# jamornsriwasansak/evplp

Hardware: AMD Instinct MI355X
Metric: Mpaths/s (higher is better)
Workload: dtype f32

## Files before the change

evplp_amd/__init__.py:

```python
from __future__ import annotations

import ctypes as C
import os
from typing import Optional, Sequence

import numpy as np

_HERE = os.path.dirname(os.path.abspath(__file__))
LIB_PATH = os.environ.get("EVPLP_LIB") or os.path.join(_HERE, "lib", "libevplp_hip.so")
INCLUDE_DIR = os.path.join(os.path.dirname(_HERE), "include")

ABI_VERSION = 5

OK, ERR_INVALID, ERR_NO_DEVICE, ERR_HIP, ERR_IO, ERR_PARSE, ERR_OOM = 0, -1, -2, -3, -4, -5, -6
USABLE_VPL, USABLE_PHOTON, LAMBERT_ONLY, PHONG_ONLY = 1, 2, 4, 8
MIS_MODES = {"one": 0, "balance": 1, "max": 2, "power2": 3, "geometryClamp": 4, "geometryBrdfClamp": 5}
BVH_LBVH, BVH_SAH, BVH_SBVH, BVH_LBVH_GPU = 0, 1, 2, 3
(BUF_RECORDS, BUF_GBUF_POSITION, BUF_GBUF_NORMAL, BUF_GBUF_DIFFUSE, BUF_GBUF_PHONG, BUF_LIGHT,
 BUF_VPL_ACCUM, BUF_PHOTON_ACCUM, BUF_COUNT) = range(9)
(PASS_PRIMARY, PASS_LIGHT_TRACE, PASS_GATHER_VPL, PASS_GATHER_VSL, PASS_SPLAT, PASS_RESOLVE, PASS_PATH_TRACE,
 PASS_GATHER_LVC, PASS_COUNT) = range(9)

RECORD_DTYPE = np.dtype([
    ("pos", np.float32, 3), ("flags", np.uint32),
# ... 581 lines not shown
    def adaptive_tiles(self) -> np.ndarray:
        out = np.zeros(((self.H + 7) // 8, (self.W + 7) // 8), dtype=np.int32)
        self._check(self._lib.evplp_adaptive_tiles(self._h, _ptr(out), out.size))
        return out

    def adaptive_set_budgets(self, samples_per_tile):
        b = np.ascontiguousarray(samples_per_tile, dtype=np.int32)
        self._check(self._lib.evplp_adaptive_set_budgets(self._h, _ptr(b), b.size))

    def adaptive_budgets(self) -> np.ndarray:
        out = np.zeros(((self.H + 7) // 8, (self.W + 7) // 8), dtype=np.int32)
        self._check(self._lib.evplp_adaptive_budgets(self._h, _ptr(out), out.size))
        return out

    def adaptive_budget_window(self, window: int):
        self._check(self._lib.evplp_adaptive_budget_window(self._h, int(window)))

    def adaptive_tile_noise(self, scale, light_scale=1.0, mask_emitter=False) -> np.ndarray:
        out = np.zeros(((self.H + 7) // 8, (self.W + 7) // 8), dtype=np.float64)
        self._check(self._lib.evplp_adaptive_tile_noise(self._h, float(scale), float(light_scale), int(mask_emitter), _ptr(out), out.size))
        return out

    def set_blocks(self, image_blocks=None):
        if image_blocks is None:
            self._check(self._lib.evplp_set_blocks(self._h, None, 0)); return
        b = np.ascontiguousarray(image_blocks, dtype=np.int32)
        self._check(self._lib.evplp_set_blocks(self._h, _ptr(b), b.size))

    def blocks(self) -> np.ndarray:
        n = self._check(self._lib.evplp_get_blocks(self._h, None, 0))
        out = np.zeros(n, dtype=np.int32)
        self._check(self._lib.evplp_get_blocks(self._h, _ptr(out), n))
        return out

    def calibrate_blocks(self, on: bool = True):
        self._check(self._lib.evplp_calibrate_blocks(self._h, int(on)))

    def block_costs(self) -> np.ndarray:
        sr = self.cfg.strip_rows if self.cfg.strip_count > 1 else (self.H + 7) // 8 * 8
        out = np.zeros((self.H + sr - 1) // sr, dtype=np.uint64)
        self._check(self._lib.evplp_block_costs(self._h, _ptr(out), out.size))
        return out

    def buffer_info(self, which: int):
        p, n = C.c_void_p(), C.c_size_t()
        self._check(self._lib.evplp_buffer_info(self._h, which, C.byref(p), C.byref(n)))
        return p.value, n.value

    def bind_buffer(self, which: int, device_ptr: int, nbytes: int):
        self._check(self._lib.evplp_bind_buffer(self._h, which, C.c_void_p(device_ptr), nbytes))

    def buffer_bytes(self, which: int) -> int:
        n = C.c_size_t()
        self._check(self._lib.evplp_buffer_info(self._h, which, None, C.byref(n)))
        return n.value

    def download(self, which: int) -> np.ndarray:
        n = self.buffer_bytes(which)
        if which == BUF_RECORDS:
            out = np.empty(n // 96, dtype=RECORD_DTYPE)
        else:
            out = np.empty((self.local_rows, self.W, 4), dtype=np.float32)
        self._check(self._lib.evplp_download(self._h, which, _ptr(out), n))
        return out

    def upload(self, which: int, data: np.ndarray):
        data = np.ascontiguousarray(data)
        self._check(self._lib.evplp_upload(self._h, which, _ptr(data), data.nbytes))

    def pass_stats(self, which: int) -> dict:
        s = PassStats()
        self._check(self._lib.evplp_pass_stats_get(self._h, which, C.byref(s)))
        return {"ms": s.ms, "pairs": s.pairs, "rays": s.rays, "usable": s.usable, "dominant_kernel_ms": s.dominant_kernel_ms,
                "nodes": s.reserved[0] | (s.reserved[1] << 32), "shaded": s.shaded, "launches": s.launches,
                "samples": (s.reserved[0] | (s.reserved[1] << 32)) if which == PASS_GATHER_VSL else 0}

    def profile_kernels(self, on: bool = True):
        self._check(self._lib.evplp_profile_kernels(self._h, int(on)))

    def profile_passes(self, on: bool = True):
        self._check(self._lib.evplp_profile_passes(self._h, int(on)))

    def debug_counters(self, which: int) -> np.ndarray:
        out = np.zeros(256, dtype=np.uint64)
        n = self._check(self._lib.evplp_debug_counters(self._h, which, _ptr(out), out.size))
        return out[:n]

    def global_rows(self) -> np.ndarray:
        from . import strips
        if self.cfg.strip_count <= 1:
            return strips.global_rows(self.H, self.cfg.strip_rank, self.cfg.strip_count, self.cfg.strip_rows)
        return strips.rows_of_blocks(self.H, self.blocks(), self.cfg.strip_rows, self.local_rows)


def refit_levels(nodes, level_capacity: int = 64):
    raw = np.ascontiguousarray(nodes).view(np.uint8).reshape(-1, 64)
    n = raw.shape[0]
    height, order, begin = np.zeros(max(n, 1), np.int32), np.zeros(max(n, 1), np.int32), np.zeros(max(level_capacity, 0) + 1, np.int32)
    rc = lib().evplp_refit_levels(_ptr(raw), n, _ptr(height), _ptr(order), _ptr(begin), int(level_capacity))
    if rc < 0:
        raise EvplpError(rc, "evplp_refit_levels: not a tree (a child index out of range, a node reached twice, a cycle), or more heights than level_capacity")
    return height[:n], order[:int(begin[rc])], begin[:rc + 1]


def accel_cost(nodes) -> dict:
    raw = np.ascontiguousarray(nodes).view(np.uint8).reshape(-1, 64)
    out = (C.c_double * 5)()
    rc = lib().evplp_accel_cost(_ptr(raw), raw.shape[0], out)
    if rc < 0:
        raise EvplpError(rc, "evplp_accel_cost: not a tree (a child index out of range, a node reached twice, a cycle), or no nodes")
    return {"cost": out[0], "root_area": out[1], "inner_area": out[2], "leaf_pair_area": out[3], "leaf_tri_area": out[4], "reached_nodes": rc}


Context.refit_levels = staticmethod(refit_levels)


def deal_blocks(costs, n_ranks: int, capacity_blocks: int) -> np.ndarray:
    c = np.ascontiguousarray(costs, dtype=np.uint64)
    owner = np.zeros(c.size, dtype=np.int32)
    rc = lib().evplp_deal_blocks(_ptr(c), c.size, n_ranks, capacity_blocks, _ptr(owner))
    if rc < 0:
        raise EvplpError(rc, "evplp_deal_blocks: the blocks do not fit the ranks' capacity")
    return owner


def plan_budgets(rel, n_t, samples: int, min_samples: int = 1, tile_rel_mse: float = 0.0, reference_quantile: float = 1.0) -> np.ndarray:
    r = np.ascontiguousarray(rel, dtype=np.float64)
    n = np.ascontiguousarray(n_t, dtype=np.int32)
    if r.size != n.size:
        raise ValueError(f"plan_budgets: {r.size} noise figures but {n.size} sample counts")
    out = np.zeros(n.shape, dtype=np.int32)
    rc = lib().evplp_plan_budgets(_ptr(r), _ptr(n), n.size, int(samples), int(min_samples), float(tile_rel_mse), float(reference_quantile), _ptr(out))
    if rc < 0:
        raise EvplpError(rc, "evplp_plan_budgets: samples 1 .. 64, min_samples 0 .. samples, reference_quantile in (0, 1], finite rel >= 0, >= 1 tile")
    return out


def split_model(num_light_paths: int, photons_per_path: int, n_ranks: int):
    out = (C.c_double * 2)()
    rc = lib().evplp_group_split_model(num_light_paths, photons_per_path, n_ranks, C.byref(out))
    return bool(rc == 1), out[0], out[1]


def rank_blocks(costs, owner, rank: int) -> np.ndarray:
    o = np.ascontiguousarray(owner, dtype=np.int32)
    c = None if costs is None else np.ascontiguousarray(costs, dtype=np.uint64)
    out = np.zeros(o.size, dtype=np.int32)
    n = lib().evplp_rank_blocks(_ptr(c), _ptr(o), o.size, rank, _ptr(out), out.size)
    if n < 0:
        raise EvplpError(n, "evplp_rank_blocks")
    return out[:n]


class Group:

    def __init__(self, res_x, res_y, num_light_paths, num_vpl_light_paths, photons_per_path, n_ranks, devices=None, strip_rows=0,
                 use_rccl=False, deterministic=False, bvh_builder=BVH_SAH, overlap_light_tracing=False, partition="strips", strip_capacity_pct=0, split_light_paths=0, cut_scratch_bytes=0, vsl_mask_bytes=0):
        self._lib = lib()
        cfg = Config()
        cfg.abi_version = ABI_VERSION; cfg.res_x = res_x; cfg.res_y = res_y
        cfg.num_light_paths = num_light_paths; cfg.num_vpl_light_paths = num_vpl_light_paths; cfg.photons_per_path = photons_per_path
        cfg.bvh_builder = bvh_builder; cfg.deterministic = int(deterministic); cfg.overlap_light_tracing = int(overlap_light_tracing)
        cfg.cut_scratch_bytes = int(cut_scratch_bytes); cfg.vsl_mask_bytes = int(vsl_mask_bytes)
        gc = GroupConfig(); gc.n_ranks = n_ranks; gc.strip_rows = strip_rows; gc.use_rccl = int(use_rccl)
        if partition not in PARTITIONS:
            raise ValueError(f"partition: one of {sorted(PARTITIONS)}, got {partition!r}")
        gc.partition = PARTITIONS[partition]; gc.strip_capacity_pct = int(strip_capacity_pct); gc.split_light_paths = int(split_light_paths)
# ... 281 lines not shown
```

evplp_amd/csrc/context.cpp:

```cpp
#include "context.hpp"

#include <algorithm>
#include <cmath>
#include <cstdarg>
#include <cstddef>
#include <cstdio>
#include <cstring>
#include <vector>
#include <cstdlib>

using namespace evplp;

static thread_local char g_create_error[512] = "";
constexpr size_t kDefaultCutScratchBytes = (size_t)8 << 30, kDefaultVslMaskBytes = (size_t)2 << 30;

void evplp_context::set_error(const char *fmt, ...) {
    va_list ap; va_start(ap, fmt);
    vsnprintf(error, sizeof(error), fmt, ap);
    va_end(ap);
}

#define CTX_CHECK(ctx) do { if (!(ctx)) return EVPLP_ERR_INVALID; if ((ctx)->quiesce && std::this_thread::get_id() != (ctx)->worker_tid) (ctx)->quiesce((ctx)->quiesce_arg); } while (0)
#define HIP_TRY(ctx, expr) do { hipError_t e_ = (expr); if (e_ != hipSuccess) { (ctx)->set_error("%s failed: %s", #expr, hipGetErrorString(e_)); return EVPLP_ERR_HIP; } } while (0)

static size_t buffer_bytes(const evplp_context *c, int which) {
    const size_t px = (size_t)c->st.W * c->st.local_rows;
    if (which == EVPLP_BUF_RECORDS) return sizeof(evplp_record) * (size_t)c->cfg.num_light_paths * c->cfg.photons_per_path;
    return px * sizeof(float4);
}

static int settle_splat(evplp_context *c);
static int adapt_reset(evplp_context *c);
namespace evplp { AdaptTiles adapt_view(const evplp_context *c, float scale); }

namespace evplp { void set_context_error(evplp_context *ctx, const char *text) { if (ctx) ctx->set_error("%s", text ? text : ""); } }

extern "C" int evplp_abi_version(void) { return EVPLP_ABI_VERSION; }

extern "C" const char *evplp_last_error(const evplp_context *ctx) { return ctx ? ctx->error : g_create_error; }

extern "C" int evplp_create(const evplp_config *cfg, evplp_context **out) {
    if (!cfg || !out) { snprintf(g_create_error, sizeof(g_create_error), "evplp_create: null argument"); return EVPLP_ERR_INVALID; }
    *out = nullptr;
    if (cfg->abi_version != EVPLP_ABI_VERSION) { snprintf(g_create_error, sizeof(g_create_error), "ABI version mismatch: caller %d, library %d", cfg->abi_version, EVPLP_ABI_VERSION); return EVPLP_ERR_INVALID; }
    if (cfg->res_x <= 0 || cfg->res_y <= 0 || cfg->photons_per_path == 0 || cfg->num_light_paths == 0) {
        snprintf(g_create_error, sizeof(g_create_error), "evplp_create: resolution, num_light_paths and photons_per_path must be positive"); return EVPLP_ERR_INVALID;
    }
    if (cfg->gather_splits_per_wave < 0 || cfg->gather_splits_per_wave > 32 || (cfg->gather_splits_per_wave & (cfg->gather_splits_per_wave - 1)) != 0) {
        snprintf(g_create_error, sizeof(g_create_error), "evplp_create: gather_splits_per_wave must be 0 (automatic) or a power of two <= 32"); return EVPLP_ERR_INVALID;
    }
    if (cfg->strip_capacity_rows < 0) { snprintf(g_create_error, sizeof(g_create_error), "evplp_create: strip_capacity_rows is negative"); return EVPLP_ERR_INVALID; }
    if (cfg->num_vpl_light_paths > cfg->num_light_paths) {
        snprintf(g_create_error, sizeof(g_create_error), "evplp_create: num_vpl_light_paths > num_light_paths (VPLs are the first paths of the same set, lighttracing.cu:368)"); return EVPLP_ERR_INVALID;
    }
    int strip_count = cfg->strip_count > 0 ? cfg->strip_count : 1;
    int strip_rows = strip_count == 1 ? ((cfg->res_y + 7) / 8) * 8 : cfg->strip_rows;
    if (strip_rows <= 0 || (strip_rows % 8) != 0 || cfg->strip_rank < 0 || cfg->strip_rank >= strip_count) {
        snprintf(g_create_error, sizeof(g_create_error), "evplp_create: strip_rows must be a positive multiple of 8 and 0 <= strip_rank < strip_count"); return EVPLP_ERR_INVALID;
    }
    int ndev = 0;
    hipError_t e = hipGetDeviceCount(&ndev);
    if (e != hipSuccess || ndev <= 0) {
        snprintf(g_create_error, sizeof(g_create_error), "no HIP device available (%s); libevplp_hip has no CPU fallback", e != hipSuccess ? hipGetErrorString(e) : "device count 0");
        return EVPLP_ERR_NO_DEVICE;
    }
    if (cfg->device < 0 || cfg->device >= ndev) { snprintf(g_create_error, sizeof(g_create_error), "device %d out of range (%d devices)", cfg->device, ndev); return EVPLP_ERR_INVALID; }
    e = hipSetDevice(cfg->device);
    if (e != hipSuccess) { snprintf(g_create_error, sizeof(g_create_error), "hipSetDevice: %s", hipGetErrorString(e)); return EVPLP_ERR_NO_DEVICE; }

    evplp_context *c = new evplp_context();
    c->cfg = *cfg; c->cfg.strip_count = strip_count; c->cfg.strip_rows = strip_rows;
    if (const char *env = std::getenv("EVPLP_BVH_BUILDER"))
        c->env_bvh_builder = !std::strcmp(env, "sbvh") ? EVPLP_BVH_SBVH : !std::strcmp(env, "lbvh") ? EVPLP_BVH_LBVH : !std::strcmp(env, "gpu") ? EVPLP_BVH_LBVH_GPU : EVPLP_BVH_SAH;
    if (const char *env = std::getenv("EVPLP_CUTS")) c->env_cuts = atoi(env) != 0 ? 1 : 0;
    if (const char *env = std::getenv("EVPLP_ITEM_DEAL")) c->env_item_deal = atoi(env) != 0 ? 1 : 0;
    if (const char *env = std::getenv("EVPLP_CUT_BYTES")) c->env_cut_bytes = (size_t)strtoull(env, nullptr, 10);
    if (const char *env = std::getenv("EVPLP_GATHER_K")) { int v = atoi(env); if (v >= 1 && v <= 32 && (v & (v - 1)) == 0) c->env_gather_k = v; }
    if (const char *env = std::getenv("EVPLP_TILE_BLOCK_LOG2")) c->env_tile_block_log2 = std::max(0, atoi(env));
    if (const char *env = std::getenv("EVPLP_SPLIT_MIN")) c->env_split_min = std::max(0, atoi(env));
    c->st.W = cfg->res_x; c->st.H = cfg->res_y;
    c->st.strip_rank = cfg->strip_rank; c->st.strip_count = strip_count; c->st.strip_rows = strip_rows;
    int nblocks = (cfg->res_y + strip_rows - 1) / strip_rows;
    int owned = (nblocks + strip_count - 1) / strip_count;
    if (strip_count > 1 && cfg->strip_capacity_rows > owned * strip_rows) owned = std::min((cfg->strip_capacity_rows + strip_rows - 1) / strip_rows, nblocks);
    c->st.local_rows = owned * strip_rows;
    c->st.cap_blocks = owned; c->image_blocks = nblocks;
    c->rows_in_image = 0;
    for (int l = 0; l < c->st.local_rows; l++) if (c->st.global_row(l) < c->st.H) c->rows_in_image++;

    auto fail = [&](const char *what, hipError_t err) {
        snprintf(g_create_error, sizeof(g_create_error), "%s: %s", what, hipGetErrorString(err));
        evplp_destroy(c); return err == hipErrorOutOfMemory ? EVPLP_ERR_OOM : EVPLP_ERR_HIP;
    };
    if ((e = hipStreamCreateWithFlags(&c->own_stream, hipStreamNonBlocking)) != hipSuccess) return fail("hipStreamCreate", e);
    c->stream = c->own_stream;
    if (cfg->overlap_light_tracing) {
        if ((e = hipStreamCreateWithFlags(&c->aux_stream, hipStreamNonBlocking)) != hipSuccess) return fail("hipStreamCreate", e);
        if ((e = hipEventCreateWithFlags(&c->ev_records_read, hipEventDisableTiming)) != hipSuccess) return fail("hipEventCreate", e);
        if ((e = hipEventCreateWithFlags(&c->ev_light_done, hipEventDisableTiming)) != hipSuccess) return fail("hipEventCreate", e);
        if ((e = hipEventCreateWithFlags(&c->ev_back_read, hipEventDisableTiming)) != hipSuccess) return fail("hipEventCreate", e);
    }
    for (int i = 0; i < EVPLP_PASS_COUNT; i++) {
        if ((e = hipEventCreate(&c->ev_begin[i])) != hipSuccess) return fail("hipEventCreate", e);
        if ((e = hipEventCreate(&c->ev_end[i])) != hipSuccess) return fail("hipEventCreate", e);
        if ((e = hipEventCreate(&c->ev_dom_begin[i])) != hipSuccess) return fail("hipEventCreate", e);
        if ((e = hipEventCreate(&c->ev_dom_end[i])) != hipSuccess) return fail("hipEventCreate", e);
    }
    for (int b = 0; b < EVPLP_BUF_COUNT; b++) {
        size_t bytes = buffer_bytes(c, b);
        if ((e = hipMalloc(&c->buf[b], bytes)) != hipSuccess) return fail("hipMalloc(buffer)", e);
        if ((e = hipMemset(c->buf[b], 0, bytes)) != hipSuccess) return fail("hipMemset", e);
        c->buf_owned[b] = true;
    }
    const uint32_t nvpl_slots = std::max<uint32_t>(cfg->num_vpl_light_paths * cfg->photons_per_path, 1u);
    if ((e = hipMalloc((void **)&c->d_vpls, sizeof(evplp_record) * nvpl_slots)) != hipSuccess) return fail("hipMalloc(vpls)", e);
    if ((e = hipMalloc((void **)&c->d_vpl_src, sizeof(uint32_t) * nvpl_slots)) != hipSuccess) return fail("hipMalloc(vpl_src)", e);
    if ((e = hipMalloc((void **)&c->d_scalars, 64 * sizeof(uint32_t))) != hipSuccess) return fail("hipMalloc(scalars)", e);
    if ((e = hipMemset(c->d_scalars, 0, 64 * sizeof(uint32_t))) != hipSuccess) return fail("hipMemset", e);
    if ((e = hipMalloc((void **)&c->d_counters, sizeof(PassCounters) * EVPLP_PASS_COUNT)) != hipSuccess) return fail("hipMalloc(counters)", e);
    if ((e = hipMemset(c->d_counters, 0, sizeof(PassCounters) * EVPLP_PASS_COUNT)) != hipSuccess) return fail("hipMemset", e);
    if ((e = hipMalloc((void **)&c->d_rgb, sizeof(float) * 3 * (size_t)c->st.W * c->st.local_rows)) != hipSuccess) return fail("hipMalloc(rgb)", e);
    c->tiles_x = (c->st.W + 7) / 8; c->tiles_y = c->st.local_rows / 8;
    const size_t ntiles = (size_t)c->tiles_x * c->tiles_y;
    const size_t nrec = (size_t)cfg->num_light_paths * cfg->photons_per_path;
    {
        size_t mean = ntiles ? nrec * 2 / std::max<size_t>(ntiles, 1) : 0, k = 64;
        while (k < 8 * mean && k < (1u << 20)) k <<= 1;
        c->bin_stride = (uint32_t)k;
        if (const char *env = std::getenv("EVPLP_BIN_STRIDE")) c->bin_stride = (uint32_t)std::max(1, atoi(env));
        c->bucket_w_log2 = 4; c->bucket_h_log2 = kBucketTilesLog2 - 4;
        auto count_buckets = [&]() {
            c->buckets_x = (c->tiles_x + (1 << c->bucket_w_log2) - 1) >> c->bucket_w_log2;
            c->num_buckets = c->buckets_x * ((c->tiles_y + (1 << c->bucket_h_log2) - 1) >> c->bucket_h_log2);
        };
        count_buckets();
        while (c->num_buckets > kMaxBuckets && c->bucket_w_log2 + c->bucket_h_log2 < kMaxBucketTilesLog2) {
            if (c->bucket_h_log2 < c->bucket_w_log2) c->bucket_h_log2++; else c->bucket_w_log2++;
            count_buckets();
        }
        if (c->num_buckets > kMaxBuckets) {
            snprintf(g_create_error, sizeof(g_create_error), "evplp_create: more than %d x %d image tiles in one context (use row strips)", kMaxBuckets, 1 << kMaxBucketTilesLog2);
            evplp_destroy(c); return EVPLP_ERR_INVALID;
        }
        c->num_bin_groups = (int32_t)((nrec + kBinGroup - 1) / kBinGroup);
    }
    if ((e = hipMalloc((void **)&c->d_tile_box, sizeof(float4) * 2 * std::max<size_t>(ntiles, 1))) != hipSuccess) return fail("hipMalloc(tile_box)", e);
    if ((e = hipMalloc((void **)&c->d_summary, sizeof(uint32_t) * (kSummaryFinal + kSummaryStride))) != hipSuccess) return fail("hipMalloc(summary)", e);
    if (const char *env = std::getenv("EVPLP_TILE_MIXED")) c->env_tile_mixed = atoi(env) != 0 ? 1 : 0;
    if (const char *env = std::getenv("EVPLP_TILE_HEAVY")) c->heavy_threshold = (uint32_t)std::max(atoi(env), 1);
    c->mixed_trigger = 2u * c->heavy_threshold;
    if (const char *env = std::getenv("EVPLP_TILE_MIXED_TRIGGER")) c->mixed_trigger = (uint32_t)std::max(atoi(env), 0);
    c->heavy_cap = (uint32_t)std::min<size_t>(std::max<size_t>((size_t)c->tiles_x * c->tiles_y, 1), 2048);
    if (const char *env = std::getenv("EVPLP_TILE_HEAVY_CAP")) c->heavy_cap = (uint32_t)std::max(atoi(env), 1);
    if ((e = hipMalloc((void **)&c->d_heavy_list, sizeof(uint32_t) * c->heavy_cap)) != hipSuccess) return fail("hipMalloc(heavy list)", e);
    if ((e = hipMalloc((void **)&c->d_tile_flags, std::max<size_t>((size_t)c->tiles_x * c->tiles_y, 1))) != hipSuccess) return fail("hipMalloc(tile flags)", e);
    if ((e = hipMemset(c->d_summary, 0, sizeof(uint32_t) * (kSummaryFinal + kSummaryStride))) != hipSuccess) return fail("hipMemset(summary)", e);
    if ((e = hipMalloc((void **)&c->d_tile_pairs, sizeof(uint32_t) * std::max<size_t>(ntiles, 1))) != hipSuccess) return fail("hipMalloc(tile_pairs)", e);
    if ((e = hipMalloc((void **)&c->d_tile_frags, sizeof(uint32_t) * std::max<size_t>(ntiles, 1))) != hipSuccess) return fail("hipMalloc(tile_frags)", e);
    if ((e = hipMalloc((void **)&c->d_tile_cursor, sizeof(uint32_t) * (ntiles + 1))) != hipSuccess) return fail("hipMalloc(tile_cursor)", e);
    const size_t ngroups = std::max(c->num_bin_groups, 1);
    if ((e = hipMalloc((void **)&c->d_seg, sizeof(uint32_t) * ngroups * kSegCap)) != hipSuccess) return fail("hipMalloc(seg)", e);
    if ((e = hipMalloc((void **)&c->d_seg_off, sizeof(uint16_t) * ngroups * (c->num_buckets + 1))) != hipSuccess) return fail("hipMalloc(seg_off)", e);
    if ((e = hipMalloc((void **)&c->d_big_list, sizeof(uint32_t) * ngroups * kBinGroup)) != hipSuccess) return fail("hipMalloc(big_list)", e);
    if ((e = hipMalloc((void **)&c->d_big_count, sizeof(uint32_t) * ngroups)) != hipSuccess) return fail("hipMalloc(big_count)", e);
    if ((e = hipMalloc((void **)&c->d_bin_items, sizeof(uint32_t) * std::max<size_t>(ntiles * c->bin_stride, 1))) != hipSuccess) return fail("hipMalloc(bin_items)", e);
    if (cfg->deterministic && (e = hipMalloc((void **)&c->d_bin_items_tmp, sizeof(uint32_t) * std::max<size_t>(ntiles * c->bin_stride, 1))) != hipSuccess) return fail("hipMalloc(bin_items_tmp)", e);
    if ((e = hipMalloc((void **)&c->d_compact, sizeof(float4) * kCompactF4 * nrec)) != hipSuccess) return fail("hipMalloc(compact)", e);
    if ((e = hipHostMalloc((void **)&c->h_summary, 8 * sizeof(uint32_t), hipHostMallocDefault)) != hipSuccess) return fail("hipHostMalloc(summary)", e);
    std::memset(c->h_summary, 0, 8 * sizeof(uint32_t));
    for (int i = 0; i < 2; i++) {
        if ((e = hipEventCreate(&c->pend[i].ev)) != hipSuccess) return fail("hipEventCreate", e);
        c->pend[i].h = c->h_summary + 4 * i;
    }
    *out = c;
    return EVPLP_OK;
}

static void free_scene_device(evplp_context *c) {
    hipFree((void *)c->sc.nodes); hipFree((void *)c->sc.nodes4); hipFree((void *)c->sc.leaves); hipFree((void *)c->sc.tri_flat); hipFree((void *)c->sc.tri_index); hipFree((void *)c->sc.attrs);
    hipFree((void *)c->sc.materials); hipFree((void *)c->sc.textures); hipFree((void *)c->sc.tex_pool); hipFree((void *)c->sc.light_cdf);
    std::memset(&c->sc, 0, sizeof(c->sc));
    hipFree(c->d_refit_order); hipFree(c->d_refit_boxes); hipFree(c->d_refit_stage); if (c->h_refit_stage) hipHostFree(c->h_refit_stage);
    c->d_refit_order = nullptr; c->d_refit_boxes = c->d_refit_stage = c->h_refit_stage = nullptr;
    c->refit_levels = 0; c->refit_level_begin.clear(); std::vector<BvhNode>().swap(c->host_nodes);
    hipFree(c->d_cost); if (c->h_cost) hipHostFree(c->h_cost);
    c->d_cost = c->h_cost = nullptr; c->refit_reached = c->refit_leaf_refs = 0;
}

extern "C" void evplp_destroy(evplp_context *c) {
    if (!c) return;
    hipSetDevice(c->cfg.device);
    c->npend = 0;
    if (c->aux_stream) hipStreamSynchronize(c->aux_stream);
    if (c->own_stream) hipStreamSynchronize(c->own_stream);
    for (int b = 0; b < EVPLP_BUF_COUNT; b++) if (c->buf_owned[b]) hipFree(c->buf[b]);
    free_scene_device(c);
    hipFree(c->d_vpls); hipFree(c->d_vpl_src); hipFree(c->d_scalars); hipFree(c->d_counters); hipFree(c->d_rgb); hipFree(c->d_partial); hipFree(c->d_vsl_masks); hipFree(c->d_cuts); hipFree(c->d_primary_cuts); hipFree(c->d_lt_overflow);
    hipFree(c->d_tile_cursor); hipFree(c->d_bin_items); hipFree(c->d_bin_items_tmp); hipFree(c->d_seg); hipFree(c->d_seg_off); hipFree(c->d_big_list); hipFree(c->d_big_count);
    hipFree(c->d_compact); hipFree(c->d_tile_box); hipFree(c->d_tile_pairs); hipFree(c->d_summary); hipFree(c->d_heavy_list); hipFree(c->d_tile_flags);
    hipFree(c->d_proxy_slabs); hipFree(c->d_proxy_hm); hipFree(c->d_tile_frags); hipFree(c->d_blocks); hipFree(c->d_block_cost);
    hipFree(c->d_err_ref); hipFree(c->d_err_keep); hipFree(c->d_err_rows);
    hipFree(c->d_noise); hipFree(c->d_noise_keep); hipFree(c->d_noise_rows);
    hipFree(c->d_adapt_tiles); hipFree(c->d_adapt_snap); hipFree(c->d_adapt_mask);
    hipFree(c->d_dn_var); hipFree(c->d_dn_pack); hipFree(c->d_dn_u);
    hipFree(c->d_pt_batch); hipFree(c->d_pt_first); hipFree(c->d_pt_table); hipFree(c->d_tile_noise);
    for (int i = 0; i < EVPLP_PASS_COUNT; i++) {
        if (c->ev_begin[i]) hipEventDestroy(c->ev_begin[i]);
        if (c->ev_end[i]) hipEventDestroy(c->ev_end[i]);
        if (c->ev_dom_begin[i]) hipEventDestroy(c->ev_dom_begin[i]);
        if (c->ev_dom_end[i]) hipEventDestroy(c->ev_dom_end[i]);
    }
    for (int i = 0; i < 2; i++) if (c->pend[i].ev) hipEventDestroy(c->pend[i].ev);
    if (c->h_summary) hipHostFree(c->h_summary);
    if (c->aux_stream) hipStreamDestroy(c->aux_stream);
    if (c->ev_records_read) hipEventDestroy(c->ev_records_read);
    if (c->ev_light_done) hipEventDestroy(c->ev_light_done);
    if (c->ev_back_read) hipEventDestroy(c->ev_back_read);
    if (c->ev_refit_staged) hipEventDestroy(c->ev_refit_staged);
    for (int i = 0; i < 5; i++) if (c->ev_refit[i]) hipEventDestroy(c->ev_refit[i]);
    for (int i = 0; i < 2; i++) if (c->ev_cost[i]) hipEventDestroy(c->ev_cost[i]);
    hipFree(c->records_back);
    for (int k = 0; k < 4; k++) hipFree(c->gbuf_back[k]);
    hipFree(c->d_tile_box_back);
    if (c->own_stream) hipStreamDestroy(c->own_stream);
    delete c;
}

extern "C" int evplp_set_stream(evplp_context *c, void *s) {
    CTX_CHECK(c);
// ... 315 lines not shown
static int refit_prepare(evplp_context *c) {
    if (c->refit_levels > 0) return EVPLP_OK;
    const int32_t nn = c->accel_nodes;
    if (c->host_nodes.empty()) {
        c->host_nodes.resize((size_t)nn);
        HIP_TRY(c, hipMemcpyAsync(c->host_nodes.data(), c->sc.nodes, sizeof(BvhNode) * (size_t)nn, hipMemcpyDeviceToHost, c->stream));
        HIP_TRY(c, hipStreamSynchronize(c->stream));
    }
    std::vector<int32_t> height((size_t)nn), order((size_t)nn);
    c->refit_level_begin.assign((size_t)kMaxDepth + 1, 0);
    const int levels = evplp_refit_levels(c->host_nodes.data(), nn, height.data(), order.data(), c->refit_level_begin.data(), kMaxDepth);
    if (levels >= 1) {
        c->refit_reached = c->refit_level_begin[(size_t)levels]; c->refit_leaf_refs = 0;
        for (int32_t k = 0; k < c->refit_reached; k++) {
            const BvhNode &f = c->host_nodes[(size_t)order[(size_t)k]];
            c->refit_leaf_refs += (f.c0 < 0 && f.c0 != kNoChild) + (f.c1 < 0 && f.c1 != kNoChild);
        }
    }
    std::vector<BvhNode>().swap(c->host_nodes);
    if (levels < 1) { c->set_error("evplp_refit_accel: the node array is not a tree of at most %d levels", kMaxDepth); return EVPLP_ERR_INVALID; }
    const size_t stage = 9 * (size_t)c->scene_tris + (size_t)c->sc.light_count;
    hipError_t e = hipMalloc((void **)&c->d_refit_order, sizeof(int32_t) * (size_t)nn);
    if (e == hipSuccess) e = hipMalloc((void **)&c->d_refit_boxes, sizeof(float) * 6 * (size_t)nn);
    if (e == hipSuccess) e = hipMalloc((void **)&c->d_refit_stage, sizeof(float) * stage);
    if (e == hipSuccess) e = hipHostMalloc((void **)&c->h_refit_stage, sizeof(float) * stage, hipHostMallocDefault);
    if (e == hipSuccess) e = hipMemcpy(c->d_refit_order, order.data(), sizeof(int32_t) * (size_t)nn, hipMemcpyHostToDevice);
    if (e == hipSuccess && !c->ev_refit_staged) e = hipEventCreateWithFlags(&c->ev_refit_staged, hipEventDisableTiming);
    for (int i = 0; i < 5 && e == hipSuccess; i++) if (!c->ev_refit[i]) e = hipEventCreate(&c->ev_refit[i]);
    if (e != hipSuccess) { c->set_error("evplp_refit_accel: plan and staging: %s", hipGetErrorString(e)); return e == hipErrorOutOfMemory ? EVPLP_ERR_OOM : EVPLP_ERR_HIP; }
    c->refit_levels = levels;
    return EVPLP_OK;
}

extern "C" int evplp_refit_accel(evplp_context *c) {
    CTX_CHECK(c);
    if (!evplp::refit_check(c)) return EVPLP_ERR_INVALID;
    if (!c->scene_dirty) return EVPLP_OK;
    HIP_TRY(c, hipSetDevice(c->cfg.device));
    int rc = refit_prepare(c); if (rc) return rc;
    std::vector<float> verts; std::vector<int32_t> first;
    flatten_verts(c, verts, first);
    std::vector<char> has_area;
    const float pad = scene_pad(verts.data(), first.back(), has_area);
    std::vector<float> cdf;
    scene_scalars(c, verts.data(), c->sc.light_first, c->sc.light_count, cdf);
    const bool timed = c->profile_passes, stages = timed && c->profile_kernels;
    if (c->refit_count > 0) HIP_TRY(c, hipEventSynchronize(c->ev_refit_staged));
    size_t staged = 0;
    for (size_t mi = 0; mi < c->meshes.size(); mi++) if (c->mesh_dirty[mi]) {
        const size_t n = 9 * (size_t)(first[mi + 1] - first[mi]);
        std::memcpy(c->h_refit_stage + staged, &verts[9 * (size_t)first[mi]], sizeof(float) * n);
        staged += n;
    }
    if (timed) HIP_TRY(c, hipEventRecord(c->ev_refit[0], c->stream));
    if (staged) HIP_TRY(c, hipMemcpyAsync(c->d_refit_stage, c->h_refit_stage, sizeof(float) * staged, hipMemcpyHostToDevice, c->stream));
    staged = 0;
    for (size_t mi = 0; mi < c->meshes.size();) {
        if (!c->mesh_dirty[mi]) { mi++; continue; }
        size_t me = mi; while (me < c->meshes.size() && c->mesh_dirty[me]) me++;
        const int32_t count = first[me] - first[mi];
        refit_scatter(c->d_refit_stage + staged, first[mi], count, (TriAttr *)c->sc.attrs, c->stream);
        staged += 9 * (size_t)count; mi = me;
    }
    if (stages) HIP_TRY(c, hipEventRecord(c->ev_refit[1], c->stream));
    RefitScene r; std::memset(&r, 0, sizeof(r));
    r.nodes = (BvhNode *)c->sc.nodes; r.nnodes = c->accel_nodes; r.leaves = (LeafBlock *)c->sc.leaves; r.tri_flat = (TriFlat *)c->sc.tri_flat; r.tri_index = c->sc.tri_index;
    r.nslots = 4 * c->accel_leaves; r.attrs = c->sc.attrs; r.ntri = c->scene_tris; r.boxes = c->d_refit_boxes;
    refit_leaves(r, c->stream);
    if (stages) HIP_TRY(c, hipEventRecord(c->ev_refit[2], c->stream));
    for (int32_t l = 0; l < c->refit_levels; l++)
        refit_level(r, c->d_refit_order + c->refit_level_begin[(size_t)l], c->refit_level_begin[(size_t)l + 1] - c->refit_level_begin[(size_t)l], pad, c->stream);
    if (stages) HIP_TRY(c, hipEventRecord(c->ev_refit[3], c->stream));
    build_nodes4_into(c->sc.nodes, c->accel_nodes, c->stream, (BvhNode4 *)c->sc.nodes4);
    if (c->mesh_dirty[(size_t)c->light_mesh]) {
        float *h = c->h_refit_stage + 9 * (size_t)c->scene_tris;
        std::memcpy(h, cdf.data(), sizeof(float) * cdf.size());
        HIP_TRY(c, hipMemcpyAsync((void *)c->sc.light_cdf, h, sizeof(float) * cdf.size(), hipMemcpyHostToDevice, c->stream));
    }
    HIP_TRY(c, hipEventRecord(c->ev_refit_staged, c->stream));
    if (timed) HIP_TRY(c, hipEventRecord(c->ev_refit[4], c->stream));
    if (c->aux_stream) HIP_TRY(c, hipStreamWaitEvent(c->aux_stream, c->ev_refit_staged, 0));
    HIP_TRY(c, hipGetLastError());
    c->accel_pad = pad; c->refit_timed = timed; c->refit_stages_timed = stages; c->refit_count++; c->refits_since_build++;
    c->primary_cuts_valid = false; c->tile_box_valid = false;
    std::fill(c->mesh_dirty.begin(), c->mesh_dirty.end(), 0); c->scene_dirty = false;
    if (c->policy_ratio > 0.0) {
        double q[5];
        if ((rc = measure_cost(c, q))) return rc;
        if (q[0] > c->policy_ratio * c->built_cost) {
            if ((rc = build_accel(c, c->policy_builder))) return rc;
            c->policy_rebuilds++; c->last_action = 2;
        } else c->last_action = 1;
    }
    return EVPLP_OK;
}

static int measure_cost(evplp_context *c, double out[5]) {
    int rc = refit_prepare(c); if (rc) return rc;
    const int32_t nchunks = (c->refit_reached + kCostChunk - 1) / kCostChunk;
    const size_t bytes = sizeof(double) * (1 + 3 * (size_t)nchunks);
    if (!c->d_cost) {
        hipError_t e = hipMalloc((void **)&c->d_cost, bytes);
        if (e == hipSuccess) e = hipHostMalloc((void **)&c->h_cost, bytes, hipHostMallocDefault);
        if (e != hipSuccess) { c->set_error("evplp_accel_quality: the sums' arrays: %s", hipGetErrorString(e)); return e == hipErrorOutOfMemory ? EVPLP_ERR_OOM : EVPLP_ERR_HIP; }
    }
    const bool timed = c->profile_passes;
    for (int i = 0; i < 2 && timed; i++) if (!c->ev_cost[i]) HIP_TRY(c, hipEventCreate(&c->ev_cost[i]));
    if (timed) HIP_TRY(c, hipEventRecord(c->ev_cost[0], c->stream));
    accel_cost(c->sc.nodes, c->accel_nodes, c->d_refit_order, c->refit_reached, c->d_cost, c->stream);
    HIP_TRY(c, hipGetLastError());
    HIP_TRY(c, hipMemcpyAsync(c->h_cost, c->d_cost, bytes, hipMemcpyDeviceToHost, c->stream));
    if (timed) HIP_TRY(c, hipEventRecord(c->ev_cost[1], c->stream));
    HIP_TRY(c, hipStreamSynchronize(c->stream));
    c->cost_timed = timed;
    accel_cost_finish(c->h_cost + 1, nchunks, c->h_cost[0], out);
    if (!c->built_cost_known) { c->built_cost = out[0]; c->built_cost_known = true; }
    return EVPLP_OK;
}

namespace evplp {
bool accel_quality_check(evplp_context *c, const char *name) {
    if (!c->accel_built) { c->set_error("%s: scene not built (evplp_build_accel)", name); return false; }
    if (c->scene_dirty) { c->set_error("%s: vertices were updated (evplp_update_mesh): call evplp_refit_accel or evplp_build_accel first", name); return false; }
    return true;
}
bool refit_policy_check(evplp_context *c, double max_cost_ratio, int32_t rebuild_builder) {
    if (!(max_cost_ratio >= 0.0) || !std::isfinite(max_cost_ratio)) { c->set_error("evplp_set_refit_policy: max_cost_ratio must be finite and >= 0 (0: off)"); return false; }
    if (rebuild_builder < -1 || rebuild_builder > EVPLP_BVH_LBVH_GPU) { c->set_error("evplp_set_refit_policy: rebuild_builder %d is neither an evplp_bvh_builder nor -1", rebuild_builder); return false; }
    if (c->scene_dirty) { c->set_error("evplp_set_refit_policy: vertices were updated (evplp_update_mesh): call evplp_refit_accel or evplp_build_accel first"); return false; }
    return true;
}
}

extern "C" int evplp_accel_quality(evplp_context *c, struct evplp_accel_quality *out) {
    CTX_CHECK(c);
    if (!out) { c->set_error("evplp_accel_quality: null destination"); return EVPLP_ERR_INVALID; }
    if (!evplp::accel_quality_check(c, "evplp_accel_quality")) return EVPLP_ERR_INVALID;
    HIP_TRY(c, hipSetDevice(c->cfg.device));
    double q[5];
    const int rc = measure_cost(c, q); if (rc) return rc;
    std::memset(out, 0, sizeof(*out));
    out->cost = q[0]; out->root_area = q[1]; out->inner_area = q[2]; out->leaf_pair_area = q[3]; out->leaf_tri_area = q[4];
    out->built_cost = c->built_cost; out->reached_nodes = c->refit_reached; out->leaf_refs = c->refit_leaf_refs;
    out->refits_since_build = c->refits_since_build; out->policy_rebuilds = c->policy_rebuilds; out->last_action = c->last_action;
    return EVPLP_OK;
}

extern "C" int evplp_set_refit_policy(evplp_context *c, double max_cost_ratio, int32_t rebuild_builder) {
    CTX_CHECK(c);
    if (!evplp::refit_policy_check(c, max_cost_ratio, rebuild_builder)) return EVPLP_ERR_INVALID;
    if (max_cost_ratio > 0.0 && c->accel_built && !c->built_cost_known) {
        HIP_TRY(c, hipSetDevice(c->cfg.device));
        double q[5];
        const int rc = measure_cost(c, q); if (rc) return rc;
    }
    c->policy_ratio = max_cost_ratio; c->policy_builder = rebuild_builder;
    return EVPLP_OK;
}

extern "C" int evplp_refit_info(evplp_context *c, int32_t *refits, int32_t *levels, float *last_refit_ms) {
    CTX_CHECK(c);
    if (refits) *refits = c->refit_count;
    if (levels) *levels = c->refit_levels;
    if (last_refit_ms) {
        *last_refit_ms = 0.f;
        if (c->refit_count > 0 && c->refit_timed) {
            HIP_TRY(c, hipSetDevice(c->cfg.device));
// ... 31 lines not shown
    HIP_TRY(c, hipMemcpyAsync(host_dst, src[which], bytes, hipMemcpyDeviceToHost, c->stream));
    HIP_TRY(c, hipStreamSynchronize(c->stream));
    return EVPLP_OK;
}

static uint32_t split_threshold(const evplp_context *c, uint32_t footprint) {
    if (c->env_split_min > 0) return (uint32_t)c->env_split_min;
    return footprint == (uint32_t)EVPLP_FOOTPRINT_PROXY ? 1536u : 768u;
}
static int settle_one(evplp_context *c) {
    if (c->npend == 0) return EVPLP_OK;
    HIP_TRY(c, hipSetDevice(c->cfg.device));
    HIP_TRY(c, hipEventSynchronize(c->pend[0].ev));
    const uint32_t total = c->pend[0].h[0], biggest = c->pend[0].h[1], overflow = c->pend[0].h[2];
    SplatArgs a = c->pend[0].args;
    std::swap(c->pend[0], c->pend[1]); c->npend--;
    c->last_bin_entries = total; c->last_bin_max = biggest;
    if (!overflow) return EVPLP_OK;
    HIP_TRY(c, hipStreamSynchronize(c->stream));
    uint64_t want = 64; while (want < (uint64_t)overflow + overflow / 4) want <<= 1;
    const size_t ntiles = (size_t)c->tiles_x * c->tiles_y;
    if (want * ntiles > 0xfffffff0ull) { c->set_error("photon bins: %llu slots per tile needed", (unsigned long long)overflow); return EVPLP_ERR_OOM; }
    if (want > c->bin_stride) {
        hipFree(c->d_bin_items); c->d_bin_items = nullptr;
        if (c->d_bin_items_tmp) { hipFree(c->d_bin_items_tmp); c->d_bin_items_tmp = nullptr; }
        hipError_t e1 = hipMalloc((void **)&c->d_bin_items, sizeof(uint32_t) * ntiles * want);
        hipError_t e2 = c->cfg.deterministic ? hipMalloc((void **)&c->d_bin_items_tmp, sizeof(uint32_t) * ntiles * want) : hipSuccess;
        if (e1 != hipSuccess || e2 != hipSuccess) { c->set_error("photon bins: cannot allocate %zu x %llu slots", ntiles, (unsigned long long)want); return EVPLP_ERR_OOM; }
        c->bin_stride = (uint32_t)want;
    }
    a.bin_items = c->d_bin_items; a.bin_items_tmp = c->d_bin_items_tmp; a.bin_stride = c->bin_stride;
    for (int i = 0; i < c->npend; i++) {
        c->pend[i].args.bin_items = c->d_bin_items; c->pend[i].args.bin_items_tmp = c->d_bin_items_tmp; c->pend[i].args.bin_stride = c->bin_stride;
    }
    HIP_TRY(c, hipEventRecord(c->ev_begin[EVPLP_PASS_SPLAT], c->stream));
    c->pass_timed[EVPLP_PASS_SPLAT] = true;
    launch_splat_bin(a, c->stream);
    const bool split_tiles = c->cfg.deterministic ? true : biggest >= split_threshold(c, a.fp.splat_footprint);
    launch_splat_tiles(a, split_tiles, c->stream, c->ev_dom_begin[EVPLP_PASS_SPLAT], c->ev_dom_end[EVPLP_PASS_SPLAT]);
    HIP_TRY(c, hipEventRecord(c->ev_end[EVPLP_PASS_SPLAT], c->stream));
    if (c->aux_stream) HIP_TRY(c, hipEventRecord((const void *)a.records == c->buf[EVPLP_BUF_RECORDS] ? c->ev_records_read : c->ev_back_read, c->stream));
    HIP_TRY(c, hipGetLastError());
    return EVPLP_OK;
}
static int settle_splat(evplp_context *c) {
    while (c->npend > 0) { int rc = settle_one(c); if (rc) return rc; }
    return EVPLP_OK;
}
static int settle_readers_of(evplp_context *c, const void *records, const void *g_pos) {
    int upto = 0;
    for (int i = 0; i < c->npend; i++)
        if ((records && (const void *)c->pend[i].args.records == records) || (g_pos && (const void *)c->pend[i].args.g_pos == g_pos)) upto = i + 1;
    for (int i = 0; i < upto; i++) { int rc = settle_one(c); if (rc) return rc; }
    return EVPLP_OK;
}
static int pass_ready(evplp_context *c, const char *name, bool need_camera, bool settle = true) {
    if (!c->accel_built) { c->set_error("%s: scene not built (evplp_build_accel)", name); return EVPLP_ERR_INVALID; }
    if (c->scene_dirty) { c->set_error("%s: vertices were updated (evplp_update_mesh): call evplp_refit_accel or evplp_build_accel first", name); return EVPLP_ERR_INVALID; }
    if (need_camera && !c->camera_set) { c->set_error("%s: camera not set", name); return EVPLP_ERR_INVALID; }
    hipError_t e = hipSetDevice(c->cfg.device);
    if (e != hipSuccess) { c->set_error("hipSetDevice: %s", hipGetErrorString(e)); return EVPLP_ERR_HIP; }
    return settle ? settle_splat(c) : EVPLP_OK;
}
#ifndef EVPLP_TRAVERSAL_STATS
#define EVPLP_TRAVERSAL_STATS 0
#endif
static bool pass_uses_counters(int pass) {
    return pass == EVPLP_PASS_GATHER_VPL || pass == EVPLP_PASS_GATHER_VSL || pass == EVPLP_PASS_GATHER_LVC || pass == EVPLP_PASS_PATH_TRACE || EVPLP_TRAVERSAL_STATS || EVPLP_DEBUG_NAN;
}
static int pass_begin(evplp_context *c, int pass) {
    if (pass_uses_counters(pass)) HIP_TRY(c, hipMemsetAsync(&c->d_counters[pass], 0, sizeof(PassCounters), c->stream));
    if (c->profile_passes || pass == EVPLP_PASS_PRIMARY) HIP_TRY(c, hipEventRecord(c->ev_begin[pass], c->stream));
    c->pass_ran[pass] = true; c->pass_has_dom[pass] = false; c->pass_timed[pass] = c->profile_passes;
    return EVPLP_OK;
}
static int pass_end(evplp_context *c, int pass) {
    if (c->pass_timed[pass]) HIP_TRY(c, hipEventRecord(c->ev_end[pass], c->stream));
    if (c->aux_stream && (pass == EVPLP_PASS_GATHER_VPL || pass == EVPLP_PASS_GATHER_VSL || pass == EVPLP_PASS_GATHER_LVC || pass == EVPLP_PASS_SPLAT))
        HIP_TRY(c, hipEventRecord(c->ev_records_read, c->stream));
    HIP_TRY(c, hipGetLastError());
    return EVPLP_OK;
}

static bool jitter_within_cuts(const evplp_context *c, const float jitter[2]) {
    return std::fabs(jitter[0]) <= 1.99f / (float)c->st.W && std::fabs(jitter[1]) <= 1.99f / (float)c->st.H;
}
static void primary_cuts_into(evplp_context *c, PrimaryArgs &a) {
    PrimaryCutArgs pc; std::memset(&pc, 0, sizeof(pc));
    pc.nodes = c->sc.nodes; pc.st = c->st; pc.cam = c->cam; pc.tiles_x = c->tiles_x; pc.tiles_y = c->tiles_y;
    pc.gw_log2 = 1; pc.gh_log2 = (c->st.strip_count == 1 || c->st.strip_rows >= 16) ? 1 : 0;
    pc.groups_x = (c->tiles_x + (1 << pc.gw_log2) - 1) >> pc.gw_log2; pc.groups_y = (c->tiles_y + (1 << pc.gh_log2) - 1) >> pc.gh_log2;
    if (!c->d_primary_cuts) {
        hipError_t me = hipMalloc((void **)&c->d_primary_cuts, (size_t)pc.groups_x * pc.groups_y * (size_t)kCutSlotBytes);
        if (me != hipSuccess) { (void)hipGetLastError(); c->d_primary_cuts = nullptr; }
        c->primary_cuts_valid = false;
    }
    if (c->d_primary_cuts) {
        pc.cuts = c->d_primary_cuts;
        if (!c->primary_cuts_valid) { launch_primary_cuts(pc, c->stream); c->primary_cuts_valid = true; }
        a.cuts = c->d_primary_cuts; a.cut_gw_log2 = pc.gw_log2; a.cut_gh_log2 = pc.gh_log2; a.cut_groups_x = pc.groups_x;
    }
}

extern "C" int evplp_primary(evplp_context *c, const float jitter[2], int32_t clear_light) {
    CTX_CHECK(c);
    static const int kPlanes[4] = { EVPLP_BUF_GBUF_POSITION, EVPLP_BUF_GBUF_NORMAL, EVPLP_BUF_GBUF_DIFFUSE, EVPLP_BUF_GBUF_PHONG };
    bool flip = c->aux_stream && c->npend > 0 && !c->gbuf_exposed && !c->gbuf_pos_exposed;
    for (int k = 0; k < 4 && flip; k++) flip = c->buf_owned[kPlanes[k]];
    int rc = pass_ready(c, "evplp_primary", true, !flip); if (rc) return rc;
    if (flip && c->gbuf_back[0] && (rc = settle_readers_of(c, nullptr, c->gbuf_back[0]))) return rc;
    if (flip) {
        for (int k = 0; k < 4; k++) if (!c->gbuf_back[k]) {
            hipError_t me = hipMalloc(&c->gbuf_back[k], buffer_bytes(c, kPlanes[k]));
            if (me != hipSuccess) { c->set_error("evplp_primary: second G-buffer: %s", hipGetErrorString(me)); return EVPLP_ERR_OOM; }
        }
        if (!c->d_tile_box_back) {
            hipError_t me = hipMalloc((void **)&c->d_tile_box_back, sizeof(float4) * 2 * std::max<size_t>((size_t)c->tiles_x * c->tiles_y, 1));
            if (me != hipSuccess) { c->set_error("evplp_primary: second tile-box table: %s", hipGetErrorString(me)); return EVPLP_ERR_OOM; }
        }
        for (int k = 0; k < 4; k++) std::swap(c->buf[kPlanes[k]], c->gbuf_back[k]);
        std::swap(c->d_tile_box, c->d_tile_box_back);
    }
    PrimaryArgs a; std::memset(&a, 0, sizeof(a));
    a.sc = c->sc; a.st = c->st; a.cam = c->cam;
    a.jitter[0] = jitter ? jitter[0] : 0.f; a.jitter[1] = jitter ? jitter[1] : 0.f; a.clear_light = clear_light;
    a.g_pos = (float4 *)c->buf[EVPLP_BUF_GBUF_POSITION]; a.g_nrm = (float4 *)c->buf[EVPLP_BUF_GBUF_NORMAL];
    a.g_dif = (float4 *)c->buf[EVPLP_BUF_GBUF_DIFFUSE]; a.g_phg = (float4 *)c->buf[EVPLP_BUF_GBUF_PHONG];
    a.g_light = (float4 *)c->buf[EVPLP_BUF_LIGHT];
    a.tile_box = c->d_tile_box;
    if (!std::isfinite(a.jitter[0]) || !std::isfinite(a.jitter[1])) { c->set_error("evplp_primary: jitter is not finite"); return EVPLP_ERR_INVALID; }
    if (c->env_cuts != 0 && c->tiles_x * c->tiles_y > 0 && jitter_within_cuts(c, a.jitter)) primary_cuts_into(c, a);
    if ((rc = pass_begin(c, EVPLP_PASS_PRIMARY))) return rc;
    launch_primary(a, c->stream);
    c->tile_box_valid = !c->gbuf_pos_exposed;
    c->stats_host[EVPLP_PASS_PRIMARY].rays = 2ull * (uint64_t)c->st.W * c->rows_in_image;
    return pass_end(c, EVPLP_PASS_PRIMARY);
}

extern "C" int evplp_trace_light_paths(evplp_context *c, uint32_t rng_seed, uint32_t path_begin, uint32_t path_count) {
    CTX_CHECK(c);
    const bool to_back_buffer = c->aux_stream && path_begin == 0 && path_count == c->cfg.num_light_paths && c->buf_owned[EVPLP_BUF_RECORDS] && !c->records_exposed;
    int rc = pass_ready(c, "evplp_trace_light_paths", false, !to_back_buffer); if (rc) return rc;
    if (to_back_buffer && c->records_back && (rc = settle_readers_of(c, c->records_back, nullptr))) return rc;
    if ((uint64_t)path_begin + path_count > c->cfg.num_light_paths) { c->set_error("evplp_trace_light_paths: path range exceeds num_light_paths"); return EVPLP_ERR_INVALID; }
    LightTraceArgs a; std::memset(&a, 0, sizeof(a));
    a.sc = c->sc; a.rng_seed = rng_seed; a.path_begin = path_begin; a.path_count = path_count; a.photons_per_path = c->cfg.photons_per_path;
    a.records = (evplp_record *)c->buf[EVPLP_BUF_RECORDS];
    {
        const size_t threads = ((size_t)path_count + 63) / 64 * 64, need = threads * (size_t)lt_overflow_entries(c->sc) * sizeof(int32_t);
        if (need > c->lt_overflow_bytes) {
            HIP_TRY(c, hipStreamSynchronize(c->stream)); if (c->aux_stream) HIP_TRY(c, hipStreamSynchronize(c->aux_stream));
            hipFree(c->d_lt_overflow); c->d_lt_overflow = nullptr; c->lt_overflow_bytes = 0;
            hipError_t me = hipMalloc((void **)&c->d_lt_overflow, need);
            if (me != hipSuccess) { c->set_error("evplp_trace_light_paths: stack overflow area: %s", hipGetErrorString(me)); return EVPLP_ERR_OOM; }
            c->lt_overflow_bytes = need;
        }
        a.stack_overflow = c->d_lt_overflow; a.overflow_stride = (uint32_t)threads;
    }
    if (!c->aux_stream) {
        if ((rc = pass_begin(c, EVPLP_PASS_LIGHT_TRACE))) return rc;
        launch_light_trace(a, c->stream);
        return pass_end(c, EVPLP_PASS_LIGHT_TRACE);
    }
    if (to_back_buffer) {
        if (!c->records_back) {
            hipError_t me = hipMalloc(&c->records_back, buffer_bytes(c, EVPLP_BUF_RECORDS));
            if (me != hipSuccess) { c->set_error("evplp_trace_light_paths: second record buffer: %s", hipGetErrorString(me)); return EVPLP_ERR_OOM; }
        }
        std::swap(c->buf[EVPLP_BUF_RECORDS], c->records_back);
        std::swap(c->ev_records_read, c->ev_back_read);
        a.records = (evplp_record *)c->buf[EVPLP_BUF_RECORDS];
    }
    HIP_TRY(c, hipStreamWaitEvent(c->aux_stream, c->ev_records_read, 0));
    if (c->pass_ran[EVPLP_PASS_PRIMARY]) HIP_TRY(c, hipStreamWaitEvent(c->aux_stream, c->ev_begin[EVPLP_PASS_PRIMARY], 0));
    if (c->profile_passes) HIP_TRY(c, hipEventRecord(c->ev_begin[EVPLP_PASS_LIGHT_TRACE], c->aux_stream));
    c->pass_ran[EVPLP_PASS_LIGHT_TRACE] = true; c->pass_has_dom[EVPLP_PASS_LIGHT_TRACE] = false; c->pass_timed[EVPLP_PASS_LIGHT_TRACE] = c->profile_passes;
    launch_light_trace(a, c->aux_stream);
    if (c->profile_passes) HIP_TRY(c, hipEventRecord(c->ev_end[EVPLP_PASS_LIGHT_TRACE], c->aux_stream));
    HIP_TRY(c, hipEventRecord(c->ev_light_done, c->aux_stream));
    HIP_TRY(c, hipStreamWaitEvent(c->stream, c->ev_light_done, 0));
    HIP_TRY(c, hipGetLastError());
    return EVPLP_OK;
}

static bool small_gather_launch(const evplp_context *c) { return (size_t)c->tiles_x * (size_t)((c->rows_in_image + 7) / 8) <= 8192; }
static int fill_gather_args(evplp_context *c, const evplp_frame_params *fp, GatherArgs &a, int pass) {
    std::memset(&a, 0, sizeof(a));
    a.sc = c->sc; a.st = c->st; a.fp = *fp; a.pdf_mc2 = fp->pdf_mc * fp->pdf_mc;
    a.g_pos = (const float4 *)c->buf[EVPLP_BUF_GBUF_POSITION]; a.g_nrm = (const float4 *)c->buf[EVPLP_BUF_GBUF_NORMAL];
    a.g_dif = (const float4 *)c->buf[EVPLP_BUF_GBUF_DIFFUSE]; a.g_phg = (const float4 *)c->buf[EVPLP_BUF_GBUF_PHONG];
    a.vpls = c->d_vpls; a.vpl_src_index = c->d_vpl_src; a.nvpl = &c->d_scalars[0];
    a.out = (float4 *)c->buf[EVPLP_BUF_VPL_ACCUM];
    a.partial_stride = (size_t)c->st.W * c->st.local_rows;
    a.counters = &c->d_counters[pass];
    a.splits_per_wave = 1;
    a.block_cost = c->calibrate ? c->d_block_cost : nullptr;
    a.item_deal = c->env_item_deal >= 0 ? c->env_item_deal : (small_gather_launch(c) ? 1 : 0);
    int sh = 8;
    if (c->st.strip_count > 1) { sh = 1; while (sh * 2 <= std::min(8, c->st.strip_rows / 8) && (c->st.strip_rows / 8) % (sh * 2) == 0) sh *= 2; }
    a.block_h_log2 = sh == 8 ? 3 : sh == 4 ? 2 : sh == 2 ? 1 : 0;
    if (c->env_tile_block_log2 >= 0) a.block_h_log2 = std::min(c->env_tile_block_log2, a.block_h_log2);
    return EVPLP_OK;
}
static int ensure_gather_workspace(evplp_context *c, GatherArgs &a, size_t groups) {
    const size_t px = (size_t)c->st.W * c->st.local_rows;
    if (c->partial_groups < groups) {
        HIP_TRY(c, hipStreamSynchronize(c->stream));
        hipFree(c->d_partial); c->d_partial = nullptr; c->partial_groups = 0;
        hipError_t e = hipMalloc((void **)&c->d_partial, sizeof(float4) * groups * px);
        if (e != hipSuccess) { c->set_error("gather: cannot allocate %zu bytes of partial sums: %s", sizeof(float4) * groups * px, hipGetErrorString(e)); return EVPLP_ERR_OOM; }
        c->partial_groups = groups;
    }
    a.partial = c->d_partial;
    return EVPLP_OK;
}
static int check_fp(evplp_context *c, const evplp_frame_params *fp, const char *name) {
    if (!fp) { c->set_error("%s: null frame params", name); return EVPLP_ERR_INVALID; }
    if (fp->photons_per_path != c->cfg.photons_per_path || fp->num_light_paths != c->cfg.num_light_paths || fp->num_vpl_light_paths > c->cfg.num_vpl_light_paths) {
        c->set_error("%s: frame params disagree with the configuration (paths / photons per path)", name); return EVPLP_ERR_INVALID;
    }
    if (fp->mis_mode > 5u) { c->set_error("%s: mis_mode %u out of range", name, fp->mis_mode); return EVPLP_ERR_INVALID; }
    return EVPLP_OK;
}
static size_t nvpl_slots_of(const evplp_context *c) { return std::max<size_t>((size_t)c->cfg.num_vpl_light_paths * c->cfg.photons_per_path, 1); }
static int run_gather(evplp_context *c, const evplp_frame_params *fp, bool vsl) {
    const int pass = vsl ? EVPLP_PASS_GATHER_VSL : EVPLP_PASS_GATHER_VPL;
    const char *name = vsl ? "evplp_gather_vsl" : "evplp_gather_vpl";
    int rc = pass_ready(c, name, false); if (rc) return rc;
    if ((rc = check_fp(c, fp, name))) return rc;
    if (fp->num_vpl_light_paths == 0) { c->set_error("%s: num_vpl_light_paths is 0 (the reference disables the pass, rtcomphoton.h:200-203)", name); return EVPLP_ERR_INVALID; }
    if (c->adapt_pt) { c->set_error("%s: adaptivity is on in path-trace mode (evplp_adaptive_enable_pt): evplp_path_trace only", name); return EVPLP_ERR_INVALID; }
    if (c->d_adapt_tiles && fp->do_accumulate == 0) { c->set_error("%s: adaptivity is on (evplp_adaptive_enable): a gather must accumulate", name); return EVPLP_ERR_INVALID; }
    GatherArgs a; fill_gather_args(c, fp, a, pass);
    AdaptArgs ad{};
    if (c->d_adapt_tiles) { ad.tiles = c->d_adapt_tiles; ad.snap = c->d_adapt_snap; ad.n1 = (int32_t)(c->adapt_n + 1); }
    const bool gbudget = c->adapt_gather_budget;
    const int32_t ntiles_all = c->tiles_x * c->tiles_y, phase = (int32_t)(c->adapt_m % c->adapt_window);
    if (gbudget) ad.tiles = c->d_adapt_mask;
    int k = 1;
    {
        const bool small_launch = small_gather_launch(c);
        k = c->cfg.gather_splits_per_wave > 0 ? c->cfg.gather_splits_per_wave : (small_launch ? 1 : kDefaultSplitsPerWave);
        if (c->env_gather_k > 0) k = c->env_gather_k;
        const size_t max_vpls = std::max<size_t>((size_t)c->cfg.num_vpl_light_paths * c->cfg.photons_per_path, 1);
        while (k > 1 && (max_vpls / kVplSplit + 1) * (size_t)k >= 65536) k >>= 1;
        if (vsl) while (k > 1 && (max_vpls / kVplSplit + 1) * (size_t)k > 4095) k >>= 1;
        if (vsl && (max_vpls / kVplSplit + 1) > 4095) {
            c->set_error("%s: %zu VSL record slots exceed the %d this build can gather in one pass", name, max_vpls, 4094 * kVplSplit); return EVPLP_ERR_INVALID;
        }
    }
    a.splits_per_wave = k;
    if ((rc = ensure_gather_workspace(c, a, (size_t)(kVplSplit / k)))) return rc;
    CutArgs ca; std::memset(&ca, 0, sizeof(ca));
    bool use_cuts = c->env_cuts != 0;
    const int sh = 1 << a.block_h_log2, nby = (c->tiles_y + sh - 1) / sh;
    int band_rows = nby;
    if (use_cuts && nby > 0) {
        ca.nodes = c->sc.nodes; ca.tile_box = c->d_tile_box; ca.tiles_x = c->tiles_x; ca.tiles_y = c->tiles_y;
        ca.gw_log2 = 1; ca.gh_log2 = (sh >= 2 && (c->st.strip_count == 1 || c->st.strip_rows >= 16)) ? 1 : 0;
        ca.groups_x = (c->tiles_x + (1 << ca.gw_log2) - 1) >> ca.gw_log2;
        ca.vpls = c->d_vpls; ca.nvpl = &c->d_scalars[0]; ca.vpl_stride = (uint32_t)nvpl_slots_of(c);
        const size_t per_block_row = (size_t)(sh >> ca.gh_log2) * ca.groups_x * ca.vpl_stride * (size_t)kCutSlotBytes;
        if (c->cut_cap == 0) {
            c->cut_cap = c->env_cut_bytes ? c->env_cut_bytes : (size_t)c->cfg.cut_scratch_bytes;
            if (c->cut_cap == 0) c->cut_cap = kDefaultCutScratchBytes;
        }
        band_rows = (int)std::min<size_t>((size_t)nby, c->cut_cap / std::max<size_t>(per_block_row, 1));
        if (band_rows < 1) { use_cuts = false; band_rows = nby; }
        const size_t need = use_cuts ? per_block_row * (size_t)band_rows : 0;
        if (use_cuts && need > c->cut_bytes) {
            HIP_TRY(c, hipStreamSynchronize(c->stream));
            hipFree(c->d_cuts); c->d_cuts = nullptr; c->cut_bytes = 0;
            if (hipMalloc((void **)&c->d_cuts, need) == hipSuccess) c->cut_bytes = need;
            else { (void)hipGetLastError(); use_cuts = false; band_rows = nby; }
        }
        ca.cuts = c->d_cuts;
        ca.adapt_tiles = c->calibrate ? nullptr : ad.tiles;
    } else use_cuts = false;
    if ((rc = pass_begin(c, pass))) return rc;
    const uint32_t nrec = fp->photons_per_path * fp->num_vpl_light_paths;
    if (gbudget) launch_gather_budget_mask(c->d_adapt_tiles, ntiles_all, phase, c->adapt_window, c->d_adapt_mask, c->stream);
    launch_compact_vpl((const evplp_record *)c->buf[EVPLP_BUF_RECORDS], nrec, c->d_vpls, c->d_vpl_src, &c->d_scalars[0], c->stream);
    if (use_cuts && !c->tile_box_valid) {
        launch_tile_boxes(c->st, (const float4 *)c->buf[EVPLP_BUF_GBUF_POSITION], c->d_tile_box, c->tiles_x, c->tiles_y, c->stream);
        c->tile_box_valid = !c->gbuf_pos_exposed;
    }
    int vsl_groups = 0, vsl_per_launch = 0;
    if (vsl) {
        a.masks_per_split = (int32_t)((nvpl_slots_of(c) + kVplSplit - 1) / kVplSplit);
        a.band_first = 0; a.band_rows = band_rows < nby ? band_rows : 0;
        const size_t tiles = (size_t)gather_launch_tiles(a), per_item = (size_t)k * (size_t)a.masks_per_split * sizeof(unsigned long long);
        vsl_groups = kVplSplit / k;
        vsl_per_launch = vsl_groups;
        if (c->mask_cap == 0) {
            c->mask_cap = (size_t)c->cfg.vsl_mask_bytes;
            if (const char *me = std::getenv("EVPLP_MASK_BYTES")) c->mask_cap = (size_t)strtoull(me, nullptr, 10);
            if (c->mask_cap == 0) c->mask_cap = kDefaultVslMaskBytes;
        }
        const size_t mask_cap = c->mask_cap;
        while (vsl_per_launch > 1 && tiles * (size_t)vsl_per_launch * per_item > mask_cap) vsl_per_launch = (vsl_per_launch + 1) / 2;
        const size_t mask_bytes = tiles * (size_t)vsl_per_launch * per_item;
        if (c->vsl_mask_bytes < mask_bytes) {
            HIP_TRY(c, hipStreamSynchronize(c->stream));
            hipFree(c->d_vsl_masks); c->d_vsl_masks = nullptr; c->vsl_mask_bytes = 0;
            hipError_t e = hipMalloc((void **)&c->d_vsl_masks, mask_bytes);
            if (e != hipSuccess) { c->set_error("gather_vsl: cannot allocate %zu bytes of lit masks: %s", mask_bytes, hipGetErrorString(e)); return EVPLP_ERR_OOM; }
            c->vsl_mask_bytes = mask_bytes;
        }
        a.vsl_masks = (unsigned long long *)c->d_vsl_masks;
    }
    HIP_TRY(c, hipEventRecord(c->ev_dom_begin[pass], c->stream));
    for (int b0 = 0; b0 < nby; b0 += band_rows) {
        const int rows = std::min(band_rows, nby - b0);
        a.band_first = b0; a.band_rows = band_rows < nby ? rows : 0;
        if (use_cuts) {
            const int gshift = ca.gh_log2, groups_total_y = (c->tiles_y + (1 << gshift) - 1) >> gshift;
            ca.group_row_first = (b0 * sh) >> gshift;
            ca.groups_y = std::min(((b0 + rows) * sh + (1 << gshift) - 1) >> gshift, groups_total_y) - ca.group_row_first;
            launch_gather_cuts(ca, c->stream);
            a.cuts = ca.cuts; a.cut_vpl_stride = ca.vpl_stride; a.cut_gw_log2 = ca.gw_log2; a.cut_gh_log2 = ca.gh_log2; a.cut_groups_x = ca.groups_x;
            a.cut_group_row_first = ca.group_row_first;
        }
        if (vsl) {
            for (int g0 = 0; g0 < vsl_groups; g0 += vsl_per_launch) {
                a.group_first = g0; a.group_count = std::min(vsl_per_launch, vsl_groups - g0);
                launch_gather_vsl(a, c->stream, ad);
            }
            a.group_first = 0; a.group_count = 0;
        } else launch_gather_vpl_items(a, c->stream, ad);
    }
    a.band_first = 0; a.band_rows = 0;
    HIP_TRY(c, hipEventRecord(c->ev_dom_end[pass], c->stream));
    if (gbudget) {
        launch_gather_reduce_budget(a, vsl ? 0 : 1, c->d_adapt_tiles, c->d_adapt_mask, c->d_adapt_snap, ad.n1, c->stream);
        launch_gather_budget_step(c->d_adapt_tiles, c->d_adapt_mask, ntiles_all, c->stream);
        for (int4 &r : c->adapt_tiles) if (gather_tile_takes(r, phase, c->adapt_window)) r.x += 1;
        c->adapt_m++;
    } else launch_gather_reduce(a, vsl ? 0 : 1, c->stream, ad);
    c->pass_has_dom[pass] = true;
    if ((rc = pass_end(c, pass))) return rc;
    if (fp->do_accumulate) c->adapt_n++;
    return EVPLP_OK;
}
extern "C" int evplp_gather_vpl(evplp_context *c, const evplp_frame_params *fp) { CTX_CHECK(c); return run_gather(c, fp, false); }
extern "C" int evplp_gather_vsl(evplp_context *c, const evplp_frame_params *fp) { CTX_CHECK(c); return run_gather(c, fp, true); }

extern "C" int evplp_gather_lvc(evplp_context *c, const evplp_frame_params *fp) {
    CTX_CHECK(c);
    const int pass = EVPLP_PASS_GATHER_LVC;
    if (c->adapt_pt) { c->set_error("evplp_gather_lvc: adaptivity is on in path-trace mode (evplp_adaptive_enable_pt): evplp_path_trace only"); return EVPLP_ERR_INVALID; }
    if (c->d_adapt_tiles) { c->set_error("evplp_gather_lvc: adaptivity is on (evplp_adaptive_enable): VPL and VSL gathers only"); return EVPLP_ERR_INVALID; }
    int rc = pass_ready(c, "evplp_gather_lvc", false); if (rc) return rc;
    if ((rc = check_fp(c, fp, "evplp_gather_lvc"))) return rc;
    if (fp->num_vpl_light_paths == 0) { c->set_error("evplp_gather_lvc: num_vpl_light_paths is 0"); return EVPLP_ERR_INVALID; }
    GatherArgs a; fill_gather_args(c, fp, a, pass);
    if ((rc = pass_begin(c, pass))) return rc;
    launch_gather_lvc(a, (const evplp_record *)c->buf[EVPLP_BUF_RECORDS], c->stream);
    return pass_end(c, pass);
}

extern "C" int evplp_path_trace(evplp_context *c, const float camera_pos[3], uint32_t rng_seed, uint32_t max_bounces, int32_t do_accumulate) {
    CTX_CHECK(c);
    if (c->d_adapt_tiles && !c->adapt_pt) { c->set_error("evplp_path_trace: adaptivity is on (evplp_adaptive_enable): VPL and VSL gathers only"); return EVPLP_ERR_INVALID; }
    if (c->adapt_budget) { c->set_error("evplp_path_trace: budget mode (evplp_adaptive_enable_pt(ctx, 2)): evplp_path_trace_batch only"); return EVPLP_ERR_INVALID; }
    if (c->adapt_pt && !do_accumulate) { c->set_error("evplp_path_trace: adaptivity is on (evplp_adaptive_enable_pt): a sample must accumulate"); return EVPLP_ERR_INVALID; }
    int rc = pass_ready(c, "evplp_path_trace", false); if (rc) return rc;
    if (!camera_pos) { c->set_error("evplp_path_trace: null camera position"); return EVPLP_ERR_INVALID; }
    PathTraceArgs a; std::memset(&a, 0, sizeof(a));
// ... 622 lines not shown
    return EVPLP_OK;
}
extern "C" int evplp_adaptive_budget_window(evplp_context *c, int32_t window) {
    CTX_CHECK(c);
    const char *name = "evplp_adaptive_budget_window";
    if (!c->adapt_gather_budget) { c->set_error("%s: gather budget mode is off (evplp_adaptive_enable(ctx, 2))", name); return EVPLP_ERR_INVALID; }
    if (window < 1 || window > kGatherBudgetMaxWindow) { c->set_error("%s: a window is 1 .. %d calls, not %d", name, kGatherBudgetMaxWindow, window); return EVPLP_ERR_INVALID; }
    c->adapt_window = window; c->adapt_m = 0;
    return EVPLP_OK;
}
extern "C" int evplp_adaptive_budgets(evplp_context *c, int32_t *out, int32_t capacity) {
    CTX_CHECK(c);
    if (!c->adapt_budget) { c->set_error("evplp_adaptive_budgets: budget mode is off (evplp_adaptive_enable(ctx, 2) / evplp_adaptive_enable_pt(ctx, 2))"); return EVPLP_ERR_INVALID; }
    const int64_t n = image_tile_count(c);
    if (!out || capacity < n) { c->set_error("evplp_adaptive_budgets: the image has %lld tiles, the output holds %d", (long long)n, capacity); return EVPLP_ERR_INVALID; }
    std::fill(out, out + n, 0);
    evplp::adaptive_budgets_into(c, out);
    return (int)n;
}
namespace evplp {
void adaptive_budgets_into(const evplp_context *c, int32_t *out) {
    for_own_tiles(c, [&](size_t local, size_t image) { out[image] = c->adapt_tiles[local].w; });
}
int adaptive_tile_noise_into(evplp_context *c, float scale, float ls, int32_t mask_emitter, double *out) {
    HIP_TRY(c, hipSetDevice(c->cfg.device));
    const size_t nt = adapt_tile_count(c);
    if (nt && !c->d_tile_noise) HIP_TRY(c, hipMalloc((void **)&c->d_tile_noise, sizeof(double) * nt));
    int rc = resolve_to_device(c, scale, scale, ls, mask_emitter, 0, true, false);
    if (rc) return rc;
    const double K = (double)c->noise_k, B = (double)c->noise_b;
    launch_tile_noise(c->st, noise_moments_of(c), K, B, (double)scale * (double)scale * K, (const float4 *)c->buf[EVPLP_BUF_LIGHT], ls, mask_emitter,
                      c->d_rgb, adapt_view(c, scale), (int32_t)nt, c->d_tile_noise, c->stream);
    HIP_TRY(c, hipGetLastError());
    std::vector<double> local(nt);
    if (nt) HIP_TRY(c, hipMemcpyAsync(local.data(), c->d_tile_noise, sizeof(double) * nt, hipMemcpyDeviceToHost, c->stream));
    HIP_TRY(c, hipStreamSynchronize(c->stream));
    for_own_tiles(c, [&](size_t l, size_t image) { out[image] = local[l]; });
    return EVPLP_OK;
}
}
extern "C" int evplp_adaptive_tile_noise(evplp_context *c, float scale, float ls, int32_t mask_emitter, double *rel_per_image_tile, int32_t capacity) {
    CTX_CHECK(c);
    const char *name = "evplp_adaptive_tile_noise";
    if (!c->d_adapt_tiles) { c->set_error("%s: adaptivity is off (evplp_adaptive_enable)", name); return EVPLP_ERR_INVALID; }
    const int64_t n = image_tile_count(c);
    if (!rel_per_image_tile || capacity < n) { c->set_error("%s: the image has %lld tiles, the output holds %d", name, (long long)n, capacity); return EVPLP_ERR_INVALID; }
    int rc = noise_ready(c, name);
    if (rc) return rc;
    std::fill(rel_per_image_tile, rel_per_image_tile + n, 0.0);
    if ((rc = evplp::adaptive_tile_noise_into(c, scale, ls, mask_emitter, rel_per_image_tile))) return rc;
    return (int)n;
}

static void count_rows_in_image(evplp_context *c) {
    c->rows_in_image = 0;
    for (int l = 0; l < c->st.local_rows; l++) if (c->st.global_row(l) < c->st.H) c->rows_in_image++;
}

extern "C" int evplp_set_blocks(evplp_context *c, const int32_t *image_blocks, int32_t count) {
    CTX_CHECK(c);
    { int rc_ = settle_splat(c); if (rc_) return rc_; }
    if (c->st.strip_count <= 1) { c->set_error("evplp_set_blocks: the context is not a row-strip context (strip_count > 1)"); return EVPLP_ERR_INVALID; }
    const int cap = c->st.cap_blocks, nb = c->image_blocks;
    if (image_blocks && (count < 0 || count > cap)) { c->set_error("evplp_set_blocks: %d blocks do not fit the context's %d (strip_capacity_rows)", count, cap); return EVPLP_ERR_INVALID; }
    std::vector<int32_t> table;
    if (image_blocks) {
        table.assign((size_t)cap + nb, -1);
        for (int l = 0; l < cap; l++) table[(size_t)l] = nb + l;
        for (int l = 0; l < count; l++) {
            const int b = image_blocks[l];
            if (b < 0 || b >= nb || table[(size_t)cap + b] >= 0) { c->set_error("evplp_set_blocks: block %d is outside the image's %d blocks or listed twice", b, nb); return EVPLP_ERR_INVALID; }
            table[(size_t)l] = b; table[(size_t)cap + b] = l;
        }
    }
    HIP_TRY(c, hipSetDevice(c->cfg.device));
    HIP_TRY(c, hipStreamSynchronize(c->stream)); if (c->aux_stream) HIP_TRY(c, hipStreamSynchronize(c->aux_stream));
    if (image_blocks) {
        if (!c->d_blocks) HIP_TRY(c, hipMalloc((void **)&c->d_blocks, sizeof(int32_t) * ((size_t)cap + nb)));
        HIP_TRY(c, hipMemcpy(c->d_blocks, table.data(), sizeof(int32_t) * table.size(), hipMemcpyHostToDevice));
        c->blocks_host.swap(table);
        c->st.blocks = c->d_blocks; c->st.blocks_host = c->blocks_host.data();
    } else { c->st.blocks = nullptr; c->st.blocks_host = nullptr; c->blocks_host.clear(); }
    count_rows_in_image(c);
    c->primary_cuts_valid = false; c->tile_box_valid = false;
    return evplp_clear_accumulators(c);
}
extern "C" int evplp_get_blocks(evplp_context *c, int32_t *image_blocks, int32_t capacity) {
    CTX_CHECK(c);
    int n = 0;
    const int cap = c->st.local_rows / c->st.strip_rows;
    for (int l = 0; l < cap; l++) {
        const int b = c->st.global_block(l);
        if (b >= c->image_blocks) continue;
        if (image_blocks && n < capacity) image_blocks[n] = b;
        n++;
    }
    return n;
}
extern "C" int evplp_calibrate_blocks(evplp_context *c, int32_t on) {
    CTX_CHECK(c);
    HIP_TRY(c, hipSetDevice(c->cfg.device));
    const size_t bytes = sizeof(unsigned long long) * (size_t)std::max(c->st.local_rows / std::max(c->st.strip_rows, 1), 1);
    if (on) {
        if (!c->d_block_cost) HIP_TRY(c, hipMalloc((void **)&c->d_block_cost, bytes));
        HIP_TRY(c, hipMemsetAsync(c->d_block_cost, 0, bytes, c->stream));
    }
    c->calibrate = on != 0;
    return EVPLP_OK;
}
extern "C" int evplp_block_costs(evplp_context *c, uint64_t *cost_per_image_block, int32_t capacity) {
    CTX_CHECK(c);
    if (!cost_per_image_block || capacity < c->image_blocks) { c->set_error("evplp_block_costs: the output needs room for %d blocks", c->image_blocks); return EVPLP_ERR_INVALID; }
    if (!c->d_block_cost) { c->set_error("evplp_block_costs: no calibration has run (evplp_calibrate_blocks)"); return EVPLP_ERR_INVALID; }
    HIP_TRY(c, hipSetDevice(c->cfg.device));
    const int cap = c->st.local_rows / c->st.strip_rows;
    std::vector<unsigned long long> local((size_t)cap);
    HIP_TRY(c, hipMemcpyAsync(local.data(), c->d_block_cost, sizeof(unsigned long long) * local.size(), hipMemcpyDeviceToHost, c->stream));
    HIP_TRY(c, hipStreamSynchronize(c->stream));
    for (int b = 0; b < c->image_blocks; b++) cost_per_image_block[b] = 0;
    int n = 0;
    for (int l = 0; l < cap; l++) {
        const int b = c->st.global_block(l);
        if (b < c->image_blocks) { cost_per_image_block[b] += local[(size_t)l]; n++; }
    }
    return n;
}

extern "C" int evplp_clear_accumulators(evplp_context *c) {
    CTX_CHECK(c);
    { int rc_ = settle_splat(c); if (rc_) return rc_; }
    HIP_TRY(c, hipSetDevice(c->cfg.device));
    HIP_TRY(c, hipMemsetAsync(c->buf[EVPLP_BUF_VPL_ACCUM], 0, buffer_bytes(c, EVPLP_BUF_VPL_ACCUM), c->stream));
    HIP_TRY(c, hipMemsetAsync(c->buf[EVPLP_BUF_PHOTON_ACCUM], 0, buffer_bytes(c, EVPLP_BUF_PHOTON_ACCUM), c->stream));
    HIP_TRY(c, hipMemsetAsync(c->buf[EVPLP_BUF_LIGHT], 0, buffer_bytes(c, EVPLP_BUF_LIGHT), c->stream));
    c->adapt_n = 0; c->splat_n = 0;
    if (c->d_adapt_tiles) { int rc_ = adapt_reset(c); if (rc_) return rc_; }
    if (c->d_noise) return noise_restart(c);
    return EVPLP_OK;
}

extern "C" int evplp_local_rows(const evplp_context *c) { return c ? c->st.local_rows : EVPLP_ERR_INVALID; }

extern "C" int evplp_buffer_info(evplp_context *c, int32_t which, void **ptr, size_t *bytes) {
    CTX_CHECK(c);
    if (which < 0 || which >= EVPLP_BUF_COUNT) { c->set_error("evplp_buffer_info: bad buffer id %d", which); return EVPLP_ERR_INVALID; }
    if (ptr) {
        *ptr = c->buf[which];
        if (which == EVPLP_BUF_GBUF_POSITION) { c->gbuf_pos_exposed = true; c->tile_box_valid = false; }
        if (which >= EVPLP_BUF_GBUF_POSITION && which <= EVPLP_BUF_GBUF_PHONG) c->gbuf_exposed = true;
        if (which == EVPLP_BUF_RECORDS) c->records_exposed = true;
    }
    if (bytes) *bytes = buffer_bytes(c, which);
    return EVPLP_OK;
}
extern "C" int evplp_bind_buffer(evplp_context *c, int32_t which, void *ptr, size_t bytes) {
    CTX_CHECK(c);
    { int rc_ = settle_splat(c); if (rc_) return rc_; }
    if (which < 0 || which >= EVPLP_BUF_COUNT || !ptr) { c->set_error("evplp_bind_buffer: bad arguments"); return EVPLP_ERR_INVALID; }
    if (bytes < buffer_bytes(c, which)) { c->set_error("evplp_bind_buffer: %zu bytes given, %zu needed", bytes, buffer_bytes(c, which)); return EVPLP_ERR_INVALID; }
    if (((uintptr_t)ptr & 15u) != 0) { c->set_error("evplp_bind_buffer: pointer must be 16-byte aligned"); return EVPLP_ERR_INVALID; }
    HIP_TRY(c, hipSetDevice(c->cfg.device));
    HIP_TRY(c, hipStreamSynchronize(c->stream));
    if (c->buf_owned[which]) hipFree(c->buf[which]);
    c->buf[which] = ptr; c->buf_owned[which] = false;
    if (which == EVPLP_BUF_GBUF_POSITION) { c->gbuf_pos_exposed = true; c->tile_box_valid = false; }
    if (which >= EVPLP_BUF_GBUF_POSITION && which <= EVPLP_BUF_GBUF_PHONG) c->gbuf_exposed = true;
    return EVPLP_OK;
}
extern "C" int evplp_download(evplp_context *c, int32_t which, void *dst, size_t bytes) {
    CTX_CHECK(c);
    { int rc_ = settle_splat(c); if (rc_) return rc_; }
    if (which < 0 || which >= EVPLP_BUF_COUNT || !dst || bytes > buffer_bytes(c, which)) { c->set_error("evplp_download: bad arguments"); return EVPLP_ERR_INVALID; }
    HIP_TRY(c, hipSetDevice(c->cfg.device));
    HIP_TRY(c, hipMemcpyAsync(dst, c->buf[which], bytes, hipMemcpyDeviceToHost, c->stream));
    HIP_TRY(c, hipStreamSynchronize(c->stream));
    return EVPLP_OK;
}
extern "C" int evplp_upload(evplp_context *c, int32_t which, const void *src, size_t bytes) {
    CTX_CHECK(c);
    { int rc_ = settle_splat(c); if (rc_) return rc_; }
    if (which < 0 || which >= EVPLP_BUF_COUNT || !src || bytes > buffer_bytes(c, which)) { c->set_error("evplp_upload: bad arguments"); return EVPLP_ERR_INVALID; }
    HIP_TRY(c, hipSetDevice(c->cfg.device));
    HIP_TRY(c, hipMemcpyAsync(c->buf[which], src, bytes, hipMemcpyHostToDevice, c->stream));
    HIP_TRY(c, hipStreamSynchronize(c->stream));
    if (which == EVPLP_BUF_GBUF_POSITION) c->tile_box_valid = false;
    return EVPLP_OK;
}

extern "C" int evplp_profile_kernels(evplp_context *c, int32_t on) { CTX_CHECK(c); c->profile_kernels = on != 0; return EVPLP_OK; }
extern "C" int evplp_profile_passes(evplp_context *c, int32_t on) { CTX_CHECK(c); c->profile_passes = on != 0; return EVPLP_OK; }

extern "C" int evplp_debug_counters(evplp_context *c, int32_t pass, uint64_t *out, int32_t capacity) {
    CTX_CHECK(c);
    { int rc_ = settle_splat(c); if (rc_) return rc_; }
    if (pass < 0 || pass >= EVPLP_PASS_COUNT || !out || capacity <= 0) { c->set_error("evplp_debug_counters: bad arguments"); return EVPLP_ERR_INVALID; }
    HIP_TRY(c, hipSetDevice(c->cfg.device));
    HIP_TRY(c, hipStreamSynchronize(c->stream));
    PassCounters pc;
    HIP_TRY(c, hipMemcpy(&pc, &c->d_counters[pass], sizeof(pc), hipMemcpyDeviceToHost));
    const int n = std::min<int>(capacity, (int)(sizeof(pc) / sizeof(uint64_t)));
    std::memcpy(out, &pc, sizeof(uint64_t) * (size_t)n);
    return n;
}

extern "C" int evplp_pass_stats_get(evplp_context *c, int32_t pass, evplp_pass_stats *out) {
    CTX_CHECK(c);
    { int rc_ = settle_splat(c); if (rc_) return rc_; }
    if (pass < 0 || pass >= EVPLP_PASS_COUNT || !out) { c->set_error("evplp_pass_stats_get: bad arguments"); return EVPLP_ERR_INVALID; }
    std::memset(out, 0, sizeof(*out));
    if (!c->pass_ran[pass]) return EVPLP_OK;
    HIP_TRY(c, hipSetDevice(c->cfg.device));
    if (c->pass_timed[pass]) {
        HIP_TRY(c, hipEventSynchronize(c->ev_end[pass]));
        HIP_TRY(c, hipEventElapsedTime(&out->ms, c->ev_begin[pass], c->ev_end[pass]));
    } else {
        HIP_TRY(c, hipStreamSynchronize(c->stream)); if (c->aux_stream) HIP_TRY(c, hipStreamSynchronize(c->aux_stream));
    }
    if (c->pass_has_dom[pass]) { HIP_TRY(c, hipEventElapsedTime(&out->dominant_kernel_ms, c->ev_dom_begin[pass], c->ev_dom_end[pass])); out->launches = 1; }
    else { out->dominant_kernel_ms = out->ms; out->launches = 1; }
    PassCounters pc; uint32_t scal[16];
    HIP_TRY(c, hipMemcpy(&pc, &c->d_counters[pass], sizeof(pc), hipMemcpyDeviceToHost));
    HIP_TRY(c, hipMemcpy(scal, c->d_scalars, sizeof(scal), hipMemcpyDeviceToHost));
    const uint64_t px = (uint64_t)c->st.W * c->rows_in_image;
    if (pass == EVPLP_PASS_GATHER_VPL || pass == EVPLP_PASS_GATHER_VSL) {
        unsigned long long rays = 0, shaded = 0;
        for (int k = 0; k < kCounterShards; k++) { rays += pc.shard_rays[k]; shaded += pc.shard_shaded[k]; }
        out->usable = scal[0]; out->pairs = px * scal[0]; out->rays = rays; out->shaded = shaded; out->reserved[0] = (uint32_t)std::min<unsigned long long>(pc.nodes, 0xffffffffull);
        out->reserved[1] = (uint32_t)(pc.nodes >> 32);
        if (pass == EVPLP_PASS_GATHER_VSL && !EVPLP_TRAVERSAL_STATS) {
            unsigned long long samples = 0; for (int k = 0; k < 64; k++) samples += pc.hist[k];
            out->reserved[0] = (uint32_t)samples; out->reserved[1] = (uint32_t)(samples >> 32);
        }
    } else if (pass == EVPLP_PASS_SPLAT) {
        std::vector<uint32_t> tp((size_t)c->tiles_x * c->tiles_y);
        HIP_TRY(c, hipMemcpy(tp.data(), c->d_tile_pairs, tp.size() * sizeof(uint32_t), hipMemcpyDeviceToHost));
        uint64_t sum = 0; for (uint32_t v : tp) sum += v;
        uint64_t fragments = 0;
        if (c->last_splat_proxy) {
            HIP_TRY(c, hipMemcpy(tp.data(), c->d_tile_frags, tp.size() * sizeof(uint32_t), hipMemcpyDeviceToHost));
            for (uint32_t v : tp) fragments += v;
        }
        out->pairs = sum; out->rays = fragments; out->usable = 0; out->reserved[0] = c->last_bin_entries; out->reserved[1] = c->last_bin_max;
        std::vector<uint32_t> sh((size_t)kSummaryFinal);
        HIP_TRY(c, hipMemcpy(sh.data(), c->d_summary, sh.size() * sizeof(uint32_t), hipMemcpyDeviceToHost));
        uint64_t total = 0;
        for (int k = 0; k < kSummaryShards; k++) total += (uint64_t)sh[(size_t)k * kSummaryStride + 4] | ((uint64_t)sh[(size_t)k * kSummaryStride + 5] << 32);
        out->shaded = total;
    } else if (pass == EVPLP_PASS_PATH_TRACE) { out->pairs = pc.pairs; out->rays = pc.rays; }
    else if (pass == EVPLP_PASS_GATHER_LVC) { out->pairs = pc.pairs; out->rays = pc.rays; }
    else if (pass == EVPLP_PASS_PRIMARY) out->rays = c->stats_host[pass].rays;
    return EVPLP_OK;
}
```

evplp_amd/csrc/context.hpp:

```cpp
#pragma once
#include "evplp_types.h"
#include "kernels.h"

#include <string>
#include <thread>
#include <vector>

namespace evplp {
int build_bvh_gpu(const float *verts_host, int32_t ntri, float pad_scale, hipStream_t stream, BvhDeviceBuild *out);
int build_nodes4(const BvhNode *d_nodes, int32_t nnodes, hipStream_t stream, BvhNode4 **out);
void build_nodes4_into(const BvhNode *d_nodes, int32_t nnodes, hipStream_t stream, BvhNode4 *out);
void refit_scatter(const float *d_src, int32_t first, int32_t count, TriAttr *attrs, hipStream_t stream);
void refit_leaves(const RefitScene &r, hipStream_t stream);
void refit_level(const RefitScene &r, const int32_t *d_order, int32_t count, float pad, hipStream_t stream);
void accel_cost(const BvhNode *d_nodes, int32_t nnodes, const int32_t *d_order, int32_t count, double *d_out, hipStream_t stream);
struct HostMesh { std::vector<float> verts, uvs; std::vector<int32_t> idx; int32_t material = 0; };
struct HostTexture { int32_t w = 0, h = 0; std::vector<float> rgba; };
struct HostStats { uint64_t rays = 0; };
struct ProxyHost { std::vector<float4> slabs; std::vector<float> hm; int32_t planes = 0; float rin = 0.f, rout = 0.f; };
void default_splat_proxy(std::vector<float> &verts, std::vector<int32_t> &tris);
bool build_proxy_slabs(const float *verts, int32_t nverts, const int32_t *tris, int32_t ntris, ProxyHost *out, std::string *why);
void sum_row_errors(const std::vector<RowError> &rows, const std::vector<char> &held, double npix, double out[3]);
}

struct evplp_context;
namespace evplp {
bool update_mesh_check(evplp_context *c, int32_t mesh, const float *vertices, int32_t nverts);
bool refit_check(evplp_context *c);
bool accel_quality_check(evplp_context *c, const char *name);
bool refit_policy_check(evplp_context *c, double max_cost_ratio, int32_t rebuild_builder);
NoisePlanes noise_planes(const evplp_context *c);
NoiseMoments noise_moments_of(const evplp_context *c);
size_t noise_bytes(const evplp_context *c);
int noise_rows(evplp_context *c, const NoiseMoments &m, const float4 *light, double K, double B, float scale, float ls, int32_t mask_emitter);
int noise_variance_to_device(evplp_context *c, const NoiseMoments &m, double K, double B, float scale);
void adaptive_tiles_into(const evplp_context *c, int32_t *out);
void adaptive_budgets_into(const evplp_context *c, int32_t *out);
int adaptive_tile_noise_into(evplp_context *c, float scale, float ls, int32_t mask_emitter, double *out);
struct DenoiseSettings { int32_t levels; float sigma_l, sigma_n, sigma_x; };
bool denoise_settings(const evplp_denoise_params *p, DenoiseSettings *out, char *why, size_t cap);
int denoise_keep_variance(evplp_context *c);
int denoise_prepare(evplp_context *c, const float4 *pos, const float4 *nrm, const float4 *dif, const float4 *phg, const float4 *light);
int denoise_filter(evplp_context *c, const DenoisePixel *frame, int rows, const DenoiseSettings &ds, float radius, float *out_rgb);
}

struct evplp_context {
    evplp_config cfg{};
    evplp::StripDev st{};
    int32_t rows_in_image = 0;
    std::vector<int32_t> blocks_host; int32_t *d_blocks = nullptr; int32_t image_blocks = 0;
    bool calibrate = false; unsigned long long *d_block_cost = nullptr;
    hipStream_t own_stream = nullptr, stream = nullptr;
    hipEvent_t ev_begin[EVPLP_PASS_COUNT] = {}, ev_end[EVPLP_PASS_COUNT] = {};
    hipEvent_t ev_dom_begin[EVPLP_PASS_COUNT] = {}, ev_dom_end[EVPLP_PASS_COUNT] = {};
    bool pass_ran[EVPLP_PASS_COUNT] = {}, pass_has_dom[EVPLP_PASS_COUNT] = {};
    bool profile_passes = true, pass_timed[EVPLP_PASS_COUNT] = {};
    bool profile_kernels = false;
    evplp::HostStats stats_host[EVPLP_PASS_COUNT];

    void *buf[EVPLP_BUF_COUNT] = {};
    bool buf_owned[EVPLP_BUF_COUNT] = {};

    std::vector<evplp::HostMesh> meshes;
    std::vector<evplp::Material> materials;
    std::vector<evplp::HostTexture> textures;
    int32_t light_mesh = -1;
    float light_unscaled[4] = {}, light_scaled[4] = {};
    evplp::CamBasis cam{}; evplp_camera cam_in{};
    bool camera_set = false, accel_built = false;
    float bounding_radius = 0.f, total_area = 0.f, light_area = 0.f;
    int32_t accel_nodes = 0, accel_leaves = 0, accel_depth = 0, accel_builder_used = -1; float accel_build_ms = 0.f;

    std::vector<char> mesh_dirty, tri_dropped; bool scene_dirty = false;
    std::vector<evplp::BvhNode> host_nodes; std::vector<int32_t> refit_level_begin; int32_t refit_levels = 0;
    int32_t *d_refit_order = nullptr; float *d_refit_boxes = nullptr, *d_refit_stage = nullptr, *h_refit_stage = nullptr;
    hipEvent_t ev_refit_staged = nullptr, ev_refit[5] = {}; bool refit_timed = false, refit_stages_timed = false;
    int32_t refit_count = 0, scene_tris = 0; float accel_pad = 0.f;
    int32_t refit_reached = 0, refit_leaf_refs = 0;
    double *d_cost = nullptr, *h_cost = nullptr; hipEvent_t ev_cost[2] = {}; bool cost_timed = false;
    double built_cost = 0.0, policy_ratio = 0.0; bool built_cost_known = false;
    int32_t policy_builder = -1, refits_since_build = 0, policy_rebuilds = 0, last_action = 0;

    evplp::SceneDev sc{};
    evplp_record *d_vpls = nullptr; uint32_t *d_vpl_src = nullptr;
    uint32_t *d_scalars = nullptr;
    evplp::PassCounters *d_counters = nullptr;
    float *d_rgb = nullptr;
    float4 *d_partial = nullptr; size_t partial_groups = 0;
    int32_t *d_lt_overflow = nullptr; size_t lt_overflow_bytes = 0;
    char *d_primary_cuts = nullptr; bool primary_cuts_valid = false;
    char *d_cuts = nullptr; size_t cut_bytes = 0, cut_cap = 0;
    size_t mask_cap = 0;
    void *d_vsl_masks = nullptr; size_t vsl_mask_bytes = 0;

    int32_t tiles_x = 0, tiles_y = 0; uint32_t bin_stride = 0, last_bin_entries = 0, last_bin_max = 0;
    hipStream_t aux_stream = nullptr; hipEvent_t ev_records_read = nullptr, ev_light_done = nullptr; bool light_in_flight = false;
    void *records_back = nullptr; hipEvent_t ev_back_read = nullptr; bool records_exposed = false;
    void *gbuf_back[4] = { nullptr, nullptr, nullptr, nullptr }; float4 *d_tile_box_back = nullptr; bool gbuf_exposed = false;
    bool gbuf_pos_exposed = false;
    bool tile_box_valid = false;
    int32_t num_bin_groups = 0, bucket_w_log2 = 0, bucket_h_log2 = 0, buckets_x = 0, num_buckets = 0;
    uint32_t *d_seg = nullptr, *d_big_list = nullptr, *d_big_count = nullptr; uint16_t *d_seg_off = nullptr;
    uint32_t *d_tile_cursor = nullptr, *d_bin_items = nullptr, *d_bin_items_tmp = nullptr;
    float4 *d_compact = nullptr; float4 *d_tile_box = nullptr; uint32_t *d_tile_pairs = nullptr; uint32_t *d_summary = nullptr;
    float4 *d_proxy_slabs = nullptr; float *d_proxy_hm = nullptr; int32_t proxy_count = 0; float proxy_rin = 0.f, proxy_rout = 0.f;
    uint32_t *d_tile_frags = nullptr; bool last_splat_proxy = false;
    uint32_t *d_heavy_list = nullptr; uint8_t *d_tile_flags = nullptr; uint32_t heavy_cap = 0, heavy_threshold = 256, mixed_trigger = 512; int env_tile_mixed = 1;
    uint32_t *h_summary = nullptr;
    struct PendingSplat { evplp::SplatArgs args; hipEvent_t ev = nullptr; uint32_t *h = nullptr; };
    PendingSplat pend[2];
    int npend = 0;

    int32_t env_bvh_builder = -1, env_gather_k = 0, env_tile_block_log2 = -1, env_cuts = -1;
    int32_t env_item_deal = -1;
    int32_t env_split_min = 0;
    size_t env_cut_bytes = 0;

    void (*quiesce)(void *) = nullptr; void *quiesce_arg = nullptr; std::thread::id worker_tid{};

    float *d_err_ref = nullptr; uint8_t *d_err_keep = nullptr;
    evplp::RowError *d_err_rows = nullptr; std::vector<evplp::RowError> err_rows;
    char *d_noise = nullptr; size_t noise_stride = 0; uint8_t *d_noise_keep = nullptr;
    evplp::RowError *d_noise_rows = nullptr; std::vector<evplp::RowError> noise_rows;
    int64_t noise_k = 0, noise_b = 0;
    int64_t adapt_n = 0; int4 *d_adapt_tiles = nullptr; float4 *d_adapt_snap = nullptr; std::vector<int4> adapt_tiles; int32_t adapt_last = 0;
    bool adapt_pt = false;
    char *d_pt_batch = nullptr; size_t pt_batch_bytes = 0; uint64_t pt_batch_cap = 1ull << 30;
    int32_t *d_pt_first = nullptr; uint32_t *d_pt_table = nullptr; size_t pt_table_items = 0;
    bool adapt_budget = false; double *d_tile_noise = nullptr;
    bool adapt_gather_budget = false; int32_t adapt_window = 16; int64_t adapt_m = 0; int4 *d_adapt_mask = nullptr; int64_t splat_n = 0;
    float *d_dn_var = nullptr; evplp::DenoisePixel *d_dn_pack = nullptr; float4 *d_dn_u = nullptr; size_t dn_u_px = 0;

    char error[512] = "";
    void set_error(const char *fmt, ...);
};
```

evplp_amd/csrc/kernels.h:

```cpp
#pragma once
#include "evplp_types.h"

namespace evplp {

struct PrimaryArgs {
    SceneDev sc; StripDev st; CamBasis cam;
    float jitter[2]; int32_t clear_light; int32_t pad;
    float4 *g_pos, *g_nrm, *g_dif, *g_phg, *g_light;
    float4 *tile_box;
    const char *cuts; int32_t cut_gw_log2, cut_gh_log2, cut_groups_x, pad2;
};
struct PrimaryCutArgs {
    const BvhNode *nodes; StripDev st; CamBasis cam;
    int32_t tiles_x, tiles_y, gw_log2, gh_log2, groups_x, groups_y;
    char *cuts;
};
void launch_primary_cuts(const PrimaryCutArgs &a, hipStream_t s);

struct LightTraceArgs {
    SceneDev sc;
    uint32_t rng_seed, path_begin, path_count, photons_per_path;
    evplp_record *records;
    int32_t *stack_overflow;
    uint32_t overflow_stride, pad;
};
#ifndef EVPLP_LT_STACK
#define EVPLP_LT_STACK 20
#endif
constexpr int kLtLdsStack = EVPLP_LT_STACK;
inline int lt_overflow_entries(const SceneDev &sc) {
    const int generic = 3 * ((sc.bvh_depth + 1) / 2) + 4;
    const int worst = sc.stack4_entries > 0 && sc.stack4_entries < generic ? sc.stack4_entries : generic;
    return worst > kLtLdsStack ? worst - kLtLdsStack : 0;
}

struct PassCounters {
    unsigned long long rays;
    unsigned long long nodes;
    unsigned long long pairs;
    unsigned long long aux;
    unsigned long long hist[64];
    unsigned long long shard_rays[64], shard_shaded[64];
    unsigned long long nonfinite;
};
#ifndef EVPLP_DEBUG_NAN
#define EVPLP_DEBUG_NAN 0
#endif
constexpr int kCounterShards = 64;

struct GatherArgs {
    SceneDev sc; StripDev st;
    const float4 *g_pos, *g_nrm, *g_dif, *g_phg;
    const evplp_record *vpls;
    const uint32_t *vpl_src_index;
    const uint32_t *nvpl;
    evplp_frame_params fp;
    float pdf_mc2; int32_t pad0;
    float4 *out;
    float4 *partial;
    size_t partial_stride;
    PassCounters *counters;
    int32_t splits_per_wave;
    int32_t block_h_log2;
    int32_t group_first, group_count;
    unsigned long long *vsl_masks; int32_t masks_per_split; int32_t pad1;
    const char *cuts; uint32_t cut_vpl_stride; int32_t cut_gw_log2, cut_gh_log2, cut_groups_x;
    int32_t band_first, band_rows, cut_group_row_first;
    int32_t item_deal;
    unsigned long long *block_cost;
};
struct AdaptArgs { const int4 *tiles; const float4 *snap; int32_t n1, pad; };
constexpr int kCutEntries = 8;
constexpr int kCutNodes = kCutEntries / 2;
constexpr int kCutSlotBytes = kCutNodes * 64;
struct CutArgs {
    const BvhNode *nodes;
    const float4 *tile_box;
    int32_t tiles_x, tiles_y;
    int32_t gw_log2, gh_log2;
    int32_t groups_x, groups_y;
    int32_t group_row_first, pad;
    const evplp_record *vpls; const uint32_t *nvpl; uint32_t vpl_stride;
    char *cuts;
    const int4 *adapt_tiles;
};
void launch_gather_cuts(const CutArgs &a, hipStream_t s);
void launch_tile_boxes(const StripDev &st, const float4 *g_pos, float4 *tile_box, int tiles_x, int tiles_y, hipStream_t s);
#ifndef EVPLP_VPL_SPLIT
#define EVPLP_VPL_SPLIT 128
#endif
constexpr int kVplSplit = EVPLP_VPL_SPLIT;
#ifndef EVPLP_GATHER_K
#define EVPLP_GATHER_K 2
#endif
constexpr int kDefaultSplitsPerWave = EVPLP_GATHER_K;

struct PathTraceArgs {
    SceneDev sc; StripDev st;
    const float4 *g_pos, *g_nrm, *g_dif, *g_phg;
    float camera_pos[3]; uint32_t rng_seed;
    uint32_t max_bounces, do_accumulate;
    float4 *out;
    PassCounters *counters;
};

constexpr int kPtBatchMaxSamples = 64;
constexpr int kPtBatchMaxTiles = 1 << 25;
constexpr size_t kPtBatchSlotBytes = 4 * 64 * sizeof(float4);
struct PtBatchSamples { float jitter[kPtBatchMaxSamples][2]; uint32_t seed[kPtBatchMaxSamples]; };
__host__ __device__ inline int32_t pt_tile_samples(int32_t mode, int4 r, int32_t S) {
    return mode == 0 ? S : mode == 1 ? (r.x == 0 ? S : 0) : (r.w < 0 || r.w > S ? S : r.w);
}
__host__ __device__ inline bool gather_tile_takes(int4 r, int32_t phase, int32_t S) {
    return r.w < 0 || phase < (r.w < S ? r.w : S);
}
constexpr int kGatherBudgetMaxWindow = 64;
void launch_gather_budget_mask(const int4 *tiles, int32_t ntiles, int32_t phase, int32_t window, int4 *mask, hipStream_t s);
void launch_gather_budget_step(int4 *tiles, const int4 *mask, int32_t ntiles, hipStream_t s);
void launch_gather_reduce_budget(const GatherArgs &a, int stencil_test, const int4 *tiles, const int4 *mask, float4 *snap, int32_t n1, hipStream_t s);
struct PtBatchChunk {
    const uint32_t *table; const int32_t *total;
    int32_t item_first, item_count;
    float4 *staging;
    unsigned long long cut_mask;
};
void launch_pt_batch_table(const int4 *tiles, int32_t ntiles, int32_t mode, int32_t samples, int32_t *first, uint32_t *table, hipStream_t s);
void launch_pt_batch_primary(const PrimaryArgs &a, const PtBatchSamples &sm, const PtBatchChunk &ch, hipStream_t s);
void launch_pt_batch_trace(const PathTraceArgs &a, const PtBatchSamples &sm, const PtBatchChunk &ch, hipStream_t s);
void launch_pt_batch_accumulate(const StripDev &st, float4 *plane, const int32_t *first, int32_t ntiles, const PtBatchChunk &ch, hipStream_t s);
void launch_pt_batch_close(const StripDev &st, int4 *tiles, int32_t mode, const int32_t *first, const float4 *snap, float4 *out, int32_t n_after, int32_t ntiles, hipStream_t s);

constexpr int kSummaryShards = 1024, kSummaryStride = 32, kSummaryFinal = kSummaryShards * kSummaryStride;
constexpr int kSummaryHeavy = kSummaryFinal + 8;
#ifndef EVPLP_BIN_CHUNKS
#define EVPLP_BIN_CHUNKS 1
#endif
constexpr int kBinChunks = EVPLP_BIN_CHUNKS;
constexpr int kBinGroup = 256 * kBinChunks;
constexpr int kSegCap = 4 * kBinGroup;
#ifndef EVPLP_SCATTER_G
#define EVPLP_SCATTER_G 2
#endif
constexpr int kScatterG = EVPLP_SCATTER_G;
constexpr int kMaxBuckets = 1024;
constexpr int kBucketTilesLog2 = 7;
constexpr int kMaxBucketTilesLog2 = 9;
struct SplatArgs {
    StripDev st; CamBasis cam;
    evplp_frame_params fp;
    const float4 *g_pos, *g_nrm, *g_dif, *g_phg;
    const evplp_record *records; uint32_t num_records;
    float4 *out;
    uint32_t *tile_pairs;
    float4 *tile_box;
    uint32_t *tile_cursor;
    uint32_t *bin_items;
    uint32_t bin_stride;
    uint32_t *seg;
    uint16_t *seg_off;
    uint32_t *big_list;
    uint32_t *big_count;
    int32_t num_bin_groups, bucket_w_log2, bucket_h_log2, buckets_x, num_buckets;
    uint32_t *bin_items_tmp;
    float4 *compact;
    uint32_t *overflow;
    uint32_t *summary;
    int32_t tiles_x, tiles_y; int32_t deterministic; int32_t boxes_valid;
    PassCounters *counters;
    const float4 *proxy_slabs; const float *proxy_hm; int32_t proxy_count; float proxy_rin, proxy_rout;
    uint32_t *tile_frags;
    uint32_t *heavy_list; uint8_t *tile_flags; uint32_t heavy_cap, heavy_threshold;
};
constexpr int kMaxProxySlabs = EVPLP_MAX_PROXY_PLANES;
constexpr float kProxyOpen = 1.0e15f;
constexpr int kSplatTile = 8;
constexpr int kCompactF4 = 4;

inline size_t lane_stack_bytes(const SceneDev &sc) { return (size_t)(sc.bvh_depth + 2) * 64 * sizeof(int32_t); }
inline size_t lane_stack_bytes4(const SceneDev &sc) {
    const int generic = 3 * ((sc.bvh_depth + 1) / 2) + 4;
    const int entries = sc.stack4_entries > 0 ? (sc.stack4_entries < generic ? sc.stack4_entries : generic) : generic;
    return (size_t)entries * 64 * sizeof(int32_t);
}

void launch_primary(const PrimaryArgs &a, hipStream_t s);
void launch_light_trace(const LightTraceArgs &a, hipStream_t s);
void launch_compact_vpl(const evplp_record *records, uint32_t nrec, evplp_record *out, uint32_t *src_index,
                        uint32_t *count_out, hipStream_t s);
void launch_gather_vpl_items(const GatherArgs &a, hipStream_t s, const AdaptArgs &ad = AdaptArgs{});
void launch_gather_vsl(const GatherArgs &a, hipStream_t s, const AdaptArgs &ad = AdaptArgs{});
int gather_launch_tiles(const GatherArgs &a);
void launch_gather_reduce(const GatherArgs &a, int stencil_test, hipStream_t s, const AdaptArgs &ad = AdaptArgs{});
void launch_gather_lvc(const GatherArgs &a, const evplp_record *records, hipStream_t s);
void launch_path_trace(const PathTraceArgs &a, hipStream_t s, const AdaptArgs &ad = AdaptArgs{});
void launch_splat_bin(const SplatArgs &a, hipStream_t s);
void launch_splat_tiles(const SplatArgs &a, bool split_tiles, hipStream_t s, hipEvent_t dominant_begin, hipEvent_t dominant_end);
void launch_resolve(const StripDev &st, const float4 *vpl, const float4 *pm, const float4 *light,
                    float vs, float ps, float ls, int mask_emitter, int gamma, float *out_rgb, hipStream_t s);
void launch_assemble_strips(const StripDev &st, int nranks, const uint32_t *owner, int chunk_rows, const float *gathered, float *frame, hipStream_t s, int channels = 3);
struct ShardPlanes { const float4 *p[64]; };
void launch_reduce_shards(const ShardPlanes &src, int n, int first_nonzero, size_t count, float4 *out, int num_cus, hipStream_t s);
void launch_fill_zero(void *p, size_t bytes, hipStream_t s);
struct RowError { double num, rel, rel_kept, kept; };
static_assert(sizeof(RowError) == 32, "RowError must be 32 bytes");
void launch_frame_error(const StripDev &st, const float *rgb, const float *ref, const uint8_t *keep, RowError *rows, hipStream_t s);
struct NoisePlanes { double *q; float4 *prev, *start; size_t stride; };
struct NoiseMoments { const double *q, *s; const float4 *prev, *start; size_t stride; };
void launch_noise_pool(const NoiseMoments &src, bool first, double *q, double *s_out, size_t n, hipStream_t s);
struct AdaptTiles { const int4 *tiles; int32_t tiles_x, pad; double n, scale; };
void launch_noise_fold(const NoisePlanes &m, const float4 *vpl, const float4 *pm, const StripDev &st, const AdaptTiles &at, int32_t k, hipStream_t s);
void launch_noise_rows(const StripDev &st, const NoiseMoments &m, double K, double B, double s2K, const float4 *light, float ls, int mask_emitter,
                       const float *rgb, const uint8_t *keep, RowError *rows, const AdaptTiles &at, hipStream_t s);
void launch_noise_variance(const StripDev &st, const NoiseMoments &m, double K, double B, double s2K, float *out_rgb, const AdaptTiles &at, hipStream_t s);
void launch_adaptive_retire(const StripDev &st, const NoiseMoments &m, double K, double B, double s2K, const float4 *light, float ls, int mask_emitter,
                            const float *rgb, double tau, int4 *tiles, int32_t tiles_x, int32_t tiles_y, int32_t n, const float4 *vpl, float4 *snap, hipStream_t s);

void launch_noise_fold_budget(const NoisePlanes &m, const StripDev &st, int4 *tiles, const float4 *snap, int32_t ntiles, hipStream_t s);
void launch_tile_noise(const StripDev &st, const NoiseMoments &m, double K, double B, double s2K, const float4 *light, float ls, int mask_emitter,
                       const float *rgb, const AdaptTiles &at, int32_t ntiles, double *out, hipStream_t s);

struct DenoisePixel { float4 u, pos, nrm, albedo, rgb; };
static_assert(sizeof(DenoisePixel) == 80, "DenoisePixel must be 80 bytes");
constexpr int kDenoiseFloats = (int)(sizeof(DenoisePixel) / sizeof(float));
void launch_denoise_prepare(const StripDev &st, const float *rgb, const float *var, const float4 *pos, const float4 *nrm, const float4 *dif,
                            const float4 *phg, const float4 *light, float4 *out, hipStream_t s);
struct DenoiseLevelArgs {
    const DenoisePixel *frame; const float4 *in; float4 *out;
    int32_t W, rows, in_step, h;
    float sigma_l, sigma_n, sigma_x_r, pad;
};
void launch_denoise_level(const DenoiseLevelArgs &a, hipStream_t s);
void launch_denoise_finish(const DenoisePixel *frame, const float4 *u, size_t n, float *out_rgb, hipStream_t s);

}
```

evplp_amd/csrc/kernels_cut.hip:

```cpp
#include "device_common.hpp"
#include "kernels.h"

namespace evplp {

struct CutFrustum {
    V3 p;
    float lo[3], hi[3];
    V3 pl[4]; float tol[4];
    bool planes;
};
EV_DEV bool cut_outside(const CutFrustum &F, const float c[3], const float h[3]) {
    bool out = false;
#pragma unroll
    for (int k = 0; k < 3; k++) out = out || (c[k] - h[k] > F.hi[k]) || (c[k] + h[k] < F.lo[k]);
    if (F.planes) {
        const V3 rel = v3(c[0] - F.p.x, c[1] - F.p.y, c[2] - F.p.z);
        const float mag = fabsf(rel.x) + fabsf(rel.y) + fabsf(rel.z) + h[0] + h[1] + h[2];
#pragma unroll
        for (int q = 0; q < 4; q++) {
            const V3 n = F.pl[q];
            const float far = __builtin_fmaf(fabsf(n.z), h[2], __builtin_fmaf(fabsf(n.y), h[1], __builtin_fmaf(fabsf(n.x), h[0], __builtin_fmaf(n.z, rel.z, __builtin_fmaf(n.y, rel.y, n.x * rel.x)))));
            out = out || (__builtin_fmaf(mag, F.tol[q], far) < 0.0f);
        }
    }
    return out;
}

constexpr int kCutRing = kCutEntries;
EV_DEV void cut_descend_and_store(const BvhNode *nodes, const CutFrustum &F, char *slot, bool work, int lane, int32_t (*s_ref)[64], uint32_t (*s_src)[64]) {
    int head = 0, count = 0;
    auto ring_push = [&](int32_t ref, uint32_t src) { const int at = (head + count) & (kCutRing - 1); s_ref[at][lane] = ref; s_src[at][lane] = src; count++; };
    struct Kids { int32_t r0, r1; bool k0, k1; };
    auto expand = [&](int32_t node) -> Kids {
        const float4 *q4 = reinterpret_cast<const float4 *>(nodes + node);
        const float4 n0 = q4[0], n1 = q4[1], n2 = q4[2], n3 = q4[3];
        const float c0[3] = { n0.x, n0.z, n1.x }, c1[3] = { n0.y, n0.w, n1.y };
        const float h0[3] = { n1.z, n2.x, n2.z }, h1[3] = { n1.w, n2.y, n2.w };
        Kids k; k.r0 = __float_as_int(n3.x); k.r1 = __float_as_int(n3.y);
        k.k0 = k.r0 != kNoChild && !cut_outside(F, c0, h0);
        k.k1 = k.r1 != kNoChild && !cut_outside(F, c1, h1);
        return k;
    };
    if (work) {
        {
            const Kids k = expand(0);
            if (k.k0) ring_push(k.r0, 0u);
            if (k.k1) ring_push(k.r1, 1u);
        }
        int leaves_in_row = 0;
        while (count > 0 && leaves_in_row < count) {
            const int32_t ref = s_ref[head][lane]; const uint32_t src = s_src[head][lane];
            if (ref < 0) { head = (head + 1) & (kCutRing - 1); count--; ring_push(ref, src); leaves_in_row++; continue; }
            const Kids k = expand(ref);
            if (count - 1 + (int)k.k0 + (int)k.k1 > kCutEntries) break;
            head = (head + 1) & (kCutRing - 1); count--;
            if (k.k0) ring_push(k.r0, (uint32_t)ref << 1);
            if (k.k1) ring_push(k.r1, ((uint32_t)ref << 1) | 1u);
            leaves_in_row = 0;
        }
        auto box_of = [&](int k, float c[3], float h[3], int32_t &ref) {
            const int at = (head + k) & (kCutRing - 1);
            ref = s_ref[at][lane]; const uint32_t src = s_src[at][lane];
            const float4 *q4 = reinterpret_cast<const float4 *>(nodes + (src >> 1));
            const float4 n0 = q4[0], n1 = q4[1], n2 = q4[2];
            const bool ch = (src & 1u) != 0u;
            c[0] = ch ? n0.y : n0.x; c[1] = ch ? n0.w : n0.z; c[2] = ch ? n1.y : n1.x;
            h[0] = ch ? n1.w : n1.z; h[1] = ch ? n2.y : n2.x; h[2] = ch ? n2.w : n2.z;
        };
        float dist[kCutEntries]; int order[kCutEntries];
#pragma unroll
        for (int k = 0; k < kCutEntries; k++) { order[k] = k; dist[k] = 3.0e38f; }
        const bool sort_needed = __builtin_amdgcn_ballot_w64(count > 1) != 0ull;
#pragma unroll
        for (int k = 0; k < kCutEntries; k++) {
            if (sort_needed && __builtin_amdgcn_ballot_w64(k < count) != 0ull && k < count) {
                float c[3], h[3]; int32_t r; box_of(k, c, h, r);
                const float ex = fmaxf(fabsf(F.p.x - c[0]) - h[0], 0.f), ey = fmaxf(fabsf(F.p.y - c[1]) - h[1], 0.f), ez = fmaxf(fabsf(F.p.z - c[2]) - h[2], 0.f);
                dist[k] = ex * ex + ey * ey + ez * ez;
            }
        }
#define EV_CX(i_, j_) { const bool sw = dist[j_] < dist[i_]; const float td = sw ? dist[j_] : dist[i_]; dist[j_] = sw ? dist[i_] : dist[j_]; dist[i_] = td; \
                        const int to = sw ? order[j_] : order[i_]; order[j_] = sw ? order[i_] : order[j_]; order[i_] = to; }
        static_assert(kCutEntries == 8, "the sorting network below is the 19-comparator network for 8 keys");
        if (sort_needed) {
            EV_CX(0, 1) EV_CX(2, 3) EV_CX(4, 5) EV_CX(6, 7)
            EV_CX(0, 2) EV_CX(1, 3) EV_CX(4, 6) EV_CX(5, 7)
            EV_CX(1, 2) EV_CX(5, 6) EV_CX(0, 4) EV_CX(3, 7)
            EV_CX(1, 5) EV_CX(2, 6)
            EV_CX(1, 4) EV_CX(3, 6)
            EV_CX(2, 4) EV_CX(3, 5)
            EV_CX(3, 4)
        }
#undef EV_CX
        const int nsyn = (count + 1) >> 1;
        float4 *out = reinterpret_cast<float4 *>(slot);
        if (nsyn == 0) out[3] = make_float4(0.f, 0.f, 0.f, 0.f);
#pragma unroll
        for (int s2 = 0; s2 < kCutNodes; s2++) {
            if (__builtin_amdgcn_ballot_w64(s2 < nsyn) != 0ull && s2 < nsyn) {
                float c[2][3], h[2][3]; int32_t r[2];
#pragma unroll
                for (int e = 0; e < 2; e++) {
                    if (2 * s2 + e < count) box_of(order[2 * s2 + e], c[e], h[e], r[e]);
                    else { r[e] = kNoChild; c[e][0] = c[e][1] = c[e][2] = 0.f; h[e][0] = h[e][1] = h[e][2] = -3.0e38f; }
                }
                out[4 * s2 + 0] = make_float4(c[0][0], c[1][0], c[0][1], c[1][1]);
                out[4 * s2 + 1] = make_float4(c[0][2], c[1][2], h[0][0], h[1][0]);
                out[4 * s2 + 2] = make_float4(h[0][1], h[1][1], h[0][2], h[1][2]);
                out[4 * s2 + 3] = make_float4(__int_as_float(r[0]), __int_as_float(r[1]), __int_as_float(nsyn), 0.f);
            }
        }
    }
}

template <bool ADAPT = false>
__global__ __launch_bounds__(64) void gather_cut_kernel(CutArgs a) {
    __shared__ int32_t s_ref[kCutRing][64];
    __shared__ uint32_t s_src[kCutRing][64];
    const int lane = threadIdx.x;
    const uint32_t nvpl = *a.nvpl;
    const uint32_t i = blockIdx.x % a.vpl_stride, gb = blockIdx.x / a.vpl_stride;
    if (i >= nvpl) return;
    const int gblocks_x = (a.groups_x + 7) >> 3;
    const int gx = (int)(gb % (uint32_t)gblocks_x) * 8 + (lane & 7), gyl = (int)(gb / (uint32_t)gblocks_x) * 8 + (lane >> 3);
    bool live = gx < a.groups_x && gyl < a.groups_y;
    if constexpr (ADAPT) {
        if (live) {
            const int gw = 1 << a.gw_log2, gh = 1 << a.gh_log2, gyi = a.group_row_first + gyl;
            bool retired = true;
            for (int ty = gyi * gh; ty < min((gyi + 1) * gh, a.tiles_y); ty++)
                for (int tx = gx * gw; tx < min((gx + 1) * gw, a.tiles_x); tx++) retired = retired && a.adapt_tiles[ty * a.tiles_x + tx].x != 0;
            live = !retired;
        }
    }
    if (__builtin_amdgcn_ballot_w64(live) == 0ull) return;
    const uint32_t g = (uint32_t)(min(gyl, a.groups_y - 1) * a.groups_x + min(gx, a.groups_x - 1));
    const int gy = a.group_row_first + min(gyl, a.groups_y - 1);
    const int gxc = min(gx, a.groups_x - 1);
    const float4 pv = reinterpret_cast<const float4 *>(a.vpls + i)[0];
    CutFrustum F; F.p = v3(pv.x, pv.y, pv.z);

    const int gw = 1 << a.gw_log2, gh = 1 << a.gh_log2;
    float ulo[3] = { 3.0e38f, 3.0e38f, 3.0e38f }, uhi[3] = { -3.0e38f, -3.0e38f, -3.0e38f };
    for (int ty = gy * gh; ty < min((gy + 1) * gh, a.tiles_y); ty++)
        for (int tx = gxc * gw; tx < min((gxc + 1) * gw, a.tiles_x); tx++) {
            const float4 lo = a.tile_box[2 * (ty * a.tiles_x + tx)], hi = a.tile_box[2 * (ty * a.tiles_x + tx) + 1];
            if (lo.x > hi.x) continue;
            ulo[0] = fminf(ulo[0], lo.x); ulo[1] = fminf(ulo[1], lo.y); ulo[2] = fminf(ulo[2], lo.z);
            uhi[0] = fmaxf(uhi[0], hi.x); uhi[1] = fmaxf(uhi[1], hi.y); uhi[2] = fmaxf(uhi[2], hi.z);
        }
    const bool any_tile = ulo[0] <= uhi[0];
    char *const slot = a.cuts + ((size_t)g * a.vpl_stride + i) * (size_t)kCutSlotBytes;
    if (live && !any_tile) reinterpret_cast<float4 *>(slot)[3] = make_float4(0.f, 0.f, 0.f, 0.f);
    const bool work = live && any_tile;
    if (!any_tile) { ulo[0] = ulo[1] = ulo[2] = 0.f; uhi[0] = uhi[1] = uhi[2] = 0.f; }
    {
        const float pp[3] = { F.p.x, F.p.y, F.p.z };
#pragma unroll
        for (int k = 0; k < 3; k++) {
            const float t0 = 0.0001f, t1 = 1.0f - 0.0001f;
            const float a0 = pp[k] * (1.0f - t0) + t0 * ulo[k], b0 = pp[k] * (1.0f - t0) + t0 * uhi[k];
            const float a1 = pp[k] * (1.0f - t1) + t1 * ulo[k], b1 = pp[k] * (1.0f - t1) + t1 * uhi[k];
            const float l = fminf(a0, a1), h = fmaxf(b0, b1);
            const float pad = 1.0e-5f * ((h - l) + fabsf(l) + fabsf(h)) + 1.0e-30f;
            F.lo[k] = l - pad; F.hi[k] = h + pad;
        }
    }
    {
        const V3 cen = v3(0.5f * (ulo[0] + uhi[0]), 0.5f * (ulo[1] + uhi[1]), 0.5f * (ulo[2] + uhi[2]));
        V3 m = cen - F.p;
        const float ml2 = dot(m, m);
        bool planes = ml2 > 1.0e-30f;
        m = m * __builtin_amdgcn_rsqf(fmaxf(ml2, 1.0e-30f));
        const V3 ax = fabsf(m.x) < 0.6f ? v3(1.f, 0.f, 0.f) : v3(0.f, 1.f, 0.f);
        V3 u = cross(m, ax); u = u * __builtin_amdgcn_rsqf(fmaxf(dot(u, u), 1.0e-30f));
        const V3 w = cross(m, u);
        float amin = 3.0e38f, amax = -3.0e38f, bmin = 3.0e38f, bmax = -3.0e38f;
#pragma unroll
        for (int q = 0; q < 8; q++) {
            const V3 d = v3(((q & 1) ? uhi[0] : ulo[0]) - F.p.x, ((q & 2) ? uhi[1] : ulo[1]) - F.p.y, ((q & 4) ? uhi[2] : ulo[2]) - F.p.z);
            const float dw = dot(m, d), dl2 = dot(d, d);
            if (!(dw > 0.0f) || dw * dw <= 0.0025f * dl2) planes = false;
            const float r = __builtin_amdgcn_rcpf(dw);
            const float ca = dot(u, d) * r, cb = dot(w, d) * r;
            amin = fminf(amin, ca); amax = fmaxf(amax, ca); bmin = fminf(bmin, cb); bmax = fmaxf(bmax, cb);
        }
        const float oa = 1.0e-4f * (1.0f + fmaxf(fabsf(amin), fabsf(amax))), ob = 1.0e-4f * (1.0f + fmaxf(fabsf(bmin), fabsf(bmax)));
        amin -= oa; amax += oa; bmin -= ob; bmax += ob;
        F.planes = planes;
        F.pl[0] = u - m * amin; F.pl[1] = m * amax - u; F.pl[2] = w - m * bmin; F.pl[3] = m * bmax - w;
#pragma unroll
        for (int q = 0; q < 4; q++) F.tol[q] = 4.0e-6f * (fabsf(F.pl[q].x) + fabsf(F.pl[q].y) + fabsf(F.pl[q].z));
    }

    cut_descend_and_store(a.nodes, F, slot, work, lane, s_ref, s_src);
}

__global__ __launch_bounds__(64) void primary_cut_kernel(PrimaryCutArgs a) {
    __shared__ int32_t s_ref[kCutRing][64];
    __shared__ uint32_t s_src[kCutRing][64];
    const int lane = threadIdx.x;
    const int gblocks_x = (a.groups_x + 7) >> 3;
    const int gx = (int)(blockIdx.x % (uint32_t)gblocks_x) * 8 + (lane & 7), gy = (int)(blockIdx.x / (uint32_t)gblocks_x) * 8 + (lane >> 3);
    const bool live = gx < a.groups_x && gy < a.groups_y;
    const int gxc = min(gx, a.groups_x - 1), gyc = min(gy, a.groups_y - 1);
    const int gw = 8 << a.gw_log2, gh = 8 << a.gh_log2;
    const int x0 = gxc * gw, x1 = min(x0 + gw, a.st.W) - 1;
    const int ly0 = gyc * gh, ly1 = min(ly0 + gh, a.st.local_rows) - 1;
    const int y0 = a.st.global_row(ly0), y1 = a.st.global_row(ly1);
    CutFrustum F; F.p = v3(a.cam.eye);
    const V3 S = v3(a.cam.s), U = v3(a.cam.u), Fw = v3(a.cam.f);
    const float px = 2.0f / (float)a.st.W, py = 2.0f / (float)a.st.H;
    const float ax0 = (((float)x0 + 0.5f) * px - 1.0f - px) * a.cam.aspect * a.cam.tan_half, ax1 = (((float)x1 + 0.5f) * px - 1.0f + px) * a.cam.aspect * a.cam.tan_half;
    const float by0 = (((float)min(y0, y1) + 0.5f) * py - 1.0f - py) * a.cam.tan_half, by1 = (((float)max(y0, y1) + 0.5f) * py - 1.0f + py) * a.cam.tan_half;
#pragma unroll
    for (int k = 0; k < 3; k++) { F.lo[k] = -3.0e38f; F.hi[k] = 3.0e38f; }
    F.planes = true;
    F.pl[0] = S - Fw * ax0; F.pl[1] = Fw * ax1 - S; F.pl[2] = U - Fw * by0; F.pl[3] = Fw * by1 - U;
#pragma unroll
    for (int q = 0; q < 4; q++) F.tol[q] = 4.0e-6f * (fabsf(F.pl[q].x) + fabsf(F.pl[q].y) + fabsf(F.pl[q].z));
    char *const slot = a.cuts + (size_t)(gyc * a.groups_x + gxc) * (size_t)kCutSlotBytes;
    cut_descend_and_store(a.nodes, F, slot, live, lane, s_ref, s_src);
}
void launch_primary_cuts(const PrimaryCutArgs &a, hipStream_t s) {
    const uint32_t gblocks = (uint32_t)(((a.groups_x + 7) >> 3) * ((a.groups_y + 7) >> 3));
    if (gblocks) hipLaunchKernelGGL(primary_cut_kernel, dim3(gblocks), dim3(64), 0, s, a);
}

void launch_gather_cuts(const CutArgs &a, hipStream_t s) {
    const uint32_t gblocks = (uint32_t)(((a.groups_x + 7) >> 3) * ((a.groups_y + 7) >> 3));
    if (a.vpl_stride == 0u || gblocks == 0u) return;
    if (a.adapt_tiles) hipLaunchKernelGGL(gather_cut_kernel<true>, dim3(gblocks * a.vpl_stride), dim3(64), 0, s, a);
    else hipLaunchKernelGGL(gather_cut_kernel<false>, dim3(gblocks * a.vpl_stride), dim3(64), 0, s, a);
}

}
```

evplp_amd/csrc/kernels_splat.hip:

```cpp
#include "device_common.hpp"
#include "kernels.h"
#include <cstring>

#ifndef EVPLP_PROXY_MIXED_WAVES
#define EVPLP_PROXY_MIXED_WAVES 6
#endif
#ifndef EVPLP_PROXY_WAVES
#define EVPLP_PROXY_WAVES 7
#endif
namespace evplp {

EV_DEV float rcp_hw(float x) { return __builtin_amdgcn_rcpf(x); }
EV_DEV V3 normalize_hw(V3 v) { return v * __builtin_amdgcn_rsqf(dot(v, v)); }
EV_DEV float pow_hw(float d, float e) { return e == 0.0f ? 1.0f : __builtin_amdgcn_exp2f(e * __builtin_amdgcn_logf(d)); }
EV_DEV V3 g_lambert_eval(V3 w10, V3 w12, V3 n, V3 rd) {
    if (dot(w10, n) <= 0.0f || dot(w12, n) <= 0.0f) return v3(0.f, 0.f, 0.f);
    return rd * EV_INV_PI;
}
EV_DEV V3 g_phong_eval(V3 outv, V3 inv_, V3 n, V3 rs, float e) {
    V3 r = reflect(-inv_, n);
    float d = dot(outv, r);
    if (d <= 0.00001f) return v3(0.f, 0.f, 0.f);
    return rs * (e + 2.0f) * pow_hw(d, e) * EV_INV_PI * 0.5f;
}
// ... 13 lines not shown
    v.fdir = v3(d); v.rd = v3(e); v.rs = v3(f); v.e = f.w;
    return v;
}

EV_DEV uint2 photon_rect(const SplatArgs &a, V3 pos) {
    const uint2 none = make_uint2(1u, 0u);
    const float r = a.fp.photon_radius;
    V3 q = pos - v3(a.cam.eye);
    float vx = dot(q, v3(a.cam.s)), vy = dot(q, v3(a.cam.u)), vz = dot(q, v3(a.cam.f));
    const float zlo = fmaxf(vz - r, 0.1f), zhi = fminf(vz + r, 100.0f);
    if (zlo > zhi) return none;
    float sx = rcp_hw(a.cam.aspect * a.cam.tan_half), sy = rcp_hw(a.cam.tan_half);
    float il = rcp_hw(zlo), ih = rcp_hw(zhi);
    float nx0 = fminf((vx - r) * il, (vx - r) * ih) * sx + a.fp.jitter[0];
    float nx1 = fmaxf((vx + r) * il, (vx + r) * ih) * sx + a.fp.jitter[0];
    float ny0 = fminf((vy - r) * il, (vy - r) * ih) * sy + a.fp.jitter[1];
    float ny1 = fmaxf((vy + r) * il, (vy + r) * ih) * sy + a.fp.jitter[1];
    float fx0 = (nx0 * 0.5f + 0.5f) * (float)a.st.W - 0.5f, fx1 = (nx1 * 0.5f + 0.5f) * (float)a.st.W - 0.5f;
    float fy0 = (ny0 * 0.5f + 0.5f) * (float)a.st.H - 0.5f, fy1 = (ny1 * 0.5f + 0.5f) * (float)a.st.H - 0.5f;
    const float guard = 1.0f / 32.0f;
    fx0 = fminf(fmaxf(fx0 - guard, -1.0f), (float)a.st.W); fx1 = fminf(fmaxf(fx1 + guard, -1.0f), (float)a.st.W);
    fy0 = fminf(fmaxf(fy0 - guard, -1.0f), (float)a.st.H); fy1 = fminf(fmaxf(fy1 + guard, -1.0f), (float)a.st.H);
    int x0 = max((int)ceilf(fx0), 0), x1 = min((int)floorf(fx1), a.st.W - 1);
    int y0 = max((int)ceilf(fy0), 0), y1 = min((int)floorf(fy1), a.st.H - 1);
    if (x0 > x1 || y0 > y1) return none;
    int tx0 = x0 >> 3, tx1 = x1 >> 3, ty0 = y0 >> 3, ty1 = y1 >> 3;
    return make_uint2((uint32_t)tx0 | ((uint32_t)tx1 << 16), (uint32_t)ty0 | ((uint32_t)ty1 << 16));
}
EV_DEV float photon_reach2(const SplatArgs &a, V3 pos) {
    const float pmag = fmaxf(fmaxf(fabsf(pos.x), fabsf(pos.y)), fmaxf(fabsf(pos.z), 1.0f));
    const float reach = a.fp.photon_radius * (1.0f + 1.0e-5f) + 4.0e-6f * pmag;
    return reach * reach;
}
EV_DEV bool box_within(float4 blo, float4 bhi, V3 c, float reach2) {
    const float dx = fmaxf(fmaxf(blo.x - c.x, c.x - bhi.x), 0.0f), dy = fmaxf(fmaxf(blo.y - c.y, c.y - bhi.y), 0.0f),
                dz = fmaxf(fmaxf(blo.z - c.z, c.z - bhi.z), 0.0f);
    return !(dx * dx + dy * dy + dz * dz > reach2);
}
EV_DEV int local_tile_row(const SplatArgs &a, int ty) {
    if (a.st.strip_count == 1) return ty;
    const int tiles_per_block = a.st.strip_rows >> 3, blk = ty / tiles_per_block, lb = a.st.local_block(blk);
    return lb < 0 ? -1 : lb * tiles_per_block + (ty - blk * tiles_per_block);
}

EV_DEV uint2 splat_prepare_one(const SplatArgs &a, uint32_t i, const float4 *s_ph, const float4 *s_prev, V3 &photon_pos) {
    const uint2 none = make_uint2(1u, 0u);
    Rec ph = load_rec(s_ph);
    if (!(ph.flags & EVPLP_USABLE_PHOTON)) return none;
    photon_pos = ph.pos;
    const uint2 rect = photon_rect(a, ph.pos);
    if ((rect.x & 0xffffu) > (rect.x >> 16)) return none;
    Rec prev = load_rec(s_prev);

    const float r = a.fp.photon_radius;
    V3 v12 = prev.pos - ph.pos;
    float d2 = dot(v12, v12);
    V3 w12 = normalize_hw(v12);
    float mix_w = g_lambert_pdf_w(prev.n, -w12) * prev.psel;
    mix_w += g_phong_pdf_w(prev.n, -w12, prev.fdir, prev.rs, prev.e) * (1.0f - prev.psel);
    float mix_a = mix_w * fmaxf(dot(ph.n, w12), 0.0f) * rcp_hw(d2);
    bool alive = mix_w > 0.0f;
    float k = EV_INV_PI * rcp_hw(r * r);
    float inv_n = rcp_hw((float)a.fp.num_light_paths);
    float wgt = 1.0f;
    const uint32_t mode = a.fp.mis_mode;
    if (mode == 1u) wgt = mix_a * rcp_hw(mix_a + a.fp.pdf_mc);
    else if (mode == 2u) wgt = mix_a > a.fp.pdf_mc ? 1.0f : 0.0f;
    else if (mode == 3u) { float a2 = mix_a * mix_a, b2 = a.fp.pdf_mc * a.fp.pdf_mc; wgt = a2 * rcp_hw(a2 + b2); }
    V3 wflux = ph.flux * (k * inv_n * wgt);
    float cpn = fmaxf(-dot(prev.n, w12), 0.0f);
    V3 brdf2 = g_lambert_eval(-w12, prev.fdir, prev.n, prev.rd) + g_phong_eval(-w12, prev.fdir, prev.n, prev.rs, prev.e);
    float4 *c = a.compact + (size_t)i * kCompactF4;
    c[0] = make_float4(ph.pos.x, ph.pos.y, ph.pos.z, cpn);
    c[1] = make_float4(w12.x, w12.y, w12.z, d2);
    c[2] = make_float4(wflux.x, wflux.y, wflux.z, alive ? 1.0f : 0.0f);
    if (mode == 5u) c[3] = make_float4(brdf2.x, brdf2.y, brdf2.z, 0.f);
    return rect;
}

__global__ __launch_bounds__(256) void splat_tile_box_kernel(SplatArgs a) {
    const int tid = threadIdx.x, lane = tid & 63, wave = tid >> 6;
    const int ntiles = a.tiles_x * a.tiles_y;
    const int tile0 = (blockIdx.x * 4 + wave) * 4;
    float4 gp[4]; bool in_image[4];
#pragma unroll
    for (int q = 0; q < 4; q++) {
        const int tile = min(tile0 + q, ntiles - 1);
        const int tx = tile % a.tiles_x, lty = tile / a.tiles_x;
        const int x = tx * 8 + (lane & 7), ly = lty * 8 + (lane >> 3);
        in_image[q] = x < a.st.W && ly < a.st.local_rows && a.st.global_row(min(ly, a.st.local_rows - 1)) < a.st.H;
        gp[q] = a.g_pos[(size_t)min(ly, a.st.local_rows - 1) * a.st.W + min(x, a.st.W - 1)];
    }
#pragma unroll
    for (int q = 0; q < 4; q++) {
        const int tile = tile0 + q;
        if (tile >= ntiles) break;
        float lo[3] = { 3.0e38f, 3.0e38f, 3.0e38f }, hi[3] = { -3.0e38f, -3.0e38f, -3.0e38f };
        if (in_image[q]) { lo[0] = hi[0] = gp[q].x; lo[1] = hi[1] = gp[q].y; lo[2] = hi[2] = gp[q].z; }
        for (int off = 32; off > 0; off >>= 1)
            for (int k = 0; k < 3; k++) { lo[k] = fminf(lo[k], __shfl_xor(lo[k], off)); hi[k] = fmaxf(hi[k], __shfl_xor(hi[k], off)); }
        if (lane == 0) {
            a.tile_box[2 * tile] = make_float4(lo[0], lo[1], lo[2], 0.f); a.tile_box[2 * tile + 1] = make_float4(hi[0], hi[1], hi[2], 0.f);
        }
    }
}

#define EV_BIN_FETCH(base_)                                                                                             \
    {                                                                                                                   \
        const float4 *src = reinterpret_cast<const float4 *>(a.records) + (size_t)(base_) * kRecF4;                      \
        const uint32_t n4 = (min((base_) + 256u, a.num_records) - (base_)) * kRecF4, last = n4 - 1u;                      \
        r0_ = src[min(tid, last)]; r1_ = src[min(tid + 256u, last)]; r2_ = src[min(tid + 512u, last)];                    \
        r3_ = src[min(tid + 768u, last)]; r4_ = src[min(tid + 1024u, last)]; r5_ = src[min(tid + 1280u, last)];           \
        pv = *(src + (((base_) != 0u && tid < (uint32_t)kRecF4) ? (int)tid - kRecF4 : 0));                                \
    }
#define EV_BIN_STAGE(base_)                                                                                             \
    {                                                                                                                   \
        const uint32_t n4 = (min((base_) + 256u, a.num_records) - (base_)) * kRecF4;                                      \
        float4 *dst = s_rec + kRecF4;                                                                                   \
        if (tid < n4) dst[tid] = r0_;                                                                                   \
        if (tid + 256u < n4) dst[tid + 256u] = r1_;                                                                     \
        if (tid + 512u < n4) dst[tid + 512u] = r2_;                                                                     \
        if (tid + 768u < n4) dst[tid + 768u] = r3_;                                                                     \
        if (tid + 1024u < n4) dst[tid + 1024u] = r4_;                                                                   \
        if (tid + 1280u < n4) dst[tid + 1280u] = r5_;                                                                   \
        if ((base_) != 0u && tid < (uint32_t)kRecF4) s_rec[tid] = pv;                                                   \
    }
__global__ __launch_bounds__(256) void splat_bin_kernel(SplatArgs a) {
    __shared__ float4 s_rec[257 * kRecF4];
    __shared__ uint32_t s_pair[kSegCap];
    extern __shared__ uint32_t s_bucket_lds[];
    const uint32_t nb4 = ((uint32_t)a.num_buckets + 3u) & ~3u;
    uint32_t *const s_cnt = s_bucket_lds, *const s_off = s_bucket_lds + nb4;
    __shared__ uint32_t s_n, s_nbig, s_wsum[4];
    const uint32_t tid = threadIdx.x, group = blockIdx.x, wg_base = group * (uint32_t)kBinGroup;
    for (uint32_t b = tid; b < nb4; b += 256u) s_cnt[b] = 0u;
    if (tid == 0u) { s_n = 0u; s_nbig = 0u; }
    for (uint32_t k = blockIdx.x * 256u + tid; k < (uint32_t)(a.tiles_x * a.tiles_y); k += gridDim.x * 256u) a.tile_cursor[k] = 0u;
    if (blockIdx.x == 0u) {
        for (uint32_t k = tid; k < (uint32_t)kSummaryShards; k += 256u) { a.summary[k * kSummaryStride] = 0u; a.summary[k * kSummaryStride + 1] = 0u; }
        if (tid == 0u) { *a.overflow = 0u; a.summary[kSummaryHeavy] = 0u; }
    }
    const uint32_t bw_mask = (1u << a.bucket_w_log2) - 1u, bh_mask = (1u << a.bucket_h_log2) - 1u;

    float4 r0_, r1_, r2_, r3_, r4_, r5_, pv;
    if (wg_base < a.num_records) EV_BIN_FETCH(wg_base)
    for (int c = 0; c < kBinChunks; c++) {
        const uint32_t base = wg_base + 256u * (uint32_t)c;
        if (base >= a.num_records) break;
        EV_BIN_STAGE(base)
        __syncthreads();
        if (c + 1 < kBinChunks && base + 256u < a.num_records) EV_BIN_FETCH(base + 256u)
        const uint32_t i = base + tid;
        uint2 rc = make_uint2(1u, 0u);
        V3 c0 = v3(0.f, 0.f, 0.f);
        if (i < a.num_records && i != 0u) rc = splat_prepare_one(a, i, &s_rec[(tid + 1u) * kRecF4], &s_rec[tid * kRecF4], c0);
        const int tx0 = rc.x & 0xffff, tx1 = rc.x >> 16, ty0 = rc.y & 0xffff, ty1 = rc.y >> 16;
        const float reach2 = photon_reach2(a, c0);
#if EVPLP_TRAVERSAL_STATS
        { const int nx_ = tx1 - tx0 + 1, ny_ = ty1 - ty0 + 1; int cls = tx0 > tx1 ? 0 : (nx_ <= 2 && ny_ <= 2) ? 1 : (nx_ <= 3 && ny_ <= 3) ? 2 : 3;
          atomicAdd(&a.counters->hist[cls], 1ull); if (cls) { atomicAdd(&a.counters->hist[4], (unsigned long long)(nx_ * ny_)); atomicAdd(&a.counters->hist[8 + min(nx_ * ny_, 16)], 1ull); } }
#endif
        if (tx0 > tx1) {
        } else if (tx1 - tx0 <= 2 && ty1 - ty0 <= 2) {
            int tx[9], lty[9]; float4 blo[9], bhi[9];
#pragma unroll
            for (int q = 0; q < 9; q++) {
                tx[q] = tx0 + (q % 3);
                const int ty = ty0 + (q / 3);
                lty[q] = (tx[q] <= tx1 && ty <= ty1) ? local_tile_row(a, ty) : -1;
            }
#pragma unroll
            for (int q = 0; q < 9; q++) if (lty[q] >= 0) { const int t = lty[q] * a.tiles_x + tx[q]; blo[q] = a.tile_box[2 * t]; bhi[q] = a.tile_box[2 * t + 1]; }
            uint32_t hit = 0u;
#pragma unroll
            for (int q = 0; q < 9; q++) if (lty[q] >= 0 && box_within(blo[q], bhi[q], c0, reach2)) hit |= 1u << q;
            const uint32_t cnt = (uint32_t)__builtin_popcount(hit);
            uint32_t at = cnt ? atomicAdd(&s_n, cnt) : 0u;
            if (at + cnt > (uint32_t)kSegCap) {
                for (uint32_t k = at; k < min(at + cnt, (uint32_t)kSegCap); k++) s_pair[k] = 0xffffffffu;
                a.big_list[(size_t)group * kBinGroup + atomicAdd(&s_nbig, 1u)] = i;
            } else {
#pragma unroll
                for (int q = 0; q < 9; q++) if (hit & (1u << q)) {
                    const uint32_t b = (uint32_t)(lty[q] >> a.bucket_h_log2) * (uint32_t)a.buckets_x + (uint32_t)(tx[q] >> a.bucket_w_log2);
                    const uint32_t tib = (((uint32_t)lty[q] & bh_mask) << a.bucket_w_log2) | ((uint32_t)tx[q] & bw_mask);
// ... 349 lines not shown
                }
                if (act && sub == 0u) {
                    const float nearp = 0.1f * rcp_hw(dot(D, v3(a.cam.f))) - 1.0f, slack = 1.0e-7f;
                    int count = 0;
                    if (enter < exitp) count = ((enter >= nearp && enter <= slack) ? 1 : 0) + ((exitp >= nearp && exitp <= slack) ? 1 : 0);
                    const uint32_t bit = 1u << (pj & 31u), word = pj >> 5;
                    if (count == 0) atomicOr(&verdict[pl * 4u + word], bit);
                    else if (count == 2) atomicOr(&verdict[pl * 4u + 2u + word], bit);
                }
                __builtin_amdgcn_fence(__ATOMIC_ACQ_REL, "wavefront"); __builtin_amdgcn_wave_barrier();
                const float4 vd = aux[lane];
                kill |= ((uint64_t)__float_as_uint(vd.y) << 32) | (uint64_t)__float_as_uint(vd.x);
                dbl |= ((uint64_t)__float_as_uint(vd.w) << 32) | (uint64_t)__float_as_uint(vd.z);
                __builtin_amdgcn_fence(__ATOMIC_ACQ_REL, "wavefront"); __builtin_amdgcn_wave_barrier();
            }
            mask &= ~kill;
            frags += (uint32_t)__builtin_popcountll(mask) + (uint32_t)__builtin_popcountll(dbl);
        }
        while (__ballot(mask != 0ull) != 0ull) {
            if (mask != 0ull) {
                const uint32_t j = (uint32_t)__builtin_ctzll(mask);
                mask &= mask - 1ull;
                float4 c0 = stage[j], c1 = stage[64 + j], c2 = stage[128 + j];
                V3 w12 = v3(c1);
                V3 brdf1 = g_lambert_eval(w10, w12, sn, sd);
                if (tile_glossy) brdf1 = brdf1 + g_phong_eval(w10, w12, sn, sps, se);
                if (c2.w != 0.0f) {
                    V3 col;
                    if (mode <= 3u) col = brdf1 * v3(c2);
                    else {
                        float cc = fmaxf(dot(sn, w12), 0.0f) * c0.w;
                        if (cc <= 0.0f) col = v3(0.f, 0.f, 0.f);
                        else {
                            float g = cc * rcp_hw(c1.w);
                            if (mode == 4u) col = (brdf1 * v3(c2)) * (fmaxf(g - clampv, 0.0f) * rcp_hw(g));
                            else {
                                V3 brdf2 = v3(stage[192 + j]);
                                V3 num = (brdf1 * brdf2) * g;
                                num = v3(fmaxf(num.x - clampv, 0.f), fmaxf(num.y - clampv, 0.f), fmaxf(num.z - clampv, 0.f));
                                V3 den = brdf2 * g;
                                V3 pre = v3(c2);
                                col = v3(den.x != 0.f ? pre.x * num.x * rcp_hw(den.x) : 0.f, den.y != 0.f ? pre.y * num.y * rcp_hw(den.y) : 0.f,
                                         den.z != 0.f ? pre.z * num.z * rcp_hw(den.z) : 0.f);
                            }
                        }
                    }
                    sum = sum + col;
                    if (PROXY && ((dbl >> j) & 1ull) != 0ull) sum = sum + col;
                }
            }
        }
        __builtin_amdgcn_wave_barrier();
    }
    for (int off = 32; off > 0; off >>= 1) { pairs += __shfl_down(pairs, off); if (PROXY) frags += __shfl_down(frags, off); }
    if (W == 4) {
        const uint32_t frags0 = (uint32_t)__shfl((int)frags, 0);
        if (wave != 0) stage[lane] = make_float4(sum.x, sum.y, sum.z, lane == 0 ? __uint_as_float(pairs) : lane == 1 ? __uint_as_float(frags0) : 0.f);
        __syncthreads();
    }
    if (part == 0) {
        if (W == 4) for (int w = 1; w < 4; w++) {
            const float4 *other = stage_base + w * stage_rows * 64;
            float4 q = other[lane]; sum = sum + v3(q);
            if (lane == 0) { pairs += __float_as_uint(q.w); if (PROXY) frags += __float_as_uint(other[1].w); }
        }
#if EVPLP_DEBUG_NAN
        if (in_image && !(isfinite(sum.x) && isfinite(sum.y) && isfinite(sum.z))) atomicAdd(&a.counters->nonfinite, 1ull);
#endif
        if (in_image) {
            float4 o = a.out[p];
            a.out[p] = make_float4(o.x + sum.x, o.y + sum.y, o.z + sum.z, o.w);
        }
#if EVPLP_TILE_TIMES
        if (lane == 0 && tile < 65536) { g_tile_times[3 * tile] = t_start; g_tile_times[3 * tile + 1] = __builtin_amdgcn_s_memrealtime(); g_tile_times[3 * tile + 2] = (unsigned long long)(e - b); }
#endif
        if (lane == 0) {
            a.tile_pairs[tile] = pairs;
            if (PROXY) a.tile_frags[tile] = frags;
            if (pairs) atomicAdd(reinterpret_cast<unsigned long long *>(&a.summary[((uint32_t)tile & (uint32_t)(kSummaryShards - 1)) * kSummaryStride + 4]), (unsigned long long)pairs);
        }
    }
}

void launch_tile_boxes(const StripDev &st, const float4 *g_pos, float4 *tile_box, int tiles_x, int tiles_y, hipStream_t s) {
    SplatArgs a; std::memset(&a, 0, sizeof(a));
    a.st = st; a.g_pos = g_pos; a.tile_box = tile_box; a.tiles_x = tiles_x; a.tiles_y = tiles_y;
    const uint32_t ntiles = (uint32_t)(tiles_x * tiles_y);
    if (ntiles) hipLaunchKernelGGL(splat_tile_box_kernel, dim3((ntiles + 15) / 16), dim3(256), 0, s, a);
}
void launch_splat_bin(const SplatArgs &a, hipStream_t s) {
    const uint32_t ntiles = (uint32_t)(a.tiles_x * a.tiles_y);
    if (!a.boxes_valid) hipLaunchKernelGGL(splat_tile_box_kernel, dim3((ntiles + 15) / 16), dim3(256), 0, s, a);
    uint32_t *items = a.deterministic ? a.bin_items_tmp : a.bin_items;
    hipLaunchKernelGGL(splat_bin_kernel, dim3((uint32_t)a.num_bin_groups), dim3(256), sizeof(uint32_t) * 2u * (size_t)(((uint32_t)a.num_buckets + 3u) & ~3u), s, a);
    const uint32_t per = 256u * kScatterG, slices = ((uint32_t)a.num_bin_groups + per - 1u) / per, big_rows = ((uint32_t)a.num_bin_groups + slices - 1u) / slices;
    hipLaunchKernelGGL(splat_scatter_kernel, dim3(slices, (uint32_t)a.num_buckets + big_rows), dim3(256), 0, s, a, items);
}
void launch_splat_tiles(const SplatArgs &a, bool split_tiles, hipStream_t s, hipEvent_t dom_begin, hipEvent_t dom_end) {
    const uint32_t ntiles = (uint32_t)(a.tiles_x * a.tiles_y);
    if (a.deterministic) hipLaunchKernelGGL(splat_sort_kernel, dim3(ntiles), dim3(256), 0, s, a.tile_cursor, a.bin_stride, a.bin_items_tmp, a.bin_items, a.overflow);
    if (dom_begin) hipEventRecord(dom_begin, s);
    const bool proxy = a.fp.splat_footprint == (uint32_t)EVPLP_FOOTPRINT_PROXY;
    const size_t lds_bytes = sizeof(float4) * (size_t)(4 * (a.fp.mis_mode == 5u ? 4 : 3) * 64) + (proxy ? sizeof(float4) * (size_t)(4 * 64 + a.proxy_count) + sizeof(float) * (size_t)a.proxy_count : 0);
    if (a.heavy_list && !a.deterministic) {
        hipLaunchKernelGGL(splat_heavy_kernel, dim3((ntiles + 255) / 256), dim3(256), 0, s, a);
        const uint32_t grid = a.heavy_cap + (ntiles + 3) / 4;
        if (proxy) hipLaunchKernelGGL((splat_tiles_kernel<0, true>), dim3(grid), dim3(256), lds_bytes, s, a); else hipLaunchKernelGGL((splat_tiles_kernel<0, false>), dim3(grid), dim3(256), lds_bytes, s, a);
        if (dom_end) hipEventRecord(dom_end, s);
        return;
    }
    if (split_tiles) { if (proxy) hipLaunchKernelGGL((splat_tiles_kernel<4, true>), dim3(ntiles), dim3(256), lds_bytes, s, a); else hipLaunchKernelGGL((splat_tiles_kernel<4, false>), dim3(ntiles), dim3(256), lds_bytes, s, a); }
    else { if (proxy) hipLaunchKernelGGL((splat_tiles_kernel<1, true>), dim3((ntiles + 3) / 4), dim3(256), lds_bytes, s, a); else hipLaunchKernelGGL((splat_tiles_kernel<1, false>), dim3((ntiles + 3) / 4), dim3(256), lds_bytes, s, a); }
    if (dom_end) hipEventRecord(dom_end, s);
}

__global__ __launch_bounds__(256) void resolve_kernel(StripDev st, const float4 *vpl, const float4 *pm, const float4 *light,
                                                      float vs, float ps, float ls, int mask_emitter, int gamma, float *out_rgb) {
    const size_t i = (size_t)blockIdx.x * 256 + threadIdx.x;
    const size_t n = (size_t)st.W * st.local_rows;
    if (i >= n) return;
    float4 v = vpl[i], q = pm[i], l = light[i];
    float lx = l.x * ls;
    float stepv = mask_emitter ? ((0.0f < lx) ? 0.0f : 1.0f) : 1.0f;
    float r = stepv * (v.x * vs + q.x * ps) + l.x * ls;
    float g = stepv * (v.y * vs + q.y * ps) + l.y * ls;
    float b = stepv * (v.z * vs + q.z * ps) + l.z * ls;
    if (gamma) { r = powf(r, 1.0f / 2.2f); g = powf(g, 1.0f / 2.2f); b = powf(b, 1.0f / 2.2f); }
    out_rgb[3 * i + 0] = r; out_rgb[3 * i + 1] = g; out_rgb[3 * i + 2] = b;
}
void launch_resolve(const StripDev &st, const float4 *vpl, const float4 *pm, const float4 *light,
                    float vs, float ps, float ls, int mask_emitter, int gamma, float *out_rgb, hipStream_t s) {
    size_t n = (size_t)st.W * st.local_rows;
    hipLaunchKernelGGL(resolve_kernel, dim3((unsigned)((n + 255) / 256)), dim3(256), 0, s, st, vpl, pm, light, vs, ps, ls, mask_emitter, gamma, out_rgb);
}
template <bool FirstNonzero>
__global__ __launch_bounds__(256) void reduce_shards_kernel(ShardPlanes src, int n, size_t count, float4 *out) {
    const size_t stride = (size_t)gridDim.x * 256;
    for (size_t i = (size_t)blockIdx.x * 256 + threadIdx.x; i < count; i += stride) {
        float4 acc = make_float4(0.f, 0.f, 0.f, 0.f);
        bool have = false;
        for (int r0 = 0; r0 < n; r0 += 4) {
            float4 v[4];
#pragma unroll
            for (int k = 0; k < 4; k++) v[k] = r0 + k < n ? src.p[r0 + k][i] : make_float4(0.f, 0.f, 0.f, 0.f);
#pragma unroll
            for (int k = 0; k < 4; k++) {
                if (r0 + k >= n) break;
                if (FirstNonzero) {
                    const bool nz = v[k].x != 0.f || v[k].y != 0.f || v[k].z != 0.f || v[k].w != 0.f;
                    if (!have && nz) { acc = v[k]; have = true; }
                } else if (r0 + k == 0) acc = v[k];
                else { acc.x = __fadd_rn(acc.x, v[k].x); acc.y = __fadd_rn(acc.y, v[k].y); acc.z = __fadd_rn(acc.z, v[k].z); acc.w = __fadd_rn(acc.w, v[k].w); }
            }
        }
        out[i] = acc;
    }
}
void launch_reduce_shards(const ShardPlanes &src, int n, int first_nonzero, size_t count, float4 *out, int num_cus, hipStream_t s) {
    const size_t blocks = std::min<size_t>((count + 255) / 256, (size_t)std::max(num_cus, 1) * 8);
    if (blocks == 0) return;
    if (first_nonzero) hipLaunchKernelGGL(reduce_shards_kernel<true>, dim3((unsigned)blocks), dim3(256), 0, s, src, n, count, out);
    else hipLaunchKernelGGL(reduce_shards_kernel<false>, dim3((unsigned)blocks), dim3(256), 0, s, src, n, count, out);
}
__global__ __launch_bounds__(256) void assemble_strips_kernel(StripDev st, int nranks, const uint32_t *owner, int chunk_rows, const float *gathered, float *frame, int channels) {
    const size_t i = (size_t)blockIdx.x * 256 + threadIdx.x;
    const size_t row_floats = (size_t)st.W * channels, n = row_floats * (size_t)st.H;
    if (i >= n) return;
    const int y = (int)(i / row_floats); const size_t x = i - (size_t)y * row_floats;
    const int blk = y / st.strip_rows; int r, lb;
// ... 12 lines not shown
```

evplp_amd/csrc/kernels_trace.hip:

```cpp
#include "device_common.hpp"
#include "kernels.h"

namespace evplp {

#ifndef EVPLP_PRIMARY_BLOCKS
#define EVPLP_PRIMARY_BLOCKS 1
#endif
#ifndef EVPLP_PRIMARY_BLOCK_LOG2
#define EVPLP_PRIMARY_BLOCK_LOG2 2
#endif
#if EVPLP_PRIMARY_TIMES
__device__ unsigned long long g_primary_times[2 * 65536];
extern "C" int evplp_debug_primary_times(unsigned long long *out, int n) { return (int)hipMemcpyFromSymbol(out, HIP_SYMBOL(g_primary_times), sizeof(unsigned long long) * (size_t)n); }
#endif
__global__ __launch_bounds__(64) void primary_kernel(PrimaryArgs a) {
#pragma clang fp contract(off)
#if EVPLP_PRIMARY_TIMES
    const unsigned long long t_start = __builtin_amdgcn_s_memrealtime();
#endif
    const int lane = threadIdx.x;
    const int tiles_x = (a.st.W + 7) >> 3;
#if EVPLP_PRIMARY_BLOCKS
    constexpr int L = EVPLP_PRIMARY_BLOCK_LOG2, B = 1 << L;
    const int tiles_y = (a.st.local_rows + 7) >> 3, nbx = (tiles_x + B - 1) >> L;
    const int bj = (int)blockIdx.x >> 3, blk = (bj >> (2 * L)) * 8 + ((int)blockIdx.x & 7), within = bj & (B * B - 1);
    const int tx = (blk % nbx) * B + (within & (B - 1)), ty = (blk / nbx) * B + (within >> L);
    if (tx >= tiles_x || ty >= tiles_y) return;
    const int tile = ty * tiles_x + tx;
#else
    const int tile = blockIdx.x;
    const int tx = tile % tiles_x, ty = tile / tiles_x;
#endif
    const int x = tx * 8 + (lane & 7);
    const int ly = ty * 8 + (lane >> 3);
    const int y = a.st.global_row(min(ly, a.st.local_rows - 1));
    const bool in_image = x < a.st.W && ly < a.st.local_rows && y < a.st.H;
    const size_t p = (size_t)min(ly, a.st.local_rows - 1) * a.st.W + min(x, a.st.W - 1);

#define PRIMARY_JIT0 a.jitter[0]
#define PRIMARY_JIT1 a.jitter[1]
#define PRIMARY_USE_CUT a.cuts
#include "primary_body.hpp"
#undef PRIMARY_JIT0
#undef PRIMARY_JIT1
#undef PRIMARY_USE_CUT
    if (a.tile_box) {
        float lo[3] = { 3.0e38f, 3.0e38f, 3.0e38f }, hi[3] = { -3.0e38f, -3.0e38f, -3.0e38f };
        if (in_image) { lo[0] = hi[0] = pos.x; lo[1] = hi[1] = pos.y; lo[2] = hi[2] = pos.z; }
        for (int off = 32; off > 0; off >>= 1)
            for (int k = 0; k < 3; k++) { lo[k] = fminf(lo[k], __shfl_xor(lo[k], off)); hi[k] = fmaxf(hi[k], __shfl_xor(hi[k], off)); }
        if (lane == 0) { a.tile_box[2 * tile] = make_float4(lo[0], lo[1], lo[2], 0.f); a.tile_box[2 * tile + 1] = make_float4(hi[0], hi[1], hi[2], 0.f); }
    }
#if EVPLP_PRIMARY_TIMES
    if (lane == 0 && tile < 65536) { g_primary_times[2 * tile] = t_start; g_primary_times[2 * tile + 1] = __builtin_amdgcn_s_memrealtime(); }
#endif
    if (!in_image) return;
    a.g_pos[p] = pos; a.g_nrm[p] = nrm; a.g_dif[p] = dif; a.g_phg[p] = phg;
    if (!(a.clear_light & EVPLP_LIGHT_SKIP)) {
        if (light_visible) a.g_light[p] = make_float4(a.sc.light_unscaled[0], a.sc.light_unscaled[1], a.sc.light_unscaled[2], 0.f);
        else if (a.clear_light & EVPLP_LIGHT_CLEAR) a.g_light[p] = make_float4(0.f, 0.f, 0.f, 0.f);
    }
}

EV_DEV float russian_prob_lt(V3 f) { return fminf(fmaxf(f.x, fmaxf(f.y, f.z)), 0.98f); }

EV_DEV void store_record(evplp_record *r, V3 pos, uint32_t flags, V3 n, float psel, V3 flux, V3 fdir, V3 rd, V3 rs, float e) {
    float4 *q = reinterpret_cast<float4 *>(r);
    q[0] = make_float4(pos.x, pos.y, pos.z, __uint_as_float(flags));
    q[1] = make_float4(n.x, n.y, n.z, psel);
    q[2] = make_float4(flux.x, flux.y, flux.z, 0.f);
    q[3] = make_float4(fdir.x, fdir.y, fdir.z, 0.f);
    q[4] = make_float4(rd.x, rd.y, rd.z, 0.f);
    q[5] = make_float4(rs.x, rs.y, rs.z, e);
}

#ifndef EVPLP_LT_WAVES
#define EVPLP_LT_WAVES 4
#endif
#ifndef EVPLP_LT_PAIRS
#define EVPLP_LT_PAIRS 1
#endif
#ifndef EVPLP_LT_SPEC
#define EVPLP_LT_SPEC 1
#endif
#if EVPLP_LT_TIMES
__device__ unsigned long long g_lt_times[2 * 16384];
extern "C" int evplp_debug_lt_times(unsigned long long *out, int n) { return (int)hipMemcpyFromSymbol(out, HIP_SYMBOL(g_lt_times), sizeof(unsigned long long) * (size_t)n); }
#endif
__global__ __launch_bounds__(64, EVPLP_LT_WAVES) void light_trace_kernel(LightTraceArgs a) {
    extern __shared__ int32_t lds_stack[];
#if EVPLP_LT_TIMES
    const unsigned long long t_start = __builtin_amdgcn_s_memrealtime();
#endif
    const int lane = threadIdx.x;
    const uint32_t local = blockIdx.x * 64u + lane;
    if (local >= a.path_count) return;
    const uint32_t id = a.path_begin + local;
    const uint32_t P = a.photons_per_path;
    evplp_record *rec = a.records + (size_t)id * P;
    int32_t *stack = lds_stack + lane;

    const V3 zero = v3(0.f, 0.f, 0.f);
    uint32_t filled = 1;

    Rng rng; rng_init(rng, id, a.rng_seed, 0u);
    V3 position, normal; float pdf;
    V3 flux = light_sample(a.sc, position, normal, pdf, rng);
    V3 direction; float phong_pdf;
    V3 att = phong_sample(direction, phong_pdf, normal, normal, v3(1.f, 1.f, 1.f), a.sc.light_intensity[3], rng);
    store_record(&rec[0], position, EVPLP_USABLE_VPL, normal, 0.0f, flux, normal, zero, v3(1.f, 1.f, 1.f), a.sc.light_intensity[3]);

    V3 pflux = flux * att;
    V3 next_pos = position, next_dir = direction;
    for (uint32_t i = 1; i < P; i++) {
        uint32_t flag = (i != P - 1) ? (EVPLP_USABLE_VPL | EVPLP_USABLE_PHOTON) : EVPLP_USABLE_PHOTON;
        float t, b, g;
        int32_t tri = closest_lane4<64, kLtLdsStack, EVPLP_LT_SPEC, EVPLP_LT_PAIRS != 0>(a.sc, next_pos, next_dir, 0.0001f, 3.0e38f, 0, t, b, g, stack, a.stack_overflow + local, a.overflow_stride);
        if (tri < 0) break;
        const TriAttr &ta = a.sc.attrs[tri];
        V3 p0 = v3(ta.v), p1 = v3(ta.v + 3), p2 = v3(ta.v + 6);
        V3 gn = normalize_exact(cross_exact(p0 - p2, p1 - p0));
        V3 wgn = normalize_exact(gn);
        V3 ffn = wgn * copysignf(1.0f, dot_exact(-next_dir, wgn));
        V3 hit_pos = madd_exact(next_pos, next_dir, t);
        const Material &m = a.sc.materials[ta.material];
        if (dot_exact(gn, next_dir) > 0.f || m.light[0] > 0.01f) break;
        V3 kd, ks; float ns;
        material_at(a.sc, ta, b, g, kd, ks, ns);
        float max_l = max_color(kd), max_p = max_color(ks);
        if (max_l + max_p <= 0.000001f) break;
        float psel = max_l / (max_p + max_l);
        float choose = fminf(rng_uniform(rng), 0.999999f);
        float russian = russian_prob_lt(pflux);
        V3 stored_flux = pflux;
// ... 77 lines not shown
```

Before: 46870.

## Cull VPL cuts by VPL and receiver normal bounds per tile group

Per-tile normal bounds are now computed alongside the position bounds in the primary and tile-box kernels. Gather-cut setup uses them to skip VPLs whose tile group lies entirely behind the VPL's surface, or whose receivers all face away from it. It also adds a fifth plane from the VPL normal to the cut-descent frustum test so BVH nodes behind the VPL are pruned. The aim is to drop VPL–tile work that contributes nothing. The cost is extra shuffle reductions, a larger tile-box table, cull counters updated with atomics, and more state to invalidate when the G-buffer is exposed or uploaded.

```diff
diff --git a/evplp_amd/__init__.py b/evplp_amd/__init__.py
--- a/evplp_amd/__init__.py
+++ b/evplp_amd/__init__.py
@@ -687,7 +687,7 @@
         self._check(self._lib.evplp_profile_passes(self._h, int(on)))
 
     def debug_counters(self, which: int) -> np.ndarray:
-        out = np.zeros(256, dtype=np.uint64)
+        out = np.zeros(320, dtype=np.uint64)
         n = self._check(self._lib.evplp_debug_counters(self._h, which, _ptr(out), out.size))
         return out[:n]
 
diff --git a/evplp_amd/csrc/context.cpp b/evplp_amd/csrc/context.cpp
--- a/evplp_amd/csrc/context.cpp
+++ b/evplp_amd/csrc/context.cpp
@@ -73,6 +73,7 @@
     if (const char *env = std::getenv("EVPLP_BVH_BUILDER"))
         c->env_bvh_builder = !std::strcmp(env, "sbvh") ? EVPLP_BVH_SBVH : !std::strcmp(env, "lbvh") ? EVPLP_BVH_LBVH : !std::strcmp(env, "gpu") ? EVPLP_BVH_LBVH_GPU : EVPLP_BVH_SAH;
     if (const char *env = std::getenv("EVPLP_CUTS")) c->env_cuts = atoi(env) != 0 ? 1 : 0;
+    if (const char *env = std::getenv("EVPLP_CUT_CULLS")) c->env_cut_culls = atoi(env) & 7;
     if (const char *env = std::getenv("EVPLP_ITEM_DEAL")) c->env_item_deal = atoi(env) != 0 ? 1 : 0;
     if (const char *env = std::getenv("EVPLP_CUT_BYTES")) c->env_cut_bytes = (size_t)strtoull(env, nullptr, 10);
     if (const char *env = std::getenv("EVPLP_GATHER_K")) { int v = atoi(env); if (v >= 1 && v <= 32 && (v & (v - 1)) == 0) c->env_gather_k = v; }
@@ -144,7 +145,7 @@
         }
         c->num_bin_groups = (int32_t)((nrec + kBinGroup - 1) / kBinGroup);
     }
-    if ((e = hipMalloc((void **)&c->d_tile_box, sizeof(float4) * 2 * std::max<size_t>(ntiles, 1))) != hipSuccess) return fail("hipMalloc(tile_box)", e);
+    if ((e = hipMalloc((void **)&c->d_tile_box, sizeof(float4) * 4 * std::max<size_t>(ntiles, 1))) != hipSuccess) return fail("hipMalloc(tile_box)", e);
     if ((e = hipMalloc((void **)&c->d_summary, sizeof(uint32_t) * (kSummaryFinal + kSummaryStride))) != hipSuccess) return fail("hipMalloc(summary)", e);
     if (const char *env = std::getenv("EVPLP_TILE_MIXED")) c->env_tile_mixed = atoi(env) != 0 ? 1 : 0;
     if (const char *env = std::getenv("EVPLP_TILE_HEAVY")) c->heavy_threshold = (uint32_t)std::max(atoi(env), 1);
@@ -626,7 +627,7 @@
     if (c->aux_stream) HIP_TRY(c, hipStreamWaitEvent(c->aux_stream, c->ev_refit_staged, 0));
     HIP_TRY(c, hipGetLastError());
     c->accel_pad = pad; c->refit_timed = timed; c->refit_stages_timed = stages; c->refit_count++; c->refits_since_build++;
-    c->primary_cuts_valid = false; c->tile_box_valid = false;
+    c->primary_cuts_valid = false; c->tile_box_valid = false; c->tile_nrm_valid = false;
     std::fill(c->mesh_dirty.begin(), c->mesh_dirty.end(), 0); c->scene_dirty = false;
     if (c->policy_ratio > 0.0) {
         double q[5];
@@ -824,6 +825,7 @@
     return EVPLP_OK;
 }
 
+static float4 *tile_nrm_of(const evplp_context *c) { return c->d_tile_box + 2 * std::max<size_t>((size_t)c->tiles_x * c->tiles_y, 1); }
 static bool jitter_within_cuts(const evplp_context *c, const float jitter[2]) {
     return std::fabs(jitter[0]) <= 1.99f / (float)c->st.W && std::fabs(jitter[1]) <= 1.99f / (float)c->st.H;
 }
@@ -857,7 +859,7 @@
             if (me != hipSuccess) { c->set_error("evplp_primary: second G-buffer: %s", hipGetErrorString(me)); return EVPLP_ERR_OOM; }
         }
         if (!c->d_tile_box_back) {
-            hipError_t me = hipMalloc((void **)&c->d_tile_box_back, sizeof(float4) * 2 * std::max<size_t>((size_t)c->tiles_x * c->tiles_y, 1));
+            hipError_t me = hipMalloc((void **)&c->d_tile_box_back, sizeof(float4) * 4 * std::max<size_t>((size_t)c->tiles_x * c->tiles_y, 1));
             if (me != hipSuccess) { c->set_error("evplp_primary: second tile-box table: %s", hipGetErrorString(me)); return EVPLP_ERR_OOM; }
         }
         for (int k = 0; k < 4; k++) std::swap(c->buf[kPlanes[k]], c->gbuf_back[k]);
@@ -869,12 +871,12 @@
     a.g_pos = (float4 *)c->buf[EVPLP_BUF_GBUF_POSITION]; a.g_nrm = (float4 *)c->buf[EVPLP_BUF_GBUF_NORMAL];
     a.g_dif = (float4 *)c->buf[EVPLP_BUF_GBUF_DIFFUSE]; a.g_phg = (float4 *)c->buf[EVPLP_BUF_GBUF_PHONG];
     a.g_light = (float4 *)c->buf[EVPLP_BUF_LIGHT];
-    a.tile_box = c->d_tile_box;
+    a.tile_box = c->d_tile_box; a.tile_nrm = tile_nrm_of(c);
     if (!std::isfinite(a.jitter[0]) || !std::isfinite(a.jitter[1])) { c->set_error("evplp_primary: jitter is not finite"); return EVPLP_ERR_INVALID; }
     if (c->env_cuts != 0 && c->tiles_x * c->tiles_y > 0 && jitter_within_cuts(c, a.jitter)) primary_cuts_into(c, a);
     if ((rc = pass_begin(c, EVPLP_PASS_PRIMARY))) return rc;
     launch_primary(a, c->stream);
-    c->tile_box_valid = !c->gbuf_pos_exposed;
+    c->tile_box_valid = !c->gbuf_pos_exposed; c->tile_nrm_valid = !c->gbuf_exposed;
     c->stats_host[EVPLP_PASS_PRIMARY].rays = 2ull * (uint64_t)c->st.W * c->rows_in_image;
     return pass_end(c, EVPLP_PASS_PRIMARY);
 }
@@ -1023,9 +1025,14 @@
     const uint32_t nrec = fp->photons_per_path * fp->num_vpl_light_paths;
     if (gbudget) launch_gather_budget_mask(c->d_adapt_tiles, ntiles_all, phase, c->adapt_window, c->d_adapt_mask, c->stream);
     launch_compact_vpl((const evplp_record *)c->buf[EVPLP_BUF_RECORDS], nrec, c->d_vpls, c->d_vpl_src, &c->d_scalars[0], c->stream);
-    if (use_cuts && !c->tile_box_valid) {
-        launch_tile_boxes(c->st, (const float4 *)c->buf[EVPLP_BUF_GBUF_POSITION], c->d_tile_box, c->tiles_x, c->tiles_y, c->stream);
-        c->tile_box_valid = !c->gbuf_pos_exposed;
+    if (use_cuts && (!c->tile_box_valid || (!c->tile_nrm_valid && !c->gbuf_exposed))) {
+        launch_tile_boxes(c->st, (const float4 *)c->buf[EVPLP_BUF_GBUF_POSITION], (const float4 *)c->buf[EVPLP_BUF_GBUF_NORMAL], c->d_tile_box, tile_nrm_of(c), c->tiles_x, c->tiles_y, c->stream);
+        c->tile_box_valid = !c->gbuf_pos_exposed; c->tile_nrm_valid = !c->gbuf_exposed;
+    }
+    if (use_cuts && !vsl) {
+        ca.tile_nrm = tile_nrm_of(c); ca.counters = &c->d_counters[pass];
+        ca.vpl_culls = 1 | 4 | ((c->tile_box_valid && c->tile_nrm_valid) ? 2 : 0);
+        if (c->env_cut_culls >= 0) ca.vpl_culls &= c->env_cut_culls;
     }
     int vsl_groups = 0, vsl_per_launch = 0;
     if (vsl) {
@@ -1814,7 +1821,7 @@
         c->st.blocks = c->d_blocks; c->st.blocks_host = c->blocks_host.data();
     } else { c->st.blocks = nullptr; c->st.blocks_host = nullptr; c->blocks_host.clear(); }
     count_rows_in_image(c);
-    c->primary_cuts_valid = false; c->tile_box_valid = false;
+    c->primary_cuts_valid = false; c->tile_box_valid = false; c->tile_nrm_valid = false;
     return evplp_clear_accumulators(c);
 }
 extern "C" int evplp_get_blocks(evplp_context *c, int32_t *image_blocks, int32_t capacity) {
@@ -1879,7 +1886,7 @@
     if (ptr) {
         *ptr = c->buf[which];
         if (which == EVPLP_BUF_GBUF_POSITION) { c->gbuf_pos_exposed = true; c->tile_box_valid = false; }
-        if (which >= EVPLP_BUF_GBUF_POSITION && which <= EVPLP_BUF_GBUF_PHONG) c->gbuf_exposed = true;
+        if (which >= EVPLP_BUF_GBUF_POSITION && which <= EVPLP_BUF_GBUF_PHONG) { c->gbuf_exposed = true; c->tile_nrm_valid = false; }
         if (which == EVPLP_BUF_RECORDS) c->records_exposed = true;
     }
     if (bytes) *bytes = buffer_bytes(c, which);
@@ -1896,7 +1903,7 @@
     if (c->buf_owned[which]) hipFree(c->buf[which]);
     c->buf[which] = ptr; c->buf_owned[which] = false;
     if (which == EVPLP_BUF_GBUF_POSITION) { c->gbuf_pos_exposed = true; c->tile_box_valid = false; }
-    if (which >= EVPLP_BUF_GBUF_POSITION && which <= EVPLP_BUF_GBUF_PHONG) c->gbuf_exposed = true;
+    if (which >= EVPLP_BUF_GBUF_POSITION && which <= EVPLP_BUF_GBUF_PHONG) { c->gbuf_exposed = true; c->tile_nrm_valid = false; }
     return EVPLP_OK;
 }
 extern "C" int evplp_download(evplp_context *c, int32_t which, void *dst, size_t bytes) {
@@ -1916,6 +1923,7 @@
     HIP_TRY(c, hipMemcpyAsync(c->buf[which], src, bytes, hipMemcpyHostToDevice, c->stream));
     HIP_TRY(c, hipStreamSynchronize(c->stream));
     if (which == EVPLP_BUF_GBUF_POSITION) c->tile_box_valid = false;
+    if (which == EVPLP_BUF_GBUF_NORMAL) c->tile_nrm_valid = false;
     return EVPLP_OK;
 }
 
diff --git a/evplp_amd/csrc/context.hpp b/evplp_amd/csrc/context.hpp
--- a/evplp_amd/csrc/context.hpp
+++ b/evplp_amd/csrc/context.hpp
@@ -99,6 +99,7 @@
     void *gbuf_back[4] = { nullptr, nullptr, nullptr, nullptr }; float4 *d_tile_box_back = nullptr; bool gbuf_exposed = false;
     bool gbuf_pos_exposed = false;
     bool tile_box_valid = false;
+    bool tile_nrm_valid = false;
     int32_t num_bin_groups = 0, bucket_w_log2 = 0, bucket_h_log2 = 0, buckets_x = 0, num_buckets = 0;
     uint32_t *d_seg = nullptr, *d_big_list = nullptr, *d_big_count = nullptr; uint16_t *d_seg_off = nullptr;
     uint32_t *d_tile_cursor = nullptr, *d_bin_items = nullptr, *d_bin_items_tmp = nullptr;
@@ -111,7 +112,7 @@
     PendingSplat pend[2];
     int npend = 0;
 
-    int32_t env_bvh_builder = -1, env_gather_k = 0, env_tile_block_log2 = -1, env_cuts = -1;
+    int32_t env_bvh_builder = -1, env_gather_k = 0, env_tile_block_log2 = -1, env_cuts = -1, env_cut_culls = -1;
     int32_t env_item_deal = -1;
     int32_t env_split_min = 0;
     size_t env_cut_bytes = 0;
diff --git a/evplp_amd/csrc/cut_cull.h b/evplp_amd/csrc/cut_cull.h
--- /dev/null
+++ b/evplp_amd/csrc/cut_cull.h
@@ -0,0 +1,49 @@
+#ifndef EVPLP_CUT_CULL_H
+#define EVPLP_CUT_CULL_H
+
+#if defined(__HIPCC__)
+#define EVC_FN __host__ __device__ static inline
+#else
+#define EVC_FN static inline
+#endif
+#if defined(__clang__)
+#define EVC_NO_CONTRACT _Pragma("clang fp contract(off)")
+#else
+#define EVC_NO_CONTRACT
+#endif
+
+#define EVC_GUARD 1.0e18f
+
+EVC_FN float evc_abs(float a) { return a < 0.0f ? -a : a; }
+EVC_FN float evc_min(float a, float b) { return a < b ? a : b; }
+EVC_FN float evc_max(float a, float b) { return a > b ? a : b; }
+
+EVC_FN int evc_vpl_side_culled(const float p[3], const float n[3], const float lo[3], const float hi[3], float nmag) {
+    EVC_NO_CONTRACT
+    float m[3]; int ok = nmag < EVC_GUARD;
+    for (int k = 0; k < 3; k++) {
+        const float A = p[k] - hi[k], B = p[k] - lo[k];
+        const float a = n[k] * A, b = n[k] * B;
+        m[k] = evc_min(a, b);
+        ok = ok && evc_abs(A) < EVC_GUARD && evc_abs(B) < EVC_GUARD && evc_abs(n[k]) < EVC_GUARD;
+    }
+    const float xy = m[0] + m[1];
+    const float low = xy + m[2];
+    return ok && low >= 0.0f;
+}
+
+EVC_FN int evc_receiver_side_culled(const float p[3], const float n[3], const float lo[3], const float hi[3], const float nlo[3], const float nhi[3]) {
+    EVC_NO_CONTRACT
+    float M[3]; int ok = 1;
+    for (int k = 0; k < 3; k++) {
+        const float A = p[k] - hi[k], B = p[k] - lo[k];
+        const float a0 = nlo[k] * A, a1 = nlo[k] * B, b0 = nhi[k] * A, b1 = nhi[k] * B;
+        M[k] = evc_max(evc_max(a0, a1), evc_max(b0, b1));
+        ok = ok && evc_abs(A) < EVC_GUARD && evc_abs(B) < EVC_GUARD && evc_abs(n[k]) < EVC_GUARD && evc_abs(nlo[k]) < EVC_GUARD && evc_abs(nhi[k]) < EVC_GUARD;
+    }
+    const float xy = M[0] + M[1];
+    const float high = xy + M[2];
+    return ok && high <= 0.0f;
+}
+
+#endif
diff --git a/evplp_amd/csrc/kernels.h b/evplp_amd/csrc/kernels.h
--- a/evplp_amd/csrc/kernels.h
+++ b/evplp_amd/csrc/kernels.h
@@ -8,6 +8,7 @@
     float jitter[2]; int32_t clear_light; int32_t pad;
     float4 *g_pos, *g_nrm, *g_dif, *g_phg, *g_light;
     float4 *tile_box;
+    float4 *tile_nrm;
     const char *cuts; int32_t cut_gw_log2, cut_gh_log2, cut_groups_x, pad2;
 };
 struct PrimaryCutArgs {
@@ -42,6 +43,7 @@
     unsigned long long hist[64];
     unsigned long long shard_rays[64], shard_shaded[64];
     unsigned long long nonfinite;
+    unsigned long long cull_pairs[32], cull_waves[32];
 };
 #ifndef EVPLP_DEBUG_NAN
 #define EVPLP_DEBUG_NAN 0
@@ -79,13 +81,16 @@
     int32_t tiles_x, tiles_y;
     int32_t gw_log2, gh_log2;
     int32_t groups_x, groups_y;
-    int32_t group_row_first, pad;
+    int32_t group_row_first;
+    int32_t vpl_culls;
+    const float4 *tile_nrm;
+    PassCounters *counters;
     const evplp_record *vpls; const uint32_t *nvpl; uint32_t vpl_stride;
     char *cuts;
     const int4 *adapt_tiles;
 };
 void launch_gather_cuts(const CutArgs &a, hipStream_t s);
-void launch_tile_boxes(const StripDev &st, const float4 *g_pos, float4 *tile_box, int tiles_x, int tiles_y, hipStream_t s);
+void launch_tile_boxes(const StripDev &st, const float4 *g_pos, const float4 *g_nrm, float4 *tile_box, float4 *tile_nrm, int tiles_x, int tiles_y, hipStream_t s);
 #ifndef EVPLP_VPL_SPLIT
 #define EVPLP_VPL_SPLIT 128
 #endif
@@ -153,6 +158,7 @@
     float4 *out;
     uint32_t *tile_pairs;
     float4 *tile_box;
+    float4 *tile_nrm;
     uint32_t *tile_cursor;
     uint32_t *bin_items;
     uint32_t bin_stride;
diff --git a/evplp_amd/csrc/kernels_cut.hip b/evplp_amd/csrc/kernels_cut.hip
--- a/evplp_amd/csrc/kernels_cut.hip
+++ b/evplp_amd/csrc/kernels_cut.hip
@@ -1,5 +1,6 @@
 #include "device_common.hpp"
 #include "kernels.h"
+#include "cut_cull.h"
 
 namespace evplp {
 
@@ -8,6 +9,7 @@
     float lo[3], hi[3];
     V3 pl[4]; float tol[4];
     bool planes;
+    bool plane5; V3 n5; float tol5, off5;
 };
 EV_DEV bool cut_outside(const CutFrustum &F, const float c[3], const float h[3]) {
     bool out = false;
@@ -22,6 +24,13 @@
             const float far = __builtin_fmaf(fabsf(n.z), h[2], __builtin_fmaf(fabsf(n.y), h[1], __builtin_fmaf(fabsf(n.x), h[0], __builtin_fmaf(n.z, rel.z, __builtin_fmaf(n.y, rel.y, n.x * rel.x)))));
             out = out || (__builtin_fmaf(mag, F.tol[q], far) < 0.0f);
         }
+    }
+    if (F.plane5) {
+        const V3 rel = v3(c[0] - F.p.x, c[1] - F.p.y, c[2] - F.p.z);
+        const float mag = fabsf(rel.x) + fabsf(rel.y) + fabsf(rel.z) + h[0] + h[1] + h[2];
+        const V3 n = F.n5;
+        const float far = __builtin_fmaf(fabsf(n.z), h[2], __builtin_fmaf(fabsf(n.y), h[1], __builtin_fmaf(fabsf(n.x), h[0], __builtin_fmaf(n.z, rel.z, __builtin_fmaf(n.y, rel.y, n.x * rel.x)))));
+        out = out || (__builtin_fmaf(mag, F.tol5, far) < F.off5);
     }
     return out;
 }
@@ -142,17 +151,44 @@
 
     const int gw = 1 << a.gw_log2, gh = 1 << a.gh_log2;
     float ulo[3] = { 3.0e38f, 3.0e38f, 3.0e38f }, uhi[3] = { -3.0e38f, -3.0e38f, -3.0e38f };
+    float nlo[3] = { 3.0e38f, 3.0e38f, 3.0e38f }, nhi[3] = { -3.0e38f, -3.0e38f, -3.0e38f };
+    const bool culls = a.vpl_culls != 0;
     for (int ty = gy * gh; ty < min((gy + 1) * gh, a.tiles_y); ty++)
         for (int tx = gxc * gw; tx < min((gxc + 1) * gw, a.tiles_x); tx++) {
             const float4 lo = a.tile_box[2 * (ty * a.tiles_x + tx)], hi = a.tile_box[2 * (ty * a.tiles_x + tx) + 1];
             if (lo.x > hi.x) continue;
             ulo[0] = fminf(ulo[0], lo.x); ulo[1] = fminf(ulo[1], lo.y); ulo[2] = fminf(ulo[2], lo.z);
             uhi[0] = fmaxf(uhi[0], hi.x); uhi[1] = fmaxf(uhi[1], hi.y); uhi[2] = fmaxf(uhi[2], hi.z);
+            if (culls) {
+                const float4 l = a.tile_nrm[2 * (ty * a.tiles_x + tx)], h = a.tile_nrm[2 * (ty * a.tiles_x + tx) + 1];
+                nlo[0] = fminf(nlo[0], l.x); nlo[1] = fminf(nlo[1], l.y); nlo[2] = fminf(nlo[2], l.z);
+                nhi[0] = fmaxf(nhi[0], h.x); nhi[1] = fmaxf(nhi[1], h.y); nhi[2] = fmaxf(nhi[2], h.z);
+            }
         }
     const bool any_tile = ulo[0] <= uhi[0];
     char *const slot = a.cuts + ((size_t)g * a.vpl_stride + i) * (size_t)kCutSlotBytes;
-    if (live && !any_tile) reinterpret_cast<float4 *>(slot)[3] = make_float4(0.f, 0.f, 0.f, 0.f);
-    const bool work = live && any_tile;
+    bool culled = false;
+    if (culls && live && any_tile) {
+        const float4 nv = reinterpret_cast<const float4 *>(a.vpls + i)[1];
+        const float pp[3] = { pv.x, pv.y, pv.z }, nn[3] = { nv.x, nv.y, nv.z };
+        float nmag = 0.0f;
+#pragma unroll
+        for (int k = 0; k < 3; k++) nmag = fmaxf(nmag, fmaxf(fabsf(nlo[k]), fabsf(nhi[k])));
+        if (!(nlo[0] <= nhi[0])) nmag = 3.0e38f;
+        culled = evc_vpl_side_culled(pp, nn, ulo, uhi, nmag) != 0;
+        if (a.vpl_culls & 2) culled = culled || evc_receiver_side_culled(pp, nn, ulo, uhi, nlo, nhi) != 0;
+    }
+    if (live && (!any_tile || culled)) reinterpret_cast<float4 *>(slot)[3] = make_float4(0.f, 0.f, 0.f, 0.f);
+    const bool work = live && any_tile && !culled;
+    const bool none_left = __builtin_amdgcn_ballot_w64(work) == 0ull;
+    if (culls) {
+        const unsigned long long cm = __builtin_amdgcn_ballot_w64(culled);
+        if (lane == 0 && cm != 0ull) {
+            atomicAdd(&a.counters->cull_pairs[blockIdx.x & 31u], (unsigned long long)__builtin_popcountll(cm));
+            if (none_left) atomicAdd(&a.counters->cull_waves[blockIdx.x & 31u], 1ull);
+        }
+    }
+    if (none_left) return;
     if (!any_tile) { ulo[0] = ulo[1] = ulo[2] = 0.f; uhi[0] = uhi[1] = uhi[2] = 0.f; }
     {
         const float pp[3] = { F.p.x, F.p.y, F.p.z };
@@ -193,6 +229,22 @@
         for (int q = 0; q < 4; q++) F.tol[q] = 4.0e-6f * (fabsf(F.pl[q].x) + fabsf(F.pl[q].y) + fabsf(F.pl[q].z));
     }
 
+    F.plane5 = false; F.n5 = v3(0.f, 0.f, 0.f); F.tol5 = 0.f; F.off5 = 0.f;
+    if (a.vpl_culls & 4) {
+        const float4 nv = reinterpret_cast<const float4 *>(a.vpls + i)[1];
+        F.n5 = v3(nv.x, nv.y, nv.z);
+        float S = 0.0f, behind = 0.0f;
+        const float pp[3] = { F.p.x, F.p.y, F.p.z }, nn[3] = { nv.x, nv.y, nv.z };
+#pragma unroll
+        for (int k = 0; k < 3; k++) {
+            S += fabsf(nn[k]) * fmaxf(fabsf(pp[k] - ulo[k]), fabsf(pp[k] - uhi[k]));
+            behind += fminf(nn[k] * (ulo[k] - pp[k]), nn[k] * (uhi[k] - pp[k]));
+        }
+        F.plane5 = __builtin_amdgcn_ballot_w64(work && !(behind > 0.0f)) != 0ull;
+        F.tol5 = 4.0e-6f * (fabsf(nv.x) + fabsf(nv.y) + fabsf(nv.z));
+        F.off5 = -1.0e-6f * S;
+        if (!(S < 1.0e30f)) { F.n5 = v3(0.f, 0.f, 0.f); F.tol5 = 0.f; F.off5 = -3.0e38f; }
+    }
     cut_descend_and_store(a.nodes, F, slot, work, lane, s_ref, s_src);
 }
 
@@ -215,7 +267,7 @@
     const float by0 = (((float)min(y0, y1) + 0.5f) * py - 1.0f - py) * a.cam.tan_half, by1 = (((float)max(y0, y1) + 0.5f) * py - 1.0f + py) * a.cam.tan_half;
 #pragma unroll
     for (int k = 0; k < 3; k++) { F.lo[k] = -3.0e38f; F.hi[k] = 3.0e38f; }
-    F.planes = true;
+    F.planes = true; F.plane5 = false; F.n5 = v3(0.f, 0.f, 0.f); F.tol5 = 0.f; F.off5 = 0.f;
     F.pl[0] = S - Fw * ax0; F.pl[1] = Fw * ax1 - S; F.pl[2] = U - Fw * by0; F.pl[3] = Fw * by1 - U;
 #pragma unroll
     for (int q = 0; q < 4; q++) F.tol[q] = 4.0e-6f * (fabsf(F.pl[q].x) + fabsf(F.pl[q].y) + fabsf(F.pl[q].z));
diff --git a/evplp_amd/csrc/kernels_splat.hip b/evplp_amd/csrc/kernels_splat.hip
--- a/evplp_amd/csrc/kernels_splat.hip
+++ b/evplp_amd/csrc/kernels_splat.hip
@@ -119,7 +119,8 @@
     const int tid = threadIdx.x, lane = tid & 63, wave = tid >> 6;
     const int ntiles = a.tiles_x * a.tiles_y;
     const int tile0 = (blockIdx.x * 4 + wave) * 4;
-    float4 gp[4]; bool in_image[4];
+    float4 gp[4], gn[4]; bool in_image[4];
+    const bool normals = a.tile_nrm != nullptr;
 #pragma unroll
     for (int q = 0; q < 4; q++) {
         const int tile = min(tile0 + q, ntiles - 1);
@@ -127,6 +128,7 @@
         const int x = tx * 8 + (lane & 7), ly = lty * 8 + (lane >> 3);
         in_image[q] = x < a.st.W && ly < a.st.local_rows && a.st.global_row(min(ly, a.st.local_rows - 1)) < a.st.H;
         gp[q] = a.g_pos[(size_t)min(ly, a.st.local_rows - 1) * a.st.W + min(x, a.st.W - 1)];
+        gn[q] = normals ? a.g_nrm[(size_t)min(ly, a.st.local_rows - 1) * a.st.W + min(x, a.st.W - 1)] : make_float4(0.f, 0.f, 0.f, 0.f);
     }
 #pragma unroll
     for (int q = 0; q < 4; q++) {
@@ -138,6 +140,15 @@
             for (int k = 0; k < 3; k++) { lo[k] = fminf(lo[k], __shfl_xor(lo[k], off)); hi[k] = fmaxf(hi[k], __shfl_xor(hi[k], off)); }
         if (lane == 0) {
             a.tile_box[2 * tile] = make_float4(lo[0], lo[1], lo[2], 0.f); a.tile_box[2 * tile + 1] = make_float4(hi[0], hi[1], hi[2], 0.f);
+        }
+        if (normals) {
+            float nl[3] = { 3.0e38f, 3.0e38f, 3.0e38f }, nh[3] = { -3.0e38f, -3.0e38f, -3.0e38f };
+            if (in_image[q]) { nl[0] = nh[0] = gn[q].x; nl[1] = nh[1] = gn[q].y; nl[2] = nh[2] = gn[q].z; }
+            for (int off = 32; off > 0; off >>= 1)
+                for (int k = 0; k < 3; k++) { nl[k] = fminf(nl[k], __shfl_xor(nl[k], off)); nh[k] = fmaxf(nh[k], __shfl_xor(nh[k], off)); }
+            if (lane == 0) {
+                a.tile_nrm[2 * tile] = make_float4(nl[0], nl[1], nl[2], 0.f); a.tile_nrm[2 * tile + 1] = make_float4(nh[0], nh[1], nh[2], 0.f);
+            }
         }
     }
 }
@@ -653,9 +664,9 @@
     }
 }
 
-void launch_tile_boxes(const StripDev &st, const float4 *g_pos, float4 *tile_box, int tiles_x, int tiles_y, hipStream_t s) {
+void launch_tile_boxes(const StripDev &st, const float4 *g_pos, const float4 *g_nrm, float4 *tile_box, float4 *tile_nrm, int tiles_x, int tiles_y, hipStream_t s) {
     SplatArgs a; std::memset(&a, 0, sizeof(a));
-    a.st = st; a.g_pos = g_pos; a.tile_box = tile_box; a.tiles_x = tiles_x; a.tiles_y = tiles_y;
+    a.st = st; a.g_pos = g_pos; a.g_nrm = g_nrm; a.tile_box = tile_box; a.tile_nrm = tile_nrm; a.tiles_x = tiles_x; a.tiles_y = tiles_y;
     const uint32_t ntiles = (uint32_t)(tiles_x * tiles_y);
     if (ntiles) hipLaunchKernelGGL(splat_tile_box_kernel, dim3((ntiles + 15) / 16), dim3(256), 0, s, a);
 }
diff --git a/evplp_amd/csrc/kernels_trace.hip b/evplp_amd/csrc/kernels_trace.hip
--- a/evplp_amd/csrc/kernels_trace.hip
+++ b/evplp_amd/csrc/kernels_trace.hip
@@ -50,6 +50,13 @@
         for (int off = 32; off > 0; off >>= 1)
             for (int k = 0; k < 3; k++) { lo[k] = fminf(lo[k], __shfl_xor(lo[k], off)); hi[k] = fmaxf(hi[k], __shfl_xor(hi[k], off)); }
         if (lane == 0) { a.tile_box[2 * tile] = make_float4(lo[0], lo[1], lo[2], 0.f); a.tile_box[2 * tile + 1] = make_float4(hi[0], hi[1], hi[2], 0.f); }
+        if (a.tile_nrm) {
+            if (in_image) { lo[0] = hi[0] = nrm.x; lo[1] = hi[1] = nrm.y; lo[2] = hi[2] = nrm.z; }
+            else { lo[0] = lo[1] = lo[2] = 3.0e38f; hi[0] = hi[1] = hi[2] = -3.0e38f; }
+            for (int off = 32; off > 0; off >>= 1)
+                for (int k = 0; k < 3; k++) { lo[k] = fminf(lo[k], __shfl_xor(lo[k], off)); hi[k] = fmaxf(hi[k], __shfl_xor(hi[k], off)); }
+            if (lane == 0) { a.tile_nrm[2 * tile] = make_float4(lo[0], lo[1], lo[2], 0.f); a.tile_nrm[2 * tile + 1] = make_float4(hi[0], hi[1], hi[2], 0.f); }
+        }
     }
 #if EVPLP_PRIMARY_TIMES
     if (lane == 0 && tile < 65536) { g_primary_times[2 * tile] = t_start; g_primary_times[2 * tile + 1] = __builtin_amdgcn_s_memrealtime(); }
```

Result: no change. 47260, median of 6 (+0.8%).
